# MoayedHajiAli/ElasticDiffusion-official

Measured on AMD Instinct MI355X. Metric: images/sec at 50 steps (SDXL 2048x1024), higher is better.
Workload: dtype fp16

## Files before the change

### elasticdiffusion_official_amd/csrc/gemm_kernels.hip

```cpp
#include <hip/hip_runtime.h>
#include <stdint.h>
#include <stdlib.h>

#include "elastic_hip.h"

namespace {

typedef float f32x4 __attribute__((ext_vector_type(4)));
typedef __bf16 bf16x8 __attribute__((ext_vector_type(8)));
typedef _Float16 f16x8 __attribute__((ext_vector_type(8)));
typedef uint32_t u32x4 __attribute__((ext_vector_type(4)));
typedef __attribute__((address_space(3))) void* lds_ptr_t;

struct BF {
  typedef bf16x8 v8;
  static __device__ __forceinline__ f32x4 mfma(v8 a, v8 b, f32x4 c) {
    return __builtin_amdgcn_mfma_f32_16x16x32_bf16(a, b, c, 0, 0, 0);
  }
  static __device__ __forceinline__ float to_f32(uint16_t h) { return __builtin_bit_cast(float, (uint32_t)h << 16); }
  static __device__ __forceinline__ uint16_t from_f32(float f) { return __builtin_bit_cast(uint16_t, (__bf16)f); }
  static __device__ __forceinline__ uint32_t pack2(float lo, float hi) {
    typedef float f2 __attribute__((ext_vector_type(2)));
    typedef __bf16 b2 __attribute__((ext_vector_type(2)));
    return __builtin_bit_cast(uint32_t, __builtin_convertvector(f2{lo, hi}, b2));
  }
};
struct HF {
  typedef f16x8 v8;
  static __device__ __forceinline__ f32x4 mfma(v8 a, v8 b, f32x4 c) {
    return __builtin_amdgcn_mfma_f32_16x16x32_f16(a, b, c, 0, 0, 0);
  }
  static __device__ __forceinline__ float to_f32(uint16_t h) { return (float)__builtin_bit_cast(_Float16, h); }
  static __device__ __forceinline__ uint16_t from_f32(float f) { return __builtin_bit_cast(uint16_t, (_Float16)f); }
  static __device__ __forceinline__ uint32_t pack2(float lo, float hi) {
    typedef float f2 __attribute__((ext_vector_type(2)));
    typedef _Float16 h2 __attribute__((ext_vector_type(2)));
    return __builtin_bit_cast(uint32_t, __builtin_convertvector(f2{lo, hi}, h2));
  }
};

constexpr int BM = 256;
constexpr int BN = 128;
constexpr int BK = 64;
constexpr int SUB = 1024;
constexpr int W_REGION = 32768;
constexpr int BUF = 65536;

__device__ __forceinline__ int swz(int p) { return p ^ (((p >> 9) & 1) << 5); }
__device__ __forceinline__ constexpr int x_sub(int rg, int kh) { return (rg * 2 + kh) * SUB; }
__device__ __forceinline__ constexpr int w_sub(int rg, int kh) { return W_REGION + (rg * 2 + kh) * SUB; }

__device__ __forceinline__ float gelu_as(float x) {
  const float z = __builtin_fabsf(x) * 0.70710678118654752f;
  const float t = __builtin_amdgcn_rcpf(__builtin_fmaf(0.3275911f, z, 1.0f));
  float p = __builtin_fmaf(1.061405429f, t, -1.453152027f);
  p = __builtin_fmaf(p, t, 1.421413741f);
  p = __builtin_fmaf(p, t, -0.284496736f);
  p = __builtin_fmaf(p, t, 0.254829592f);
  const float q = p * t * __builtin_amdgcn_exp2f(-1.4426950408889634f * z * z);
  const float h = 0.5f * x * q;
  return x > 0.f ? x - h : h;
}

__device__ __forceinline__ float abs_mul(float a, float b) {
  float r;
  asm("v_mul_f32_e64 %0, |%1|, %2" : "=v"(r) : "v"(a), "v"(b));
  return r;
}
__device__ __forceinline__ float relu1(float a) {
  float r;
  asm("v_max_f32_e32 %0, 0, %1" : "=v"(r) : "v"(a));
  return r;
}
__device__ __forceinline__ float geglu_one(float v, float g) {
  const float z = abs_mul(g, 0.70710678118654752f);
  const float t = __builtin_amdgcn_rcpf(__builtin_fmaf(0.3275911f, z, 1.0f));
  float p = __builtin_fmaf(0.5f * 1.061405429f, t, 0.5f * -1.453152027f);
  p = __builtin_fmaf(p, t, 0.5f * 1.421413741f);
  p = __builtin_fmaf(p, t, 0.5f * -0.284496736f);
  p = __builtin_fmaf(p, t, 0.5f * 0.254829592f);
  const float hq = (p * t) * __builtin_amdgcn_exp2f((-1.4426950408889634f * z) * z);
  return v * (relu1(g) - abs_mul(g, hq));
}

#define ED_WAIT_VM(n) asm volatile("s_waitcnt vmcnt(" #n ")" ::: "memory")
#define ED_WAIT_LGKM(n) asm volatile("s_waitcnt lgkmcnt(" #n ")" ::: "memory")
#define ED_BARRIER()                          \
  do {                                        \
    asm volatile("s_barrier" ::: "memory");   \
    __builtin_amdgcn_sched_barrier(0);        \
  } while (0)

struct Ctx {
  __amdgpu_buffer_rsrc_t xr, wr_;
  int x_voff[2], w_voff[2];
  int px_mask[2];
  int img_w, cin2, cpt;
  int wave;
  int xrd, wrd;
};

constexpr int CONV_UP2X = 2;
constexpr int CONV_S2 = 3;
constexpr int CONV_S2P0 = 4;
struct KPos {
  int tile, tap, ct, w;
};
template <int CONV>
__device__ __forceinline__ KPos k_next(KPos p, int cpt) {
  ++p.tile;
  if (CONV) {
    ++p.tap;
    p.w += cpt;
    if (p.tap == 9) {
      p.tap = 0;
      ++p.ct;
      p.w = p.ct;
    }
  } else {
    p.w = p.tile;
  }
  return p;
}

template <int BUFI, int CONV>
__device__ __forceinline__ void stage_x(uint8_t* lds, const Ctx& c, KPos p, int h) {
  const int rg = (c.wave & 3) + 8 * (c.wave >> 2) + 4 * h;
  uint8_t* dst = lds + BUFI * BUF + x_sub(0, 0) + rg * (2 * SUB);
  if (CONV) {
    const int dy = p.tap / 3 - 1, dx = p.tap - 3 * (p.tap / 3) - 1;
    int delta;
    if (CONV == CONV_UP2X) {
      const int yp = (c.px_mask[h] >> 16) & 1, xp = (c.px_mask[h] >> 17) & 1;
      delta = (((yp + dy) >> 1) * c.img_w + ((xp + dx) >> 1)) * c.cin2 + p.ct * (BK * 2);
    } else {
      delta = (dy * c.img_w + dx) * c.cin2 + p.ct * (BK * 2);
    }
    const int vo = ((c.px_mask[h] >> p.tap) & 1) ? c.x_voff[h] + delta : (int)0x80000000;
    __builtin_amdgcn_raw_ptr_buffer_load_lds(c.xr, (lds_ptr_t)dst, 16, vo, 0, 0, 0);
    __builtin_amdgcn_raw_ptr_buffer_load_lds(c.xr, (lds_ptr_t)(dst + SUB), 16, vo + 64, 0, 0, 0);
  } else {
    const int vo = c.x_voff[h] + p.tile * (BK * 2);
    __builtin_amdgcn_raw_ptr_buffer_load_lds(c.xr, (lds_ptr_t)dst, 16, vo, 0, 0, 0);
    __builtin_amdgcn_raw_ptr_buffer_load_lds(c.xr, (lds_ptr_t)(dst + SUB), 16, vo + 64, 0, 0, 0);
  }
}
template <int BUFI>
__device__ __forceinline__ void stage_w(uint8_t* lds, const Ctx& c, int widx, int g) {
  const int rg = 8 * g + c.wave;
  const int vo = c.w_voff[g] + widx * (BK * 2);
  uint8_t* dst = lds + BUFI * BUF + w_sub(0, 0) + rg * (2 * SUB);
  __builtin_amdgcn_raw_ptr_buffer_load_lds(c.wr_, (lds_ptr_t)dst, 16, vo, 0, 0, 0);
  __builtin_amdgcn_raw_ptr_buffer_load_lds(c.wr_, (lds_ptr_t)(dst + SUB), 16, vo + 64, 0, 0, 0);
}

template <class T>
struct Frags {
  typename T::v8 x[4][2];
  typename T::v8 wv[2][2];
  typename T::v8 wg[2][2];
};

template <class T, int BUFI>
__device__ __forceinline__ void read_x(const uint8_t* lds, const Ctx& c, Frags<T>& f, int mh) {
#pragma unroll
  for (int mf = 0; mf < 4; ++mf)
#pragma unroll
    for (int kh = 0; kh < 2; ++kh)
      f.x[mf][kh] = *reinterpret_cast<const typename T::v8*>(lds + c.xrd + BUFI * BUF + x_sub(mh * 4 + mf, kh));
}
template <class T, int BUFI, int G>
__device__ __forceinline__ void read_w(const uint8_t* lds, const Ctx& c, Frags<T>& f) {
#pragma unroll
  for (int nf = 0; nf < 2; ++nf)
#pragma unroll
    for (int kh = 0; kh < 2; ++kh) {
      typename T::v8 v = *reinterpret_cast<const typename T::v8*>(lds + c.wrd + BUFI * BUF + w_sub(8 * G + nf, kh) - W_REGION);
      if (G == 0) f.wv[nf][kh] = v; else f.wg[nf][kh] = v;
    }
}

template <class T, int MH, int G>
__device__ __forceinline__ void mma16(f32x4 (&acc)[8][4], const Frags<T>& f) {
  __builtin_amdgcn_s_setprio(1);
#pragma unroll
  for (int kh = 0; kh < 2; ++kh)
#pragma unroll
    for (int mf = 0; mf < 4; ++mf)
#pragma unroll
      for (int nf = 0; nf < 2; ++nf)
        acc[MH * 4 + mf][G * 2 + nf] = T::mfma(G == 0 ? f.wv[nf][kh] : f.wg[nf][kh], f.x[mf][kh], acc[MH * 4 + mf][G * 2 + nf]);
  __builtin_amdgcn_s_setprio(0);
}

template <class T, int BUFI, int CONV, bool FIRST = false>
__device__ __forceinline__ void tile_phases(uint8_t* lds, const Ctx& c, Frags<T>& f, f32x4 (&acc)[8][4], int tile, bool s1,
                                            bool s2, KPos p1, KPos p2) {
  read_w<T, BUFI, 0>(lds, c, f);
  __builtin_amdgcn_sched_barrier(0);
  read_x<T, BUFI>(lds, c, f, 0);
  if (s1) stage_x<BUFI ^ 1, CONV>(lds, c, p1, 1);
  ED_WAIT_LGKM(8);
  if (FIRST) ED_WAIT_VM(10);
  ED_BARRIER();
  ED_WAIT_LGKM(0);
  __builtin_amdgcn_sched_barrier(0);
  mma16<T, 0, 0>(acc, f);
  if (FIRST) ED_WAIT_VM(10);
  ED_BARRIER();
  read_w<T, BUFI, 1>(lds, c, f);
  if (s2) stage_w<BUFI>(lds, c, p2.w, 0);
  if (FIRST) ED_WAIT_VM(10);
  ED_BARRIER();
  ED_WAIT_LGKM(0);
  __builtin_amdgcn_sched_barrier(0);
  mma16<T, 0, 1>(acc, f);
  if (FIRST) ED_WAIT_VM(10);
  ED_BARRIER();
  read_x<T, BUFI>(lds, c, f, 1);
  if (s2) stage_x<BUFI, CONV>(lds, c, p2, 0);
  ED_BARRIER();
  ED_WAIT_LGKM(0);
  __builtin_amdgcn_sched_barrier(0);
  mma16<T, 1, 1>(acc, f);
  ED_BARRIER();
  if (s2) {
    stage_w<BUFI>(lds, c, p2.w, 1);
    ED_WAIT_VM(6);
  } else {
    ED_WAIT_VM(0);
  }
  ED_BARRIER();
  mma16<T, 1, 0>(acc, f);
  ED_BARRIER();
}

constexpr int TWO_MIN_TILES = 20;
template <class T, int BUFI, int CONV>
__device__ __forceinline__ void tile_phases_two(uint8_t* lds, const Ctx& c, Frags<T>& f, f32x4 (&acc)[8][4], int tile, bool s1, bool s2,
                                                KPos p1, KPos p2) {
  read_w<T, BUFI, 0>(lds, c, f);
  read_x<T, BUFI>(lds, c, f, 0);
  read_w<T, BUFI, 1>(lds, c, f);
  if (s1) stage_x<BUFI ^ 1, CONV>(lds, c, p1, 1);
  ED_WAIT_LGKM(0);
  ED_BARRIER();
  mma16<T, 0, 0>(acc, f);
  mma16<T, 0, 1>(acc, f);
  ED_BARRIER();
  read_x<T, BUFI>(lds, c, f, 1);
  if (s2) {
    stage_w<BUFI>(lds, c, p2.w, 0);
    stage_x<BUFI, CONV>(lds, c, p2, 0);
    stage_w<BUFI>(lds, c, p2.w, 1);
    ED_WAIT_VM(6);
  } else {
    ED_WAIT_VM(0);
  }
  ED_WAIT_LGKM(0);
  ED_BARRIER();
  mma16<T, 1, 1>(acc, f);
  mma16<T, 1, 0>(acc, f);
  ED_BARRIER();
}

template <class T, int BUFI, int CONV>
__device__ __forceinline__ void tile_phases_half(uint8_t* lds, const Ctx& c, Frags<T>& f, f32x4 (&acc)[8][4], int tile, bool s1, bool s2,
                                                 KPos p1, KPos p2) {
  read_w<T, BUFI, 0>(lds, c, f);
  read_x<T, BUFI>(lds, c, f, 0);
  if (s1) stage_x<BUFI ^ 1, CONV>(lds, c, p1, 1);
  ED_WAIT_LGKM(0);
  ED_BARRIER();
  mma16<T, 0, 0>(acc, f);
  ED_BARRIER();
  read_x<T, BUFI>(lds, c, f, 1);
  if (s2) {
    stage_w<BUFI>(lds, c, p2.w, 0);
    stage_x<BUFI, CONV>(lds, c, p2, 0);
    ED_WAIT_VM(4);
  } else {
    ED_WAIT_VM(0);
  }
  ED_WAIT_LGKM(0);
  ED_BARRIER();
  mma16<T, 1, 0>(acc, f);
  ED_BARRIER();
}

template <class T, int BUFI, int CONV>
__device__ __forceinline__ void tile_phases_rows(uint8_t* lds, const Ctx& c, Frags<T>& f, f32x4 (&acc)[8][4], bool s1, bool s2, KPos p1,
                                                 KPos p2) {
  read_w<T, BUFI, 0>(lds, c, f);
  read_x<T, BUFI>(lds, c, f, 0);
  if (s1) stage_w<BUFI ^ 1>(lds, c, p1.w, 1);
  ED_WAIT_LGKM(0);
  ED_BARRIER();
  mma16<T, 0, 0>(acc, f);
  ED_BARRIER();
  read_w<T, BUFI, 1>(lds, c, f);
  if (s2) {
    stage_w<BUFI>(lds, c, p2.w, 0);
    stage_x<BUFI, CONV>(lds, c, p2, 0);
    ED_WAIT_VM(4);
  } else {
    ED_WAIT_VM(0);
  }
  ED_WAIT_LGKM(0);
  ED_BARRIER();
  mma16<T, 0, 1>(acc, f);
  ED_BARRIER();
}

template <class T, int EPI, int CONV, bool ADD = true, bool OUT32 = false, bool TWO = false, bool ROWS = false>
__global__ void __launch_bounds__(512, 2)
k_gemm_8phase(const uint16_t* __restrict__ x, const uint16_t* __restrict__ w, const uint16_t* __restrict__ bias,
              const uint16_t* __restrict__ row_bias, const uint16_t* __restrict__ residual, uint16_t* __restrict__ out, int M,
              int K, int I, int n_blocks_n, int n_blocks, int img_h, int img_w, int rows_per_sample, float out_scale,
              const float* __restrict__ act_absmax) {
  __shared__ __attribute__((aligned(1024))) uint8_t lds[2 * BUF];

  const int bid = blockIdx.x;
  const int q = n_blocks >> 3, r = n_blocks & 7, xcd = bid & 7;
  const int tid = (xcd < r ? xcd * (q + 1) : r * (q + 1) + (xcd - r) * q) + (bid >> 3);
  const int n_blocks_m = n_blocks / n_blocks_n;
  const int per_group = 8 * n_blocks_n, grp = tid / per_group, first = grp * 8;
  const int rows_here = n_blocks_m - first < 8 ? n_blocks_m - first : 8;
  constexpr int TBM = ROWS ? BM / 2 : BM;
  constexpr int WROWS = TBM / 2;
  constexpr int NMB = WROWS / 16;
  const int m0 = (first + (tid % per_group) % rows_here) * TBM;
  const int n0 = ((tid % per_group) / rows_here) * (EPI == 0 ? BN : 2 * BN);
  const int gap = EPI == 0 ? I : BN;

  const int lane = threadIdx.x & 63;
  Ctx c;
  c.wave = __builtin_amdgcn_readfirstlane(threadIdx.x >> 6);
  const int wrow = c.wave >> 2, wcol = c.wave & 3;

  const int ps = swz(16 * lane), srow = ps >> 6, skb = ps & 63;
  const int row_bytes = K * 2;
  const int x_row_bytes = CONV ? row_bytes / 9 : row_bytes;
  c.xr = __builtin_amdgcn_make_buffer_rsrc((void*)x, 0, (int)((int64_t)(CONV == CONV_UP2X ? M / 4 : CONV >= CONV_S2 ? 4 * (int64_t)M : M) * x_row_bytes),
                                           0x00020000);
  c.wr_ = __builtin_amdgcn_make_buffer_rsrc((void*)w, 0, (int)((int64_t)(EPI == 0 ? 2 : 1) * I * row_bytes), 0x00020000);
  const int xrow0 = m0 + ((c.wave & 3) + (ROWS ? 4 : 8) * (c.wave >> 2)) * 16 + srow;
  c.x_voff[0] = xrow0 * x_row_bytes + skb;
  c.x_voff[1] = c.x_voff[0] + 64 * x_row_bytes;
  c.img_w = CONV == CONV_UP2X ? img_w / 2 : CONV >= CONV_S2 ? 2 * img_w : img_w;
  c.cin2 = x_row_bytes;
  c.cpt = CONV ? K / (9 * BK) : 1;
  c.px_mask[0] = c.px_mask[1] = 0;
  if (CONV) {
#pragma unroll
    for (int h = 0; h < 2; ++h) {
      const int m = xrow0 + 64 * h;
      if (m < M) {
        const int rem = m % (img_h * img_w), py = rem / img_w, px = rem - py * img_w;
        int mask = 0;
#pragma unroll
        for (int t = 0; t < 9; ++t) {
          if (CONV == CONV_S2) {
            if (2 * py + t / 3 - 1 >= 0 && 2 * px + t % 3 - 1 >= 0) mask |= 1 << t;
          } else if (CONV == CONV_S2P0) {
            if (2 * py + t / 3 < 2 * img_h && 2 * px + t % 3 < 2 * img_w) mask |= 1 << t;
          } else {
            const int yy = py + t / 3 - 1, xx = px + t % 3 - 1;
            if (yy >= 0 && yy < img_h && xx >= 0 && xx < img_w) mask |= 1 << t;
          }
        }
        c.px_mask[h] = mask;
        if (CONV == CONV_UP2X) {
          const int hs = img_h / 2, ws = img_w / 2;
          c.px_mask[h] = mask | ((py & 1) << 16) | ((px & 1) << 17);
          c.x_voff[h] = ((m / (img_h * img_w)) * (hs * ws) + (py >> 1) * ws + (px >> 1)) * x_row_bytes + skb;
        }
        if (CONV >= CONV_S2) {
          const int o1 = CONV == CONV_S2P0 ? 1 : 0;
          c.x_voff[h] = (((m / (img_h * img_w)) * (2 * img_h) + 2 * py + o1) * (2 * img_w) + 2 * px + o1) * x_row_bytes + skb;
        }
      }
    }
  }
  c.w_voff[0] = (n0 + 32 * (c.wave >> 1) + 8 * (srow >> 2) + (srow & 3) + 4 * (c.wave & 1)) * row_bytes + skb;
  c.w_voff[1] = c.w_voff[0] + gap * row_bytes;
  const int rd = swz((lane & 15) * 64 + (lane >> 4) * 16);
  c.xrd = rd + wrow * 8 * (2 * SUB);
  c.wrd = rd + W_REGION + wcol * 2 * (2 * SUB);

  const int ncol = n0 + 32 * wcol + 8 * (lane >> 4);
  u32x4 bias_v = {0, 0, 0, 0}, bias_g = {0, 0, 0, 0};
  if (bias && !OUT32) {
    if (EPI == 0 || ncol < I) bias_v = *reinterpret_cast<const u32x4*>(bias + ncol);
    if (EPI == 0 || ncol + gap < I) bias_g = *reinterpret_cast<const u32x4*>(bias + gap + ncol);
  }

  f32x4 acc[8][4];
#pragma unroll
  for (int a = 0; a < 8; ++a)
#pragma unroll
    for (int b = 0; b < 4; ++b) acc[a][b] = f32x4{0.f, 0.f, 0.f, 0.f};
  Frags<T> f;

  const int nt = K / BK;
  const KPos p0 = {0, 0, 0, 0};
  KPos pa = k_next<CONV>(p0, c.cpt);
  KPos pb = k_next<CONV>(pa, c.cpt);
  const bool half = !ROWS && EPI == 1 && n0 + BN >= I;
  if (ROWS) {
    stage_w<0>(lds, c, 0, 0);
    stage_x<0, CONV>(lds, c, p0, 0);
    stage_w<0>(lds, c, 0, 1);
    if (nt > 1) {
      stage_w<1>(lds, c, pa.w, 0);
      stage_x<1, CONV>(lds, c, pa, 0);
      ED_WAIT_VM(4);
    } else {
      ED_WAIT_VM(0);
    }
    ED_BARRIER();
    if (wrow == 1) ED_BARRIER();
    int tr = 0;
    for (; tr + 1 < nt; tr += 2) {
      tile_phases_rows<T, 0, CONV>(lds, c, f, acc, true, tr + 2 < nt, pa, pb);
      pa = pb;
      pb = k_next<CONV>(pb, c.cpt);
      tile_phases_rows<T, 1, CONV>(lds, c, f, acc, tr + 2 < nt, tr + 3 < nt, pa, pb);
      pa = pb;
      pb = k_next<CONV>(pb, c.cpt);
    }
    if (tr < nt) tile_phases_rows<T, 0, CONV>(lds, c, f, acc, false, false, pa, pb);
    if (wrow == 0) ED_BARRIER();
  } else if (half) {
    stage_w<0>(lds, c, 0, 0);
    stage_x<0, CONV>(lds, c, p0, 0);
    stage_x<0, CONV>(lds, c, p0, 1);
    if (nt > 1) {
      stage_w<1>(lds, c, pa.w, 0);
      stage_x<1, CONV>(lds, c, pa, 0);
      ED_WAIT_VM(4);
    } else {
      ED_WAIT_VM(0);
    }
    ED_BARRIER();
    if (wrow == 1) ED_BARRIER();
    int th = 0;
    for (; th + 1 < nt; th += 2) {
      tile_phases_half<T, 0, CONV>(lds, c, f, acc, th, true, th + 2 < nt, pa, pb);
      pa = pb;
      pb = k_next<CONV>(pb, c.cpt);
      tile_phases_half<T, 1, CONV>(lds, c, f, acc, th + 1, th + 2 < nt, th + 3 < nt, pa, pb);
      pa = pb;
      pb = k_next<CONV>(pb, c.cpt);
    }
    if (th < nt) tile_phases_half<T, 0, CONV>(lds, c, f, acc, th, false, false, pa, pb);
    if (wrow == 0) ED_BARRIER();
  } else {
  stage_w<0>(lds, c, 0, 0);
  stage_x<0, CONV>(lds, c, p0, 0);
  stage_w<0>(lds, c, 0, 1);
  stage_x<0, CONV>(lds, c, p0, 1);
  constexpr bool two = TWO;
  const bool early = nt >= 3 && !two;
  if (nt > 1) {
    stage_w<1>(lds, c, pa.w, 0);
    stage_x<1, CONV>(lds, c, pa, 0);
    stage_w<1>(lds, c, pa.w, 1);
    if (early) ED_WAIT_VM(10);
    else ED_WAIT_VM(6);
  } else {
    ED_WAIT_VM(0);
  }
  ED_BARRIER();
  if (wrow == 1) ED_BARRIER();

  int t = 0;
  if (two) {
    for (; t + 1 < nt; t += 2) {
      tile_phases_two<T, 0, CONV>(lds, c, f, acc, t, true, t + 2 < nt, pa, pb);
      pa = pb;
      pb = k_next<CONV>(pb, c.cpt);
      tile_phases_two<T, 1, CONV>(lds, c, f, acc, t + 1, t + 2 < nt, t + 3 < nt, pa, pb);
      pa = pb;
      pb = k_next<CONV>(pb, c.cpt);
    }
    if (t < nt) tile_phases_two<T, 0, CONV>(lds, c, f, acc, t, false, false, pa, pb);
    t = nt;
  }
  if (early) {
    tile_phases<T, 0, CONV, true>(lds, c, f, acc, 0, true, true, pa, pb);
    pa = pb;
    pb = k_next<CONV>(pb, c.cpt);
    tile_phases<T, 1, CONV>(lds, c, f, acc, 1, true, 3 < nt, pa, pb);
    pa = pb;
    pb = k_next<CONV>(pb, c.cpt);
    t = 2;
  }
  for (; t + 1 < nt; t += 2) {
    tile_phases<T, 0, CONV>(lds, c, f, acc, t, true, t + 2 < nt, pa, pb);
    pa = pb;
    pb = k_next<CONV>(pb, c.cpt);
    tile_phases<T, 1, CONV>(lds, c, f, acc, t + 1, t + 2 < nt, t + 3 < nt, pa, pb);
    pa = pb;
    pb = k_next<CONV>(pb, c.cpt);
  }
  if (t < nt) tile_phases<T, 0, CONV>(lds, c, f, acc, t, false, false, pa, pb);
  if (wrow == 0) ED_BARRIER();
  }

  if (OUT32) {
    const float* biasf = reinterpret_cast<const float*>(bias);
    const float* resf = reinterpret_cast<const float*>(residual);
    float* outf = reinterpret_cast<float*>(out);
    if (act_absmax) {
      const int E = (int)((__builtin_bit_cast(uint32_t, *act_absmax) >> 23) & 0xffu) - 127;
      const int e = E > 14 ? E - 14 : 0;
      out_scale *= __builtin_bit_cast(float, (uint32_t)(127 + e) << 23);
    }
    const bool col_v = ncol < I, col_g = ncol + gap < I;
    f32x4 b32[2][2] = {{f32x4{0.f, 0.f, 0.f, 0.f}, f32x4{0.f, 0.f, 0.f, 0.f}}, {f32x4{0.f, 0.f, 0.f, 0.f}, f32x4{0.f, 0.f, 0.f, 0.f}}};
    if (biasf) {
#pragma unroll
      for (int fr = 0; fr < 2; ++fr) {
        if (col_v) b32[0][fr] = *reinterpret_cast<const f32x4*>(biasf + ncol + 4 * fr);
        if (col_g) b32[1][fr] = *reinterpret_cast<const f32x4*>(biasf + ncol + gap + 4 * fr);
      }
    }
#pragma unroll
    for (int mb = 0; mb < NMB; ++mb) {
      const int m = m0 + WROWS * wrow + 16 * mb + (lane & 15);
      if (m >= M) continue;
#pragma unroll
      for (int hf = 0; hf < 2; ++hf) {
        if (!(hf == 0 ? col_v : col_g)) continue;
        const int64_t o = (int64_t)m * I + ncol + hf * gap;
#pragma unroll
        for (int fr = 0; fr < 2; ++fr) {
          f32x4 v = acc[mb][2 * hf + fr] * out_scale + b32[hf][fr];
          if (ADD && resf) v += *reinterpret_cast<const f32x4*>(resf + o + 4 * fr);
          *reinterpret_cast<f32x4*>(outf + o + 4 * fr) = v;
        }
      }
    }
    return;
  }
  float bv[2][4], bg[2][4];
#pragma unroll
  for (int e = 0; e < 8; ++e) {
    bv[e >> 2][e & 3] = T::to_f32((uint16_t)(bias_v[e >> 1] >> (16 * (e & 1))));
    bg[e >> 2][e & 3] = T::to_f32((uint16_t)(bias_g[e >> 1] >> (16 * (e & 1))));
  }
#pragma unroll
  for (int mb = 0; mb < NMB; ++mb) {
    const int m = m0 + WROWS * wrow + 16 * mb + (lane & 15);
    if (EPI == 0) {
      uint32_t pk[4];
#pragma unroll
      for (int nf = 0; nf < 2; ++nf)
#pragma unroll
        for (int jj = 0; jj < 2; ++jj) {
          const float o0 = geglu_one(acc[mb][nf][2 * jj] + bv[nf][2 * jj], acc[mb][2 + nf][2 * jj] + bg[nf][2 * jj]);
          const float o1 = geglu_one(acc[mb][nf][2 * jj + 1] + bv[nf][2 * jj + 1], acc[mb][2 + nf][2 * jj + 1] + bg[nf][2 * jj + 1]);
          pk[nf * 2 + jj] = T::pack2(o0, o1);
        }
      if (m < M) *reinterpret_cast<u32x4*>(out + (int64_t)m * I + ncol) = u32x4{pk[0], pk[1], pk[2], pk[3]};
    } else {
      const bool ok_v = m < M && ncol < I, ok_g = m < M && ncol + gap < I;
      u32x4 av[2] = {u32x4{0, 0, 0, 0}, u32x4{0, 0, 0, 0}}, ag[2] = {u32x4{0, 0, 0, 0}, u32x4{0, 0, 0, 0}};
      if (ADD && row_bias) {
        const int64_t rb = (int64_t)(m / rows_per_sample) * I;
        if (ok_v) av[0] = *reinterpret_cast<const u32x4*>(row_bias + rb + ncol);
        if (ok_g) ag[0] = *reinterpret_cast<const u32x4*>(row_bias + rb + ncol + gap);
      }
      if (ADD && residual) {
        if (ok_v) av[1] = *reinterpret_cast<const u32x4*>(residual + (int64_t)m * I + ncol);
        if (ok_g) ag[1] = *reinterpret_cast<const u32x4*>(residual + (int64_t)m * I + ncol + gap);
      }
      uint32_t pv[4], pg[4];
#pragma unroll
      for (int e = 0; e < 8; e += 2) {
        float v0 = acc[mb][e >> 2][e & 3] + bv[e >> 2][e & 3], v1 = acc[mb][e >> 2][(e & 3) + 1] + bv[e >> 2][(e & 3) + 1];
        float g0 = acc[mb][2 + (e >> 2)][e & 3] + bg[e >> 2][e & 3], g1 = acc[mb][2 + (e >> 2)][(e & 3) + 1] + bg[e >> 2][(e & 3) + 1];
        if (ADD) {
#pragma unroll
          for (int a = 0; a < 2; ++a) {
            v0 += T::to_f32((uint16_t)av[a][e >> 1]), v1 += T::to_f32((uint16_t)(av[a][e >> 1] >> 16));
            g0 += T::to_f32((uint16_t)ag[a][e >> 1]), g1 += T::to_f32((uint16_t)(ag[a][e >> 1] >> 16));
          }
        }
        pv[e >> 1] = (uint32_t)T::from_f32(v0) | ((uint32_t)T::from_f32(v1) << 16);
        pg[e >> 1] = (uint32_t)T::from_f32(g0) | ((uint32_t)T::from_f32(g1) << 16);
      }
      if (ok_v) *reinterpret_cast<u32x4*>(out + (int64_t)m * I + ncol) = u32x4{pv[0], pv[1], pv[2], pv[3]};
      if (ok_g) *reinterpret_cast<u32x4*>(out + (int64_t)m * I + ncol + gap) = u32x4{pg[0], pg[1], pg[2], pg[3]};
    }
  }
}

struct TilePos {
  int m0, n0;
};
__device__ __forceinline__ TilePos geglu_tile_of(int bid, int n_blocks, int n_blocks_n) {
  const int q = n_blocks >> 3, r = n_blocks & 7, xcd = bid & 7;
  const int tid = (xcd < r ? xcd * (q + 1) : r * (q + 1) + (xcd - r) * q) + (bid >> 3);
  const int n_blocks_m = n_blocks / n_blocks_n;
  const int per_group = 8 * n_blocks_n, grp = tid / per_group, first = grp * 8;
  const int rows_here = n_blocks_m - first < 8 ? n_blocks_m - first : 8;
  return TilePos{(first + (tid % per_group) % rows_here) * BM, ((tid % per_group) / rows_here) * BN};
}

template <class T>
__global__ void __launch_bounds__(512, 2)
k_geglu_persist(const uint16_t* __restrict__ x, const uint16_t* __restrict__ w, const uint16_t* __restrict__ bias,
                uint16_t* __restrict__ out, int M, int K, int I, int n_blocks_n, int n_blocks) {
  __shared__ __attribute__((aligned(1024))) uint8_t lds[2 * BUF];
  const int lane = threadIdx.x & 63;
  const int wave = __builtin_amdgcn_readfirstlane(threadIdx.x >> 6);
  const int wrow = wave >> 2, wcol = wave & 3;
  const int ps = swz(16 * lane), srow = ps >> 6, skb = ps & 63;
  const int row_bytes = K * 2;
  const int rd = swz((lane & 15) * 64 + (lane >> 4) * 16);
  const int nt = K / BK;
  const bool early = nt >= 3;

  auto setup = [&](TilePos tp) {
    Ctx c;
    c.wave = wave;
    c.xr = __builtin_amdgcn_make_buffer_rsrc((void*)x, 0, (int)((int64_t)M * row_bytes), 0x00020000);
    c.wr_ = __builtin_amdgcn_make_buffer_rsrc((void*)w, 0, (int)((int64_t)2 * I * row_bytes), 0x00020000);
    c.x_voff[0] = (tp.m0 + ((wave & 3) + 8 * (wave >> 2)) * 16 + srow) * row_bytes + skb;
    c.x_voff[1] = c.x_voff[0] + 64 * row_bytes;
    c.img_w = 0, c.cin2 = row_bytes, c.cpt = 1;
    c.px_mask[0] = c.px_mask[1] = 0;
    c.w_voff[0] = (tp.n0 + 32 * (wave >> 1) + 8 * (srow >> 2) + (srow & 3) + 4 * (wave & 1)) * row_bytes + skb;
    c.w_voff[1] = c.w_voff[0] + I * row_bytes;
    c.xrd = rd + wrow * 8 * (2 * SUB);
    c.wrd = rd + W_REGION + wcol * 2 * (2 * SUB);
    return c;
  };
  auto load_bias = [&](int ncol, u32x4& bv_raw, u32x4& bg_raw) {
    bv_raw = u32x4{0, 0, 0, 0}, bg_raw = u32x4{0, 0, 0, 0};
    if (bias) {
      bv_raw = *reinterpret_cast<const u32x4*>(bias + ncol);
      bg_raw = *reinterpret_cast<const u32x4*>(bias + I + ncol);
    }
  };
  auto issue_prologue = [&](const Ctx& c) {
    const KPos p0 = {0, 0, 0, 0}, p1 = {1, 0, 0, 1};
    stage_w<0>(lds, c, 0, 0);
    stage_x<0, false>(lds, c, p0, 0);
    stage_w<0>(lds, c, 0, 1);
    stage_x<0, false>(lds, c, p0, 1);
    if (nt > 1) {
      stage_w<1>(lds, c, 1, 0);
      stage_x<1, false>(lds, c, p1, 0);
      stage_w<1>(lds, c, 1, 1);
    }
  };

  int bid = blockIdx.x;
  TilePos tp = geglu_tile_of(bid, n_blocks, n_blocks_n);
  Ctx c = setup(tp);
  u32x4 bias_v, bias_g;
  load_bias(tp.n0 + 32 * wcol + 8 * (lane >> 4), bias_v, bias_g);
  issue_prologue(c);

  for (;;) {
    f32x4 acc[8][4];
#pragma unroll
    for (int a = 0; a < 8; ++a)
#pragma unroll
      for (int b = 0; b < 4; ++b) acc[a][b] = f32x4{0.f, 0.f, 0.f, 0.f};
    Frags<T> f;
    KPos pa = {1, 0, 0, 1}, pb = {2, 0, 0, 2};
    if (nt > 1) {
      if (early) ED_WAIT_VM(10);
      else ED_WAIT_VM(6);
    } else {
      ED_WAIT_VM(0);
    }
    ED_BARRIER();
    if (wrow == 1) ED_BARRIER();

    int t = 0;
    if (early) {
      tile_phases<T, 0, false, true>(lds, c, f, acc, 0, true, true, pa, pb);
      pa = pb, pb = KPos{pb.tile + 1, 0, 0, pb.tile + 1};
      tile_phases<T, 1, false>(lds, c, f, acc, 1, true, 3 < nt, pa, pb);
      pa = pb, pb = KPos{pb.tile + 1, 0, 0, pb.tile + 1};
      t = 2;
    }
    for (; t + 1 < nt; t += 2) {
      tile_phases<T, 0, false>(lds, c, f, acc, t, true, t + 2 < nt, pa, pb);
      pa = pb, pb = KPos{pb.tile + 1, 0, 0, pb.tile + 1};
      tile_phases<T, 1, false>(lds, c, f, acc, t + 1, t + 2 < nt, t + 3 < nt, pa, pb);
      pa = pb, pb = KPos{pb.tile + 1, 0, 0, pb.tile + 1};
    }
    if (t < nt) tile_phases<T, 0, false>(lds, c, f, acc, t, false, false, pa, pb);
    if (wrow == 0) ED_BARRIER();

    const int m0 = tp.m0, ncol = tp.n0 + 32 * wcol + 8 * (lane >> 4);
    float bv[2][4], bg[2][4];
#pragma unroll
    for (int e = 0; e < 8; ++e) {
      bv[e >> 2][e & 3] = T::to_f32((uint16_t)(bias_v[e >> 1] >> (16 * (e & 1))));
      bg[e >> 2][e & 3] = T::to_f32((uint16_t)(bias_g[e >> 1] >> (16 * (e & 1))));
    }
#pragma unroll
    for (int e = 0; e < 8; ++e) asm volatile("" : "+v"(bv[e >> 2][e & 3]), "+v"(bg[e >> 2][e & 3]));

    const int next = bid + (int)gridDim.x;
    const bool has_next = next < n_blocks;
    Ctx c2 = c;
    TilePos tp2 = tp;
    if (has_next) {
      tp2 = geglu_tile_of(next, n_blocks, n_blocks_n);
      c2 = setup(tp2);
      load_bias(tp2.n0 + 32 * wcol + 8 * (lane >> 4), bias_v, bias_g);
      __builtin_amdgcn_sched_barrier(0);
      issue_prologue(c2);
      __builtin_amdgcn_sched_barrier(0);
    }
#pragma unroll
    for (int mb = 0; mb < 8; ++mb) {
      const int m = m0 + 128 * wrow + 16 * mb + (lane & 15);
      uint32_t pk[4];
#pragma unroll
      for (int nf = 0; nf < 2; ++nf)
#pragma unroll
        for (int jj = 0; jj < 2; ++jj) {
          const float o0 = geglu_one(acc[mb][nf][2 * jj] + bv[nf][2 * jj], acc[mb][2 + nf][2 * jj] + bg[nf][2 * jj]);
          const float o1 = geglu_one(acc[mb][nf][2 * jj + 1] + bv[nf][2 * jj + 1], acc[mb][2 + nf][2 * jj + 1] + bg[nf][2 * jj + 1]);
          pk[nf * 2 + jj] = T::pack2(o0, o1);
        }
      if (m < M) *reinterpret_cast<u32x4*>(out + (int64_t)m * I + ncol) = u32x4{pk[0], pk[1], pk[2], pk[3]};
    }
    if (!has_next) break;
    bid = next, tp = tp2, c = c2;
  }
}

}

static int gemm_cus() {
  static int cus[16] = {0};
  int dev = 0;
  if (hipGetDevice(&dev) != hipSuccess || dev < 0 || dev >= 16) return 0;
  if (cus[dev] == 0) {
    int n = 0;
    if (hipDeviceGetAttribute(&n, hipDeviceAttributeMultiprocessorCount, dev) != hipSuccess || n < 8) return 0;
    cus[dev] = n / 8 * 8;
  }
  return cus[dev];
}
constexpr double ROWS_TILE_COST = 0.72;

template <int EPI, int CONV, bool OUT32 = false>
static int launch(const void* x, const void* w, const void* bias, const void* row_bias, const void* residual, void* out, int dtype,
                  int64_t M, int K, int I, int img_h, int img_w, int rows_per_sample, void* stream, float out_scale = 1.0f,
                  const float* act_absmax = nullptr) {
  if (M == 0) return 0;
  const int bad = (int)hipErrorInvalidValue;
  if (M < 0 || K % BK != 0 || K < BK || I <= 0 || (EPI == 0 ? I % BN != 0 : I % 8 != 0)) return bad;
  if (CONV && (K % (9 * BK) != 0 || img_h <= 0 || img_w <= 0 || M % ((int64_t)img_h * img_w) != 0)) return bad;
  if (CONV == CONV_UP2X && (img_h % 2 != 0 || img_w % 2 != 0 || row_bias || residual)) return bad;
  if (CONV >= CONV_S2 && (row_bias || residual || 4 * M * (int64_t)(K / 9) * 2 >= 0x7ffffff0ll)) return bad;
  if (row_bias && (rows_per_sample <= 0 || M % rows_per_sample != 0)) return bad;
  if (M * (int64_t)(CONV ? K / 9 : K) * 2 >= 0x7ffffff0ll || (int64_t)(EPI == 0 ? 2 : 1) * I * K * 2 >= 0x7ffffff0ll) return bad;
  if ((((uintptr_t)x | (uintptr_t)w | (uintptr_t)out | (uintptr_t)bias | (uintptr_t)row_bias | (uintptr_t)residual) & 15u)) return bad;
  const int nbn = EPI == 0 ? I / BN : (I + 2 * BN - 1) / (2 * BN);
  const int64_t nb256 = ((M + BM - 1) / BM) * nbn, nb128 = ((M + BM / 2 - 1) / (BM / 2)) * nbn;
  if (nb128 >= (1ll << 31) || M >= (1ll << 31)) return bad;
  hipStream_t s = (hipStream_t)stream;
  const bool add = EPI == 1 && (row_bias || residual);
  const bool two = CONV && K / BK >= TWO_MIN_TILES;
  bool rows = false;
  if (!OUT32 && EPI == 1 && CONV < CONV_UP2X) {
    const int cus = gemm_cus();
    const double r256 = (double)((nb256 + cus - 1) / cus), r128 = (double)((nb128 + cus - 1) / cus) * ROWS_TILE_COST;
    rows = cus > 0 && r128 < r256 - 1e-9;
    if (const char* e = getenv("ED_GEMM_ROWS")) rows = e[0] == '1' ? true : (e[0] == '0' ? false : rows);
  }
  const int64_t nb = rows ? nb128 : nb256;
#define ED_LAUNCH1(TT, ADD_, TWO_, ROWS_)                                                                                            \
  k_gemm_8phase<TT, EPI, CONV, ADD_, OUT32, TWO_, ROWS_><<<(int)nb, 512, 0, s>>>((const uint16_t*)x, (const uint16_t*)w, (const uint16_t*)bias, \
                                                             (const uint16_t*)row_bias, (const uint16_t*)residual, (uint16_t*)out,  \
                                                             (int)M, K, I, nbn, (int)nb, img_h, img_w, rows_per_sample > 0 ? rows_per_sample : 1, out_scale, \
                                                             act_absmax)
#define ED_LAUNCH(TT, ADD_)                                   \
  do {                                                        \
    if constexpr (OUT32 || EPI == 0) {                        \
      if constexpr (CONV) {                                   \
        if (two) ED_LAUNCH1(TT, ADD_, true, false);           \
        else ED_LAUNCH1(TT, ADD_, false, false);              \
      } else {                                                \
        ED_LAUNCH1(TT, ADD_, false, false);                   \
      }                                                       \
    } else if (CONV < CONV_UP2X && rows) {                    \
      if constexpr (CONV < CONV_UP2X) ED_LAUNCH1(TT, ADD_, false, true);   \
    } else if constexpr (CONV) {                              \
      if (two) ED_LAUNCH1(TT, ADD_, true, false);             \
      else ED_LAUNCH1(TT, ADD_, false, false);                \
    } else {                                                  \
      ED_LAUNCH1(TT, ADD_, false, false);                     \
    }                                                         \
  } while (0)
  if constexpr (OUT32) {
    if (dtype != ED_F16 || row_bias) return bad;
    if constexpr (CONV >= CONV_UP2X) {
      ED_LAUNCH(HF, false);
    } else {
      if (add) ED_LAUNCH(HF, true);
      else ED_LAUNCH(HF, false);
    }
  } else {
    if constexpr (CONV >= CONV_UP2X) {
      if (dtype == ED_BF16) ED_LAUNCH(BF, false);
      else if (dtype == ED_F16) ED_LAUNCH(HF, false);
      else return bad;
    } else if (dtype == ED_BF16) {
      if (EPI == 0 || add) ED_LAUNCH(BF, true);
      else ED_LAUNCH(BF, EPI == 0);
    } else if (dtype == ED_F16) {
      if (EPI == 0 || add) ED_LAUNCH(HF, true);
      else ED_LAUNCH(HF, EPI == 0);
    } else {
      return bad;
    }
  }
#undef ED_LAUNCH
#undef ED_LAUNCH1
  return (int)hipGetLastError();
}

extern "C" {

int ed_geglu_gemm(const void* x, const void* w, const void* bias, void* out, int dtype, int64_t M, int K, int I, void* stream) {
  if (M == 0) return 0;
  const int bad = (int)hipErrorInvalidValue;
  if (M < 0 || K % BK != 0 || K < BK || I <= 0 || I % BN != 0) return bad;
  if (M * (int64_t)K * 2 >= 0x7ffffff0ll || (int64_t)2 * I * K * 2 >= 0x7ffffff0ll) return bad;
  if ((((uintptr_t)x | (uintptr_t)w | (uintptr_t)out | (uintptr_t)bias) & 15u)) return bad;
  const int nbn = I / BN;
  const int64_t nb = ((M + BM - 1) / BM) * nbn;
  if (nb >= (1ll << 31) || M >= (1ll << 31)) return bad;
  const int ncu = gemm_cus();
  if (ncu <= 0) return (int)hipErrorInvalidDevice;
  const int grid = nb < ncu ? (int)nb : ncu;
  hipStream_t s = (hipStream_t)stream;
  if (dtype == ED_BF16)
    k_geglu_persist<BF><<<grid, 512, 0, s>>>((const uint16_t*)x, (const uint16_t*)w, (const uint16_t*)bias, (uint16_t*)out, (int)M, K, I, nbn, (int)nb);
  else if (dtype == ED_F16)
    k_geglu_persist<HF><<<grid, 512, 0, s>>>((const uint16_t*)x, (const uint16_t*)w, (const uint16_t*)bias, (uint16_t*)out, (int)M, K, I, nbn, (int)nb);
  else
    return bad;
  return (int)hipGetLastError();
}

int ed_linear(const void* x, const void* w, const void* bias, const void* residual, void* out, int dtype, int64_t M, int K, int N,
              void* stream) {
  return launch<1, 0>(x, w, bias, nullptr, residual, out, dtype, M, K, N, 0, 0, 0, stream);
}

int ed_conv3x3_nhwc(const void* x, const void* w, const void* bias, const void* sample_bias, const void* residual, void* out,
                    int dtype, int B, int H, int W, int Cin, int N, void* stream) {
  if (B < 0 || H <= 0 || W <= 0 || Cin <= 0) return (int)hipErrorInvalidValue;
  return launch<1, 1>(x, w, bias, sample_bias, residual, out, dtype, (int64_t)B * H * W, 9 * Cin, N, H, W, H * W, stream);
}

int ed_conv3x3_nhwc_up2x(const void* x, const void* w, const void* bias, void* out, int dtype, int B, int H, int W, int Cin, int N,
                         void* stream) {
  if (B < 0 || H <= 0 || W <= 0 || Cin <= 0) return (int)hipErrorInvalidValue;
  if ((int64_t)B * (H / 2) * (W / 2) * Cin * 2 >= 0x7ffffff0ll) return (int)hipErrorInvalidValue;
  return launch<1, CONV_UP2X>(x, w, bias, nullptr, nullptr, out, dtype, (int64_t)B * H * W, 9 * Cin, N, H, W, H * W, stream);
}

int ed_conv3x3_nhwc_s2(const void* x, const void* w, const void* bias, void* out, int dtype, int B, int H, int W, int Cin, int N,
                       void* stream) {
  if (B < 0 || H <= 0 || W <= 0 || Cin <= 0) return (int)hipErrorInvalidValue;
  return launch<1, CONV_S2>(x, w, bias, nullptr, nullptr, out, dtype, (int64_t)B * H * W, 9 * Cin, N, H, W, H * W, stream);
}

int ed_conv3x3_nhwc_f32out(const void* x, const void* w, const float* bias, const float* residual, float* out, int dtype, int B, int H, int W,
                           int Cin, int N, float out_scale, const float* act_absmax, void* stream) {
  if (B < 0 || H <= 0 || W <= 0 || Cin <= 0 || ((uintptr_t)act_absmax & 3u)) return (int)hipErrorInvalidValue;
  return launch<1, 1, true>(x, w, bias, nullptr, residual, out, dtype, (int64_t)B * H * W, 9 * Cin, N, H, W, H * W, stream, out_scale,
                               act_absmax);
}

int ed_conv3x3_nhwc_f32out_s2(const void* x, const void* w, const float* bias, float* out, int dtype, int B, int H, int W, int Cin, int N,
                              float out_scale, const float* act_absmax, void* stream) {
  if (B < 0 || H <= 0 || W <= 0 || Cin <= 0 || ((uintptr_t)act_absmax & 3u)) return (int)hipErrorInvalidValue;
  return launch<1, CONV_S2P0, true>(x, w, bias, nullptr, nullptr, out, dtype, (int64_t)B * H * W, 9 * Cin, N, H, W, H * W, stream, out_scale,
                                    act_absmax);
}

}
```

### elasticdiffusion_official_amd/csrc/vae_kernels.hip

```cpp
#include <hip/hip_runtime.h>
#include <stdint.h>

#include "elastic_hip.h"

namespace {

#define GV_THREADS 256
#define GV_UNROLL 4
#define GV_MAXG 256

__device__ __forceinline__ float silu32(float x) { return x / (1.0f + expf(-x)); }
__device__ __forceinline__ _Float16 sat16(float v) { return (_Float16)(v > 65504.f ? 65504.f : (v < -65504.f ? -65504.f : v)); }
__device__ __forceinline__ int split_exponent(float absmax) {
  const int E = (int)((__builtin_bit_cast(uint32_t, absmax) >> 23) & 0xffu) - 127;
  return E > 14 ? E - 14 : 0;
}

__global__ void __launch_bounds__(GV_THREADS)
k_gn32_nhwc_partial(const float* __restrict__ x, float* __restrict__ partial, int C, int HW, int G, int rows_per_block) {
  extern __shared__ float sh[];
  const int n = blockIdx.y, chunk = blockIdx.x;
  const int VC = C >> 2, cpg = C / G;
  const int ncol = (VC + GV_THREADS - 1) / GV_THREADS;
  const int R = ncol == 1 ? GV_THREADS / VC : 1;
  const int my_r = ncol == 1 ? threadIdx.x / VC : 0;
  const int my_c = ncol == 1 ? threadIdx.x % VC : threadIdx.x;
  const bool active = ncol == 1 ? (int)threadIdx.x < R * VC : true;
  const int r0 = chunk * rows_per_block, r1 = min(HW, r0 + rows_per_block);
  const float* base = x + (int64_t)n * HW * C;
  if (active) {
    for (int j = 0; j < ncol; ++j) {
      const int vc = my_c + j * GV_THREADS;
      if (vc >= VC) break;
      float s = 0.f, q = 0.f;
      const float K = base[((vc << 2) / cpg) * cpg];
      auto add = [&](float4 v) {
        v.x -= K, v.y -= K, v.z -= K, v.w -= K;
        s += (v.x + v.y) + (v.z + v.w);
        q += (v.x * v.x + v.y * v.y) + (v.z * v.z + v.w * v.w);
      };
      const float* col = base + (vc << 2);
      const int64_t step = (int64_t)R * C;
      int row = r0 + my_r;
      for (; row + (GV_UNROLL - 1) * R < r1; row += GV_UNROLL * R) {
        const float* p0 = col + (int64_t)row * C;
        float4 v[GV_UNROLL];
#pragma unroll
        for (int u = 0; u < GV_UNROLL; ++u) v[u] = *reinterpret_cast<const float4*>(p0 + u * step);
#pragma unroll
        for (int u = 0; u < GV_UNROLL; ++u) add(v[u]);
      }
      for (; row < r1; row += R) add(*reinterpret_cast<const float4*>(col + (int64_t)row * C));
      float* slot = sh + ((int64_t)my_r * VC + vc) * 2;
      slot[0] = s, slot[1] = q;
    }
  }
  __syncthreads();
  float* dst = partial + ((int64_t)n * gridDim.x + chunk) * 2 * G;
  const int cols_per_group = cpg >> 2;
  for (int g = threadIdx.x; g < G; g += GV_THREADS) {
    double s = 0.0, q = 0.0;
    for (int vc = g * cols_per_group; vc < (g + 1) * cols_per_group; ++vc)
      for (int r = 0; r < R; ++r) {
        const float* slot = sh + ((int64_t)r * VC + vc) * 2;
        s += (double)slot[0];
        q += (double)slot[1];
      }
    dst[2 * g] = (float)s;
    dst[2 * g + 1] = (float)q;
  }
}

template <bool ACT, bool SPLIT>
__global__ void __launch_bounds__(GV_THREADS)
k_gn32_nhwc_apply(const float* __restrict__ x, const float* __restrict__ gamma, const float* __restrict__ beta,
                  const float* __restrict__ partial, void* __restrict__ out, int C, int HW, int G, int rows_per_block, double count,
                  float eps) {
  __shared__ double red[2 * GV_THREADS];
  __shared__ float stats[2 * GV_MAXG];
  const int n = gridDim.y - 1 - blockIdx.y, chunk = gridDim.x - 1 - blockIdx.x, nchunks = gridDim.x;
  {
    const int parts = GV_THREADS / G > 0 ? GV_THREADS / G : 1;
    const int g = threadIdx.x % G, part = threadIdx.x / G;
    double s = 0.0, q = 0.0;
    if (part < parts) {
      const float* p = partial + (int64_t)n * nchunks * 2 * G + 2 * g;
      for (int c = part; c < nchunks; c += parts) {
        s += (double)p[(int64_t)c * 2 * G];
        q += (double)p[(int64_t)c * 2 * G + 1];
      }
    }
    red[2 * threadIdx.x] = s, red[2 * threadIdx.x + 1] = q;
    __syncthreads();
    if ((int)threadIdx.x < G) {
      double ss = 0.0, qq = 0.0;
      for (int k = 0; k < parts; ++k) {
        ss += red[2 * (k * G + threadIdx.x)];
        qq += red[2 * (k * G + threadIdx.x) + 1];
      }
      const double dmean = ss / count;
      double var = qq / count - dmean * dmean;
      if (var < 0.0) var = 0.0;
      const double mean = (double)x[(int64_t)n * HW * C + (int64_t)threadIdx.x * (C / G)] + dmean;
      stats[2 * threadIdx.x] = (float)mean;
      stats[2 * threadIdx.x + 1] = (float)(1.0 / sqrt(var + (double)eps));
    }
    __syncthreads();
  }
  const int VC = C >> 2, cpg = C / G;
  const int ncol = (VC + GV_THREADS - 1) / GV_THREADS;
  const int R = ncol == 1 ? GV_THREADS / VC : 1;
  const int my_r = ncol == 1 ? threadIdx.x / VC : 0;
  const int my_c = ncol == 1 ? threadIdx.x % VC : threadIdx.x;
  if (ncol == 1 && (int)threadIdx.x >= R * VC) return;
  const int r0 = chunk * rows_per_block, r1 = min(HW, r0 + rows_per_block);
  const float* xb = x + (int64_t)n * HW * C;
  for (int j = 0; j < ncol; ++j) {
    const int vc = my_c + j * GV_THREADS;
    if (vc >= VC) break;
    const int c0 = vc << 2, g = c0 / cpg;
    const float mean = stats[2 * g], rstd = stats[2 * g + 1];
    const float4 gm = *reinterpret_cast<const float4*>(gamma + c0), bt = *reinterpret_cast<const float4*>(beta + c0);
    const float a0 = rstd * gm.x, a1 = rstd * gm.y, a2 = rstd * gm.z, a3 = rstd * gm.w;
    const float b0 = fmaf(-a0, mean, bt.x), b1 = fmaf(-a1, mean, bt.y), b2 = fmaf(-a2, mean, bt.z), b3 = fmaf(-a3, mean, bt.w);
    auto norm = [&](const float4& v) {
      float4 o;
      o.x = fmaf(a0, v.x, b0), o.y = fmaf(a1, v.y, b1), o.z = fmaf(a2, v.z, b2), o.w = fmaf(a3, v.w, b3);
      if (ACT) o.x = silu32(o.x), o.y = silu32(o.y), o.z = silu32(o.z), o.w = silu32(o.w);
      return o;
    };
    auto store = [&](int64_t row, const float4& y) {
      if (SPLIT) {
        uint16_t* ob = reinterpret_cast<uint16_t*>(out) + ((int64_t)n * HW + row) * (3 * (int64_t)C) + c0;
        const _Float16 h0 = sat16(y.x), h1 = sat16(y.y), h2 = sat16(y.z), h3 = sat16(y.w);
        const _Float16 l0 = sat16(y.x - (float)h0), l1 = sat16(y.y - (float)h1), l2 = sat16(y.z - (float)h2), l3 = sat16(y.w - (float)h3);
        uint2 hi, lo;
        hi.x = (uint32_t)__builtin_bit_cast(uint16_t, h0) | ((uint32_t)__builtin_bit_cast(uint16_t, h1) << 16);
        hi.y = (uint32_t)__builtin_bit_cast(uint16_t, h2) | ((uint32_t)__builtin_bit_cast(uint16_t, h3) << 16);
        lo.x = (uint32_t)__builtin_bit_cast(uint16_t, l0) | ((uint32_t)__builtin_bit_cast(uint16_t, l1) << 16);
        lo.y = (uint32_t)__builtin_bit_cast(uint16_t, l2) | ((uint32_t)__builtin_bit_cast(uint16_t, l3) << 16);
        *reinterpret_cast<uint2*>(ob) = hi;
        *reinterpret_cast<uint2*>(ob + C) = lo;
        *reinterpret_cast<uint2*>(ob + 2 * C) = hi;
      } else {
        *reinterpret_cast<float4*>(reinterpret_cast<float*>(out) + ((int64_t)n * HW + row) * C + c0) = y;
      }
    };
    const int64_t step = (int64_t)R * C;
    int row = r0 + my_r;
    for (; row + (GV_UNROLL - 1) * R < r1; row += GV_UNROLL * R) {
      const float* p0 = xb + (int64_t)row * C + c0;
      float4 v[GV_UNROLL];
#pragma unroll
      for (int u = 0; u < GV_UNROLL; ++u) v[u] = *reinterpret_cast<const float4*>(p0 + u * step);
#pragma unroll
      for (int u = 0; u < GV_UNROLL; ++u) store(row + u * R, norm(v[u]));
    }
    for (; row < r1; row += R) store(row, norm(*reinterpret_cast<const float4*>(xb + (int64_t)row * C + c0)));
  }
}

template <int U>
__global__ void __launch_bounds__(256)
k_split32_nhwc(const float* __restrict__ x, uint16_t* __restrict__ out, int C, int H, int W, int64_t n_vec, const float* __restrict__ absmax) {
  const int VC = C >> 2;
  const float sc = absmax ? __builtin_bit_cast(float, (uint32_t)(127 - split_exponent(*absmax)) << 23) : 1.0f;
  for (int64_t i = (int64_t)blockIdx.x * blockDim.x + threadIdx.x; i < n_vec; i += (int64_t)gridDim.x * blockDim.x) {
    const int64_t pix = i / VC;
    const int c0 = (int)(i - pix * VC) << 2;
    const float4 v = *reinterpret_cast<const float4*>(x + pix * C + c0);
    const float f[4] = {v.x * sc, v.y * sc, v.z * sc, v.w * sc};
    uint32_t hw[2], lw[2];
#pragma unroll
    for (int e = 0; e < 4; e += 2) {
      uint16_t hb[2], lb[2];
#pragma unroll
      for (int j = 0; j < 2; ++j) {
        const _Float16 h = sat16(f[e + j]);
        const _Float16 l = sat16(f[e + j] - (float)h);
        hb[j] = __builtin_bit_cast(uint16_t, h), lb[j] = __builtin_bit_cast(uint16_t, l);
      }
      hw[e >> 1] = (uint32_t)hb[0] | ((uint32_t)hb[1] << 16);
      lw[e >> 1] = (uint32_t)lb[0] | ((uint32_t)lb[1] << 16);
    }
    const uint2 hi = {hw[0], hw[1]}, lo = {lw[0], lw[1]};
    const int64_t n = pix / ((int64_t)H * W), rem = pix - n * (int64_t)H * W;
    const int y = (int)(rem / W), xx = (int)(rem - (int64_t)y * W);
#pragma unroll
    for (int dy = 0; dy < U; ++dy)
#pragma unroll
      for (int dx = 0; dx < U; ++dx) {
        uint16_t* ob = out + ((n * (U * H) + (U * y + dy)) * (int64_t)(U * W) + (U * xx + dx)) * (3 * (int64_t)C) + c0;
        *reinterpret_cast<uint2*>(ob) = hi;
        *reinterpret_cast<uint2*>(ob + C) = lo;
        *reinterpret_cast<uint2*>(ob + 2 * C) = hi;
      }
  }
}

__global__ void __launch_bounds__(256)
k_absmax32(const float* __restrict__ x, uint32_t* __restrict__ out, int64_t n) {
  uint32_t m = 0;
  const int64_t n4 = n >> 2;
  for (int64_t i = (int64_t)blockIdx.x * blockDim.x + threadIdx.x; i < n4; i += (int64_t)gridDim.x * blockDim.x) {
    const uint4 v = *reinterpret_cast<const uint4*>(x + 4 * i);
    const uint32_t a = max(v.x & 0x7fffffffu, v.y & 0x7fffffffu), b = max(v.z & 0x7fffffffu, v.w & 0x7fffffffu);
    m = max(m, max(a, b));
  }
  if (blockIdx.x == 0 && (int64_t)threadIdx.x < n - 4 * n4) m = max(m, __builtin_bit_cast(uint32_t, x[4 * n4 + threadIdx.x]) & 0x7fffffffu);
#pragma unroll
  for (int off = 32; off > 0; off >>= 1) m = max(m, (uint32_t)__shfl_xor((int)m, off, 64));
  if ((threadIdx.x & 63) == 0 && m) atomicMax(out, m);
}

inline int done() { return (int)hipGetLastError(); }

inline int gv_chunks(int C, int HW, int* rows_per_block) {
  int rpb = (65536 + C - 1) / C;
  if ((HW + rpb - 1) / rpb > 256) rpb = (HW + 255) / 256;
  if (rpb < 1) rpb = 1;
  *rows_per_block = rpb;
  return (HW + rpb - 1) / rpb;
}

}

extern "C" {

int64_t ed_groupnorm_nhwc_f32_workspace(int N, int C, int HW, int G) {
  if (G <= 0 || C <= 0 || HW <= 0) return 0;
  int rpb;
  const int nchunks = gv_chunks(C, HW, &rpb);
  return (int64_t)N * nchunks * G * 2 * (int64_t)sizeof(float);
}

int ed_groupnorm_nhwc_f32(const void* x, const void* gamma, const void* beta, void* out, float* workspace, int N, int C, int HW, int G,
                          float eps, int act_silu, int split16, void* stream) {
  if (N == 0) return 0;
  if (N < 0 || G <= 0 || G > GV_MAXG || C % G != 0 || (C / G) % 4 != 0 || C > 4 * GV_THREADS * 4 || N > 65535 ||
      (((uintptr_t)x | (uintptr_t)out | (uintptr_t)gamma | (uintptr_t)beta | (uintptr_t)workspace) & 15u))
    return (int)hipErrorInvalidValue;
  hipStream_t s = (hipStream_t)stream;
  int rpb;
  const int nchunks = gv_chunks(C, HW, &rpb);
  dim3 grid(nchunks, N);
  const int VC = C / 4;
  const size_t lds = sizeof(float) * 2 * (size_t)VC * (VC <= GV_THREADS ? GV_THREADS / VC : 1);
  k_gn32_nhwc_partial<<<grid, GV_THREADS, lds, s>>>((const float*)x, workspace, C, HW, G, rpb);
  const double count = (double)HW * (C / G);
#define GV_APPLY(ACT, SPLIT)                                                                                                      \
  k_gn32_nhwc_apply<ACT, SPLIT><<<grid, GV_THREADS, 0, s>>>((const float*)x, (const float*)gamma, (const float*)beta, workspace, \
                                                            out, C, HW, G, rpb, count, eps)
  if (act_silu && split16) GV_APPLY(true, true);
  else if (act_silu) GV_APPLY(true, false);
  else if (split16) GV_APPLY(false, true);
  else GV_APPLY(false, false);
#undef GV_APPLY
  return done();
}

int ed_absmax_f32(const void* x, int64_t n, float* out, void* stream) {
  if (n < 0 || !out || ((uintptr_t)x & 15u) || ((uintptr_t)out & 3u)) return (int)hipErrorInvalidValue;
  hipStream_t s = (hipStream_t)stream;
  hipError_t e = hipMemsetAsync(out, 0, sizeof(float), s);
  if (e != hipSuccess) return (int)e;
  if (n == 0) return 0;
  int64_t blocks = ((n >> 2) + 256 * 8 - 1) / (256 * 8);
  if (blocks < 1) blocks = 1;
  if (blocks > 2048) blocks = 2048;
  k_absmax32<<<(unsigned)blocks, 256, 0, s>>>((const float*)x, reinterpret_cast<uint32_t*>(out), n);
  return done();
}

int ed_split_f32_nhwc(const void* x, void* out, int N, int C, int H, int W, int upsample2x, const float* absmax, void* stream) {
  if (N == 0) return 0;
  if (N < 0 || C <= 0 || C % 4 != 0 || H <= 0 || W <= 0 || (((uintptr_t)x | (uintptr_t)out) & 15u) || ((3 * C * 2) % 8) != 0 ||
      ((uintptr_t)absmax & 3u))
    return (int)hipErrorInvalidValue;
  const int64_t n_vec = (int64_t)N * H * W * (C / 4);
  int64_t blocks = (n_vec + 255) / 256;
  if (blocks > 65536 * 16) blocks = 65536 * 16;
  hipStream_t s = (hipStream_t)stream;
  if (upsample2x) k_split32_nhwc<2><<<(unsigned)blocks, 256, 0, s>>>((const float*)x, (uint16_t*)out, C, H, W, n_vec, absmax);
  else k_split32_nhwc<1><<<(unsigned)blocks, 256, 0, s>>>((const float*)x, (uint16_t*)out, C, H, W, n_vec, absmax);
  return done();
}

}
```

### elasticdiffusion_official_amd/models.py

```python
import math
import os
from types import SimpleNamespace

import torch
import torch.nn as nn
import torch.nn.functional as F

from . import ops


FUSED_KERNELS = True


CHANNELS_LAST = os.environ.get("ED_CHANNELS_LAST", "1") == "1"


_HALF = (torch.bfloat16, torch.float16)


def _fusable(x):
    return FUSED_KERNELS and x.is_cuda and x.dtype in _HALF and x.is_contiguous()


def _fusable_nhwc(x):
    return FUSED_KERNELS and x.is_cuda and x.dtype in _HALF and ops.is_nhwc(x)


def _stream32(x, module_dtype):
    return x.dtype == torch.float32 and module_dtype in _HALF


def _derived(module, slot, params, build):
    key = tuple((id(p), p.data_ptr(), p._version, p.dtype, str(p.device)) for p in params)
    cache = module.__dict__.setdefault("_derived", {})
    hit = cache.get(slot)
    if hit is None or hit[0] != key:
        hit = cache[slot] = (key, build())
    return hit[1]


def _f32_params(norm):
    w, b = norm.weight, norm.bias
    return _derived(norm, "f32", (w, b), lambda: (w.detach().float(), b.detach().float()))


def _f32_bias(mod):
    b = mod.bias
    return None if b is None else _derived(mod, "bias32", (b,), lambda: b.detach().float())


def group_norm_act(norm, x, silu=False, tokens=False, chan_bias=None, conv_bias=None):
    N, C, H, W = x.shape
    G = norm.num_groups
    cpg = C // G
    s32 = _stream32(x, norm.weight.dtype)
    nhwc = not s32 and _fusable_nhwc(x) and C % 8 == 0 and cpg >= 8
    if (chan_bias is not None or conv_bias is not None) and (
            s32 or not (FUSED_TEMB_ADD and (nhwc or (_fusable(x) and (H * W) % 8 == 0 and not tokens)))):
        if conv_bias is not None:
            x = x + conv_bias[None, :, None, None]
        if chan_bias is not None:
            x = x + chan_bias[:, :, None, None]
        chan_bias = conv_bias = None
        nhwc = not s32 and _fusable_nhwc(x) and C % 8 == 0 and cpg >= 8
    if s32 or nhwc:
        if nhwc:
            y = ops.groupnorm_nhwc(x, norm.weight, norm.bias, G, norm.eps, silu=silu,
                                   chan_bias=None if chan_bias is None else chan_bias.contiguous(), conv_bias=conv_bias)
        elif FUSED_KERNELS and x.is_cuda and C % 8 == 0 and cpg >= 8 and C <= 4096 and G <= 256 and ops.is_nhwc(x):
            y = ops.groupnorm_nhwc_s32(x, norm.weight, norm.bias, G, norm.eps, silu=silu)
        else:
            y = F.group_norm(x, G, *_f32_params(norm), norm.eps)
            if silu:
                y = F.silu(y)
            y = y.to(norm.weight.dtype)
            if CHANNELS_LAST and y.is_cuda:
                y = y.contiguous(memory_format=torch.channels_last)
        return y.permute(0, 2, 3, 1).reshape(N, H * W, C) if tokens else y
    if chan_bias is not None or conv_bias is not None:
        return ops.groupnorm(x, norm.weight, norm.bias, G, norm.eps, silu=silu,
                             chan_bias=None if chan_bias is None else chan_bias.contiguous(), conv_bias=conv_bias)
    if _fusable(x) and (H * W) % 8 == 0 and (not tokens or cpg % 4 == 0):
        return ops.groupnorm(x, norm.weight, norm.bias, G, norm.eps, silu=silu, tokens=tokens)
    if FUSED_KERNELS and x.is_cuda and x.dtype == torch.float32 and not tokens and norm.weight.dtype == torch.float32:
        if VAE_SPLIT_CONV and ops.is_nhwc(x) and ops.groupnorm_nhwc_f32_ok(C, G):
            return ops.groupnorm_nhwc_f32(x, norm.weight, norm.bias, G, norm.eps, silu=silu)
        if VAE_HIP_GROUPNORM and x.is_contiguous() and (H * W) % 4 == 0 and N * G <= 65535:
            return ops.groupnorm_f32(x, norm.weight, norm.bias, G, norm.eps, silu=silu)
    y = F.group_norm(x, G, norm.weight, norm.bias, norm.eps)
    if silu:
        y = F.silu(y)
    return y.permute(0, 2, 3, 1).reshape(N, H * W, C) if tokens else y


FUSED_LAYERNORM = True
FUSED_TEMB_ADD = True
FUSED_CONV_BIAS = True
FUSED_ADD_LAYERNORM = True
FUSED_TOKENS_ADD = True
FLASH_ATTENTION = True
FUSED_QKV = True
HIP_GEGLU_GEMM = True
HIP_LINEAR = True
FUSED_SKIP_CAT = True
FUSED_PROJ_OUT_ADD = True
HIP_DOWNSAMPLE_CONV = False
FUSED_RESIDUAL_LINEAR = False
FUSED_UPSAMPLE_CONV = True
HIP_CONV3X3 = True
VAE_HIP_GROUPNORM = True
VAE_HIP_ATTENTION = True
VAE_NCHW_RESIDUAL = True
VAE_SPLIT_CONV = True
VAE_SPLIT_DOWNSAMPLE = True
for _name in filter(None, os.environ.get("ED_DISABLE", "").split(",")):
    if _name not in globals() or not isinstance(globals()[_name], bool):
        raise RuntimeError(f"ED_DISABLE: unknown switch {_name!r}")
    globals()[_name] = False


def fused_unet_entry_points():
    hip_conv = FUSED_KERNELS and HIP_CONV3X3 and CHANNELS_LAST
    on = [("ed_groupnorm_nhwc" if CHANNELS_LAST else "ed_groupnorm", FUSED_KERNELS),
          ("ed_geglu_gemm" if HIP_GEGLU_GEMM else "ed_geglu", FUSED_KERNELS),
          ("ed_layernorm", FUSED_KERNELS and FUSED_LAYERNORM),
          ("ed_flash_attention", FUSED_KERNELS and FLASH_ATTENTION),
          ("ed_add_layernorm", FUSED_KERNELS and FUSED_ADD_LAYERNORM),
          ("ed_tokens_add_nchw", FUSED_KERNELS and FUSED_TOKENS_ADD and not CHANNELS_LAST),
          ("ed_bias_residual_add", FUSED_KERNELS and FUSED_CONV_BIAS and FUSED_TEMB_ADD and not hip_conv)]
    return {n for n, flag in on if flag}


def linear_(x, weight, bias=None):
    if (HIP_LINEAR and FUSED_KERNELS and _fusable(x) and weight.dtype == x.dtype and weight.is_contiguous()
            and ops.linear_wins(x.numel() // x.shape[-1], x.shape[-1], weight.shape[0])):
        return ops.linear(x, weight, bias)
    return F.linear(x, weight, bias)


def linear_res_(x, weight, bias, residual):
    if (FUSED_RESIDUAL_LINEAR and residual is not None and HIP_LINEAR and FUSED_KERNELS and _fusable(x) and _fusable(residual)
            and weight.dtype == x.dtype == residual.dtype and weight.is_contiguous()
            and residual.shape == x.shape[:-1] + (weight.shape[0],)
            and ops.linear_wins(x.numel() // x.shape[-1], x.shape[-1], weight.shape[0])):
        return ops.linear(x, weight, bias, residual=residual), True
    return linear_(x, weight, bias), False


def _hip_conv3x3(conv, like, cin):
    w = conv.weight
    if not (HIP_CONV3X3 and w.dtype == like.dtype and w.is_contiguous(memory_format=torch.channels_last)):
        return False
    B, _, H, W = like.shape
    return ops.conv3x3_wins(B, H, W, cin, w.shape[0])


def _hip_conv_pair(blk, like, cin):
    cout = blk.conv1.out_channels
    return (_fusable_nhwc(like) and cout % 8 == 0 and cout // blk.norm2.num_groups >= 8
            and _hip_conv3x3(blk.conv1, like, cin) and _hip_conv3x3(blk.conv2, like, cout))


def _shortcut_nhwc(sc, x):
    return linear_(x.permute(0, 2, 3, 1), sc.weight.reshape(sc.out_channels, -1), sc.bias).permute(0, 3, 1, 2)


def _sliced(x, nb, fn):
    outs = [fn(x[i:i + nb]) for i in range(0, x.shape[0], nb)]
    return outs[0] if len(outs) == 1 else torch.cat(outs).contiguous(memory_format=torch.channels_last)


def _to_nchw(x):
    return x if x.is_contiguous() else x.contiguous()


def _vae_split_ok(x, blk):
    if not (VAE_SPLIT_CONV and FUSED_KERNELS and x.is_cuda and x.dtype == torch.float32 and x.dim() == 4
            and blk.time_emb_proj is None and blk.conv1.weight.dtype == torch.float32):
        return False
    B, cin, H, W = x.shape
    cout = blk.conv1.out_channels
    return (ops.groupnorm_nhwc_f32_ok(cin, blk.norm1.num_groups) and ops.groupnorm_nhwc_f32_ok(cout, blk.norm2.num_groups)
            and cin % 64 == 0 and cout % 64 == 0 and H * W * 3 * max(cin, cout) * 2 < 2 ** 31 - 16)


def _split_weight(conv):
    return _derived(conv, "split", (conv.weight,), lambda: ops.split_conv_weight(conv.weight))


def _split_shortcut(sc, C1):
    def build():
        w2d = sc.weight.detach().reshape(sc.weight.shape[0], -1)
        return w2d[:, :C1].contiguous(), w2d[:, C1:].contiguous()
    return _derived(sc, ("ksplit", C1), (sc.weight,), build)


def prepare_vae_split(vae):
    if not (VAE_SPLIT_CONV and FUSED_KERNELS):
        return 0
    n = 0
    for m in vae.modules():
        convs = ()
        if isinstance(m, ResnetBlock2D) and m.time_emb_proj is None:
            convs = (m.conv1, m.conv2)
        elif isinstance(m, Upsample2D) and m.vae:
            convs = (m.conv,)
        elif isinstance(m, Downsample2D) and m.padding == 0:
            convs = (m.conv,)
        for c in convs:
            w = c.weight
            if w.is_cuda and w.dtype == torch.float32 and w.shape[1] % 64 == 0 and w.shape[0] % 8 == 0 and tuple(w.shape[2:]) == (3, 3):
                _split_weight(c)
                n += 1
    return n


def layer_norm(norm, x):
    D = x.shape[-1]
    if norm.elementwise_affine and _stream32(x, norm.weight.dtype):
        if FUSED_LAYERNORM and FUSED_KERNELS and x.is_cuda and x.is_contiguous() and D % 8 == 0 and D <= 2048:
            return ops.layernorm_s32(x, norm.weight, norm.bias, norm.eps)
        return F.layer_norm(x, (D,), *_f32_params(norm), norm.eps).to(norm.weight.dtype)
    if FUSED_LAYERNORM and _fusable(x) and D % 8 == 0 and D <= 2048 and norm.elementwise_affine:
        return ops.layernorm(x, norm.weight, norm.bias, norm.eps)
    return norm(x)


def add_layer_norm(norm, a, b):
    D = a.shape[-1]
    if (FUSED_ADD_LAYERNORM and _fusable(a) and _fusable(b) and a.shape == b.shape and D % 8 == 0 and D <= 2048
            and norm.elementwise_affine):
        return ops.add_layernorm(a, b, norm.weight, norm.bias, norm.eps)
    if (FUSED_ADD_LAYERNORM and FUSED_KERNELS and norm.elementwise_affine and _fusable(a) and _stream32(b, a.dtype) and b.is_cuda
            and b.is_contiguous() and a.shape == b.shape and D % 8 == 0 and D <= 2048 and norm.weight.dtype == a.dtype):
        return ops.add_layernorm_s32(a, b, norm.weight, norm.bias, norm.eps)
    s = a + b
    return s, layer_norm(norm, s)


class ModelOutput(dict):

    __getattr__ = dict.__getitem__


def timestep_embedding(t, dim, flip_sin_to_cos=True, freq_shift=0.0, max_period=10000.0):
    half = dim // 2
    exponent = -math.log(max_period) * torch.arange(half, dtype=torch.float32, device=t.device) / (half - freq_shift)
    emb = t[:, None].float() * torch.exp(exponent)[None, :]
    sin, cos = torch.sin(emb), torch.cos(emb)
    return torch.cat([cos, sin], dim=-1) if flip_sin_to_cos else torch.cat([sin, cos], dim=-1)


class TimestepEmbedding(nn.Module):
    def __init__(self, in_dim, dim):
        super().__init__()
        self.linear_1 = nn.Linear(in_dim, dim)
        self.linear_2 = nn.Linear(dim, dim)

    def forward(self, x):
        return self.linear_2(F.silu(self.linear_1(x)))


SHORTCUT_AS_GEMM = False


class ResnetBlock2D(nn.Module):
    def __init__(self, cin, cout, temb_dim=None, eps=1e-5, groups=32):
        super().__init__()
        self.norm1 = nn.GroupNorm(groups, cin, eps=eps)
        self.conv1 = nn.Conv2d(cin, cout, 3, padding=1)
        self.time_emb_proj = nn.Linear(temb_dim, cout) if temb_dim else None
        self.norm2 = nn.GroupNorm(groups, cout, eps=eps)
        self.conv2 = nn.Conv2d(cout, cout, 3, padding=1)
        self.conv_shortcut = nn.Conv2d(cin, cout, 1) if cin != cout else None

    def forward(self, x, temb=None):
        if _vae_split_ok(x, self):
            return self._forward_split(x)
        tb = self.time_emb_proj(F.silu(temb)) if self.time_emb_proj is not None else None
        sc, c1, c2 = self.conv_shortcut, self.conv1, self.conv2
        cout = c1.out_channels
        if _stream32(x, c1.weight.dtype):
            def add_to_stream(h):
                if sc is None:
                    return x + h
                xs = x.to(h.dtype)
                return (_shortcut_nhwc(sc, xs) if ops.is_nhwc(xs) else sc(xs)).float() + h

            def close(a2):
                B, _, H, W = a2.shape
                if a2.dtype == torch.float16 and ops.conv3x3_f32out_ok(B, H, W, cout, cout):
                    res = x if sc is None else _shortcut_nhwc(sc, x.to(a2.dtype)).float()
                    res = res.contiguous(memory_format=torch.channels_last)
                    return ops.conv3x3_f32out(a2, c2.weight, _f32_bias(c2), res, 1.0)
                return add_to_stream(ops.conv3x3_nhwc(a2, c2.weight, c2.bias))

            a = group_norm_act(self.norm1, x, silu=True)
            if _hip_conv_pair(self, a, a.shape[1]):
                return self._hip_convs(a, tb, close)
            return add_to_stream(c2(group_norm_act(self.norm2, c1(a), silu=True, chan_bias=tb)))
        cl = _fusable_nhwc(x) and cout % 8 == 0 and cout // self.norm2.num_groups >= 8
        if x.shape[1] // self.norm1.num_groups >= 8 and _hip_conv_pair(self, x, x.shape[1]):
            return self._hip_convs(group_norm_act(self.norm1, x, silu=True), tb, lambda a2: ops.conv3x3_nhwc(
                a2, c2.weight, c2.bias, residual=x if sc is None else _shortcut_nhwc(sc, x)))
        if FUSED_CONV_BIAS and FUSED_TEMB_ADD and (cl or (_fusable(x) and (x.shape[2] * x.shape[3]) % 8 == 0)):
            h = F.conv2d(group_norm_act(self.norm1, x, silu=True), c1.weight, None, padding=1)
            a = group_norm_act(self.norm2, h, silu=True, chan_bias=tb, conv_bias=c1.bias)
            h = F.conv2d(a, c2.weight, None, padding=1)
            if sc is None:
                return ops.bias_residual_add(h, c2.bias, x)
            if cl:
                res = F.linear(x.permute(0, 2, 3, 1), sc.weight.reshape(cout, -1)).permute(0, 3, 1, 2)
            else:
                res = F.conv2d(x, sc.weight, None)
            return ops.bias_residual_add(h, c2.bias, res, sc.bias)
        h = c1(group_norm_act(self.norm1, x, silu=True))
        a = group_norm_act(self.norm2, h, silu=True, chan_bias=tb)
        if sc is not None and SHORTCUT_AS_GEMM and _fusable(x):
            N, C, H, W = x.shape
            h = F.conv2d(a, c2.weight, c2.bias + sc.bias, padding=1)
            w = sc.weight.view(1, cout, C).expand(N, -1, -1)
            return torch.baddbmm(h.view(N, cout, H * W), w, x.view(N, C, H * W)).view(N, cout, H, W)
        return (x if sc is None else sc(x)) + c2(a)

    def _hip_convs(self, a, tb, close):
        h = ops.conv3x3_nhwc(a, self.conv1.weight, self.conv1.bias, sample_bias=None if tb is None else tb.contiguous())
        return close(group_norm_act(self.norm2, h, silu=True))

    def forward_cat(self, x, skip, temb=None):
        sc, c2 = self.conv_shortcut, self.conv2
        C1, C = x.shape[1], x.shape[1] + skip.shape[1]
        if (FUSED_SKIP_CAT and FUSED_KERNELS and sc is not None and _fusable_nhwc(skip) and x.dtype == skip.dtype
                and _hip_conv_pair(self, x, C) and ops.groupnorm_nhwc_cat_ok(x, skip, self.norm1.num_groups)
                and self.conv1.weight.shape[1] == C and sc.weight.dtype == x.dtype):
            def close(a2):
                w1, w2 = _split_shortcut(sc, C1)
                xt, st = x.permute(0, 2, 3, 1), skip.permute(0, 2, 3, 1)
                y = linear_(xt, w1, sc.bias)
                M, cout = st.numel() // st.shape[-1], w2.shape[0]
                if HIP_LINEAR and ops.linear_wins(M, st.shape[-1], cout):
                    y = ops.linear(st, w2, None, residual=y)
                else:
                    y = torch.addmm(y.reshape(M, cout), st.reshape(M, -1), w2.t()).view(y.shape)
                return ops.conv3x3_nhwc(a2, c2.weight, c2.bias, residual=y.permute(0, 3, 1, 2))

            tb = self.time_emb_proj(F.silu(temb)) if self.time_emb_proj is not None else None
            n1 = self.norm1
            return self._hip_convs(ops.groupnorm_nhwc_cat(x, skip, n1.weight, n1.bias, n1.num_groups, n1.eps, silu=True), tb, close)
        return self(torch.cat([x, skip], dim=1), temb)

    def _forward_split(self, x):
        n1, n2, sc = self.norm1, self.norm2, self.conv_shortcut
        _, cin, H, W = x.shape

        def block(xs):
            w1, s1 = _split_weight(self.conv1)
            w2, s2 = _split_weight(self.conv2)
            a = ops.groupnorm_nhwc_f32(xs, n1.weight, n1.bias, n1.num_groups, n1.eps, silu=True, split=True)
            h = ops.conv3x3_f32out(a, w1, self.conv1.bias, None, s1)
            a = ops.groupnorm_nhwc_f32(h, n2.weight, n2.bias, n2.num_groups, n2.eps, silu=True, split=True)
            res = xs if sc is None else _shortcut_nhwc(sc, xs)
            return ops.conv3x3_f32out(a, w2, self.conv2.bias, res, s2)

        per = H * W * 3 * max(cin, self.conv1.out_channels) * 2
        return _sliced(x.contiguous(memory_format=torch.channels_last), max(1, (2 ** 31 - 16) // per), block)


class Attention(nn.Module):
    def __init__(self, dim, heads, head_dim, cross_dim=None, bias=False):
        super().__init__()
        inner = heads * head_dim
        self.heads = heads
        self.to_q = nn.Linear(dim, inner, bias=bias)
        self.to_k = nn.Linear(cross_dim or dim, inner, bias=bias)
        self.to_v = nn.Linear(cross_dim or dim, inner, bias=bias)
        self.to_out = nn.ModuleList([nn.Linear(inner, dim), nn.Dropout(0.0)])
        self.to_k_ip = self.to_v_ip = None
        self.ip_tokens = 0
        self.ip_scale = 1.0

    def set_ip_adapter(self, to_k_ip=None, to_v_ip=None, tokens=0):
        for name, mod in (("to_k_ip", to_k_ip), ("to_v_ip", to_v_ip)):
            if isinstance(getattr(self, name), nn.Module):
                delattr(self, name)
            setattr(self, name, mod)
        self.ip_tokens = int(tokens) if to_k_ip is not None else 0
        self.__dict__.pop("_derived", None)

    def _fused_weight(self, names, q_scale=None):
        ws = [getattr(self, n).weight for n in names]

        def build():
            parts = [w.detach() for w in ws]
            if q_scale is not None:
                parts[0] = (parts[0].float() * q_scale).to(parts[0].dtype)
            return torch.cat(parts, dim=0).contiguous()
        return _derived(self, (names, q_scale), ws, build)

    def project_kv(self, context, out=None):
        w = self._fused_weight(("to_k", "to_v"))
        if out is None:
            out = torch.empty(context.shape[:-1] + (w.shape[0],), dtype=context.dtype, device=context.device)
        if self.ip_tokens:
            nt = context.shape[-2] - self.ip_tokens
            out[..., :nt, :] = torch.matmul(context[..., :nt, :], w.t())
            out[..., nt:, :] = torch.matmul(context[..., nt:, :], self._fused_weight(("to_k_ip", "to_v_ip")).t())
            return out
        torch.matmul(context, w.t(), out=out)
        return out

    def forward(self, x, context=None, kv=None, residual=None):
        out, fused = self._attend(x, context, kv, residual)
        return out if residual is None else (out, fused)

    def _attend(self, x, context, kv, residual):
        B, N, _ = x.shape
        inner = self.to_q.out_features
        if (FLASH_ATTENTION and _fusable(x) and inner % self.heads == 0 and inner // self.heads in (40, 64, 80, 160)
                and self.to_q.bias is None
                and (context is None or (_fusable(context) and context.dtype == x.dtype))):
            if context is None:
                c = ops.flash_prescale(N, N, 3 * inner if FUSED_QKV else inner) if inner == self.heads * 64 else None
                if FUSED_QKV:
                    qkv = linear_(x, self._fused_weight(("to_q", "to_k", "to_v"), c))
                    q, k, v = qkv[..., :inner], qkv[..., inner:2 * inner], qkv[..., 2 * inner:]
                else:
                    q = linear_(x, self.to_q.weight if c is None else self._fused_weight(("to_q",), c))
                    k, v = self.to_k(x), self.to_v(x)
                o = ops.flash_attention(q, k, v, self.heads, prescaled=c is not None)
            elif self.ip_tokens:
                q = linear_(x, self.to_q.weight)
                if kv is None:
                    kv = self.project_kv(context)
                k, v = kv[..., :inner], kv[..., inner:]
                nt = kv.shape[1] - self.ip_tokens
                if ops.flash_attention_ip_ok(inner // self.heads, nt, self.ip_tokens):
                    o = ops.flash_attention_ip(q, k, v, self.heads, nt, self.ip_scale)
                else:
                    o = ops.flash_attention(q, k[:, :nt], v[:, :nt], self.heads)
                    o = o.add_(ops.flash_attention(q, k[:, nt:], v[:, nt:], self.heads), alpha=self.ip_scale)
            else:
                q = linear_(x, self.to_q.weight)
                if kv is not None or FUSED_QKV:
                    if kv is None:
                        kv = self.project_kv(context)
                    k, v = kv[..., :inner], kv[..., inner:]
                else:
                    k, v = self.to_k(context), self.to_v(context)
                o = ops.flash_attention(q, k, v, self.heads)
            return linear_res_(o, self.to_out[0].weight, self.to_out[0].bias, residual)
        ctx = x if context is None else context
        q = self.to_q(x).view(B, N, self.heads, -1).transpose(1, 2)
        if context is not None and self.ip_tokens:
            if kv is None:
                kv = self.project_kv(ctx)
            nt = kv.shape[1] - self.ip_tokens
            k, v = (t.reshape(B, kv.shape[1], self.heads, -1).transpose(1, 2) for t in (kv[..., :inner], kv[..., inner:]))
            o = F.scaled_dot_product_attention(q, k[:, :, :nt], v[:, :, :nt])
            o = o + self.ip_scale * F.scaled_dot_product_attention(q, k[:, :, nt:], v[:, :, nt:])
            return self.to_out[0](o.transpose(1, 2).reshape(B, N, -1)), False
        if kv is not None:
            k, v = (t.reshape(B, ctx.shape[1], self.heads, -1).transpose(1, 2) for t in (kv[..., :inner], kv[..., inner:]))
        else:
            k = self.to_k(ctx).view(B, ctx.shape[1], self.heads, -1).transpose(1, 2)
            v = self.to_v(ctx).view(B, ctx.shape[1], self.heads, -1).transpose(1, 2)
        o = F.scaled_dot_product_attention(q, k, v)
        return self.to_out[0](o.transpose(1, 2).reshape(B, N, -1)), False


class GEGLU(nn.Module):
    def __init__(self, dim, inner):
        super().__init__()
        self.proj = nn.Linear(dim, inner * 2)

    def forward(self, x):
        if (HIP_GEGLU_GEMM and FUSED_KERNELS and _fusable(x) and self.proj.weight.dtype == x.dtype
                and ops.geglu_gemm_wins(x.numel() // x.shape[-1], x.shape[-1], self.proj.out_features // 2)):
            return ops.geglu_gemm(x, self.proj.weight, self.proj.bias)
        y = self.proj(x)
        if _fusable(y) and (y.shape[-1] // 2) % 8 == 0:
            return ops.geglu(y, y.shape[-1] // 2)
        h, gate = y.chunk(2, dim=-1)
        return h * F.gelu(gate)


class FeedForward(nn.Module):
    def __init__(self, dim):
        super().__init__()
        self.net = nn.ModuleList([GEGLU(dim, dim * 4), nn.Dropout(0.0), nn.Linear(dim * 4, dim)])

    def forward(self, x, residual=None):
        if residual is not None:
            return linear_res_(self.net[0](x), self.net[2].weight, self.net[2].bias, residual)
        return linear_(self.net[0](x), self.net[2].weight, self.net[2].bias)


class BasicTransformerBlock(nn.Module):
    def __init__(self, dim, heads, head_dim, cross_dim):
        super().__init__()
        self.norm1 = nn.LayerNorm(dim)
        self.attn1 = Attention(dim, heads, head_dim)
        self.norm2 = nn.LayerNorm(dim)
        self.attn2 = Attention(dim, heads, head_dim, cross_dim)
        self.norm3 = nn.LayerNorm(dim)
        self.ff = FeedForward(dim)

    def forward(self, x, context, pending=None, kv=None):
        if pending is not None:
            x, h = add_layer_norm(self.norm1, pending, x)
        else:
            h = layer_norm(self.norm1, x)
        a, fused = self.attn1(h, residual=x)
        x, h = (a, layer_norm(self.norm2, a)) if fused else add_layer_norm(self.norm2, a, x)
        a, fused = self.attn2(h, context, None if kv is None else kv.get(id(self.attn2)), residual=x)
        x, h = (a, layer_norm(self.norm3, a)) if fused else add_layer_norm(self.norm3, a, x)
        a, fused = self.ff(h, residual=x)
        return (None, a) if fused else (a, x)


class Transformer2DModel(nn.Module):
    def __init__(self, ch, heads, depth, cross_dim, linear_proj):
        super().__init__()
        self.linear_proj = linear_proj
        self.norm = nn.GroupNorm(32, ch, eps=1e-6)
        self.proj_in = nn.Linear(ch, ch) if linear_proj else nn.Conv2d(ch, ch, 1)
        self.transformer_blocks = nn.ModuleList([BasicTransformerBlock(ch, heads, ch // heads, cross_dim) for _ in range(depth)])
        self.proj_out = nn.Linear(ch, ch) if linear_proj else nn.Conv2d(ch, ch, 1)

    def forward(self, x, context, kv=None):
        B, C, H, W = x.shape
        if self.linear_proj:
            h = linear_(group_norm_act(self.norm, x, tokens=True), self.proj_in.weight, self.proj_in.bias)
        else:
            h = self.proj_in(group_norm_act(self.norm, x)).permute(0, 2, 3, 1).reshape(B, H * W, C).contiguous()
        s32 = _stream32(x, self.proj_out.weight.dtype)
        if s32:
            h = h.float()
        pend = None
        for blk in self.transformer_blocks:
            pend, h = blk(h, context, pend, kv)
        if pend is not None:
            h = pend + h
        if s32:
            h = h.to(self.proj_out.weight.dtype)
        if self.linear_proj:
            if (FUSED_PROJ_OUT_ADD and HIP_LINEAR and FUSED_KERNELS and _fusable_nhwc(x) and _fusable(h) and self.proj_out.weight.dtype == x.dtype == h.dtype
                    and self.proj_out.weight.is_contiguous() and ops.linear_wins(B * H * W, C, C)):
                y = ops.linear(h, self.proj_out.weight, self.proj_out.bias, residual=x.permute(0, 2, 3, 1).reshape(B, H * W, C))
                return y.view(B, H, W, C).permute(0, 3, 1, 2)
            h = linear_(h, self.proj_out.weight, self.proj_out.bias)
            if (FUSED_TOKENS_ADD and _fusable(x) and _fusable(h) and C % 64 == 0 and (H * W) % 64 == 0):
                return ops.tokens_add_nchw(x, h)
            h = h.view(B, H, W, C).permute(0, 3, 1, 2)
        else:
            h = self.proj_out(h.view(B, H, W, C).permute(0, 3, 1, 2))
        return x + h


class Downsample2D(nn.Module):
    def __init__(self, ch, padding=1):
        super().__init__()
        self.padding = padding
        self.conv = nn.Conv2d(ch, ch, 3, stride=2, padding=padding)

    def forward(self, x):
        if _stream32(x, self.conv.weight.dtype):
            return self.forward(x.to(self.conv.weight.dtype)).float()
        if self.padding == 0 and VAE_SPLIT_CONV and VAE_SPLIT_DOWNSAMPLE and FUSED_KERNELS and x.is_cuda and x.dtype == torch.float32 \
                and x.dim() == 4 and self.conv.weight.dtype == torch.float32:
            B, C, H, W = x.shape
            if C % 64 == 0 and ops.conv3x3_f32out_s2_ok(1, H, W, 3 * C, self.conv.weight.shape[0]):
                w, sc = _split_weight(self.conv)

                def conv(xs):
                    am = ops.absmax_f32(xs)
                    return ops.conv3x3_f32out_s2(ops.split_f32(xs, absmax=am), w, self.conv.bias, sc, act_absmax=am)
                return _sliced(x.contiguous(memory_format=torch.channels_last), max(1, (2 ** 31 - 16) // (H * W * 3 * C * 2)), conv)
        if self.padding == 0:
            x = F.pad(_to_nchw(x), (0, 1, 0, 1))
        if HIP_DOWNSAMPLE_CONV and HIP_CONV3X3 and self.padding == 1 and _fusable_nhwc(x) and x.shape[2] % 2 == 0 and x.shape[3] % 2 == 0:
            w = self.conv.weight
            B, C, H, W = x.shape
            if w.dtype == x.dtype and w.is_contiguous(memory_format=torch.channels_last) and ops.conv3x3_s2_wins(B, H // 2, W // 2, C, w.shape[0]):
                return ops.conv3x3_nhwc_s2(x, w, self.conv.bias)
        return self.conv(x)


class Upsample2D(nn.Module):
    def __init__(self, ch, vae=False):
        super().__init__()
        self.conv = nn.Conv2d(ch, ch, 3, padding=1)
        self.vae = vae

    def _split_ok(self, x):
        if not (self.vae and VAE_SPLIT_CONV and FUSED_KERNELS and x.is_cuda and x.dim() == 4 and self.conv.weight.dtype == torch.float32):
            return False
        B, C, H, W = x.shape
        return C % 64 == 0 and 4 * H * W * 3 * C * 2 < 2 ** 31 - 16

    def forward(self, x):
        if _stream32(x, self.conv.weight.dtype):
            return self.forward(x.to(self.conv.weight.dtype)).float()
        if x.dtype == torch.float32:
            if self._split_ok(x):
                w, sc = _split_weight(self.conv)
                B, C, H, W = x.shape

                def conv(xs):
                    am = ops.absmax_f32(xs)
                    return ops.conv3x3_f32out(ops.split_f32(xs, upsample2x=True, absmax=am), w, self.conv.bias, None, sc, act_absmax=am)
                return _sliced(x.contiguous(memory_format=torch.channels_last), max(1, (2 ** 31 - 16) // (4 * H * W * 3 * C * 2)), conv)
            x = _to_nchw(x)
        if FUSED_UPSAMPLE_CONV and HIP_CONV3X3 and _fusable_nhwc(x):
            w = self.conv.weight
            B, C, H, W = x.shape
            if w.dtype == x.dtype and w.is_contiguous(memory_format=torch.channels_last) and ops.conv3x3_up2x_wins(B, 2 * H, 2 * W, C, w.shape[0]):
                return ops.conv3x3_nhwc_up2x(x, w, self.conv.bias)
        up = F.interpolate(x, scale_factor=2.0, mode="nearest")
        if _fusable_nhwc(up) and _hip_conv3x3(self.conv, up, up.shape[1]):
            return ops.conv3x3_nhwc(up, self.conv.weight, self.conv.bias)
        return self.conv(up)


UNET_CONFIGS = {
    "sd15": dict(sample_size=64, in_channels=4, block_out_channels=(320, 640, 1280, 1280), layers_per_block=2,
                 attn=(True, True, True, False), transformer_depth=(1, 1, 1, 1), heads=(8, 8, 8, 8),
                 cross_attention_dim=768, use_linear_projection=False, addition_time_embed_dim=None,
                 pooled_projection_dim=None),
    "sd2": dict(sample_size=64, in_channels=4, block_out_channels=(320, 640, 1280, 1280), layers_per_block=2,
                attn=(True, True, True, False), transformer_depth=(1, 1, 1, 1), heads=(5, 10, 20, 20),
                cross_attention_dim=1024, use_linear_projection=True, addition_time_embed_dim=None,
                pooled_projection_dim=None),
    "sdxl": dict(sample_size=128, in_channels=4, block_out_channels=(320, 640, 1280), layers_per_block=2,
                 attn=(False, True, True), transformer_depth=(1, 2, 10), heads=(5, 10, 20),
                 cross_attention_dim=2048, use_linear_projection=True, addition_time_embed_dim=256,
                 pooled_projection_dim=1280),
}


SMALL_UNET_CONFIGS = {
    "sd15": dict(sample_size=64, in_channels=4, block_out_channels=(64, 128, 256, 256), layers_per_block=2,
                 attn=(True, True, True, False), transformer_depth=(1, 1, 1, 1), heads=(1, 2, 4, 4),
                 cross_attention_dim=64, use_linear_projection=False, addition_time_embed_dim=None,
                 pooled_projection_dim=None),
    "sdxl": dict(sample_size=128, in_channels=4, block_out_channels=(64, 128, 256), layers_per_block=2,
                 attn=(False, True, True), transformer_depth=(1, 1, 2), heads=(1, 2, 4),
                 cross_attention_dim=64, use_linear_projection=True, addition_time_embed_dim=16,
                 pooled_projection_dim=32),
}
SMALL_VAE_CHANNELS = (32, 64, 64, 64)

INPAINT_IN_CHANNELS = 9
INPAINT_SUFFIX = "-inpaint"


def unet_config(fam, small=False, in_channels=4):
    if in_channels not in (4, INPAINT_IN_CHANNELS):
        raise ValueError(f"in_channels must be 4 or {INPAINT_IN_CHANNELS} (an inpainting checkpoint), got {in_channels}")
    table = SMALL_UNET_CONFIGS if small else UNET_CONFIGS
    if fam not in table:
        raise ValueError(f"no {'reduced-width ' if small else ''}architecture for family {fam!r}")
    return dict(table[fam], in_channels=in_channels)


class _DownBlock(nn.Module):
    def __init__(self, cin, cout, temb, layers, attn, heads, depth, cross, linear, downsample):
        super().__init__()
        self.resnets = nn.ModuleList([ResnetBlock2D(cin if i == 0 else cout, cout, temb) for i in range(layers)])
        self.attentions = nn.ModuleList([Transformer2DModel(cout, heads, depth, cross, linear) for _ in range(layers)]) if attn else None
        self.downsamplers = nn.ModuleList([Downsample2D(cout)]) if downsample else None

    def forward(self, x, temb, ctx, kv=None):
        outs = []
        for i, r in enumerate(self.resnets):
            x = r(x, temb)
            if self.attentions is not None:
                x = self.attentions[i](x, ctx, kv)
            outs.append(x)
        if self.downsamplers is not None:
            x = self.downsamplers[0](x)
            outs.append(x)
        return x, outs


class _MidBlock(nn.Module):
    def __init__(self, ch, temb, heads, depth, cross, linear):
        super().__init__()
        self.resnets = nn.ModuleList([ResnetBlock2D(ch, ch, temb), ResnetBlock2D(ch, ch, temb)])
        self.attentions = nn.ModuleList([Transformer2DModel(ch, heads, depth, cross, linear)])

    def forward(self, x, temb, ctx, kv=None):
        return self.resnets[1](self.attentions[0](self.resnets[0](x, temb), ctx, kv), temb)


class _UpBlock(nn.Module):
    def __init__(self, cin, cout, cprev, temb, layers, attn, heads, depth, cross, linear, upsample):
        super().__init__()
        rs = []
        for i in range(layers):
            skip = cin if i == layers - 1 else cout
            rs.append(ResnetBlock2D((cprev if i == 0 else cout) + skip, cout, temb))
        self.resnets = nn.ModuleList(rs)
        self.attentions = nn.ModuleList([Transformer2DModel(cout, heads, depth, cross, linear) for _ in range(layers)]) if attn else None
        self.upsamplers = nn.ModuleList([Upsample2D(cout)]) if upsample else None

    def forward(self, x, skips, temb, ctx, kv=None):
        for i, r in enumerate(self.resnets):
            x = r.forward_cat(x, skips.pop(), temb)
            if self.attentions is not None:
                x = self.attentions[i](x, ctx, kv)
        if self.upsamplers is not None:
            x = self.upsamplers[0](x)
        return x


class ImageProjection(nn.Module):

    def __init__(self, clip_dim, cross_dim, tokens):
        super().__init__()
        self.tokens, self.cross_dim = tokens, cross_dim
        self.proj = nn.Linear(clip_dim, tokens * cross_dim)
        self.norm = nn.LayerNorm(cross_dim)

    def forward(self, embeds):
        return self.norm(self.proj(embeds).reshape(-1, self.tokens, self.cross_dim))


def flatten_ip_adapter_state(state):
    if not isinstance(state, dict):
        raise ValueError(f"IP-Adapter state must be a dict of tensors, got {type(state).__name__}")
    flat = {}
    for key, val in state.items():
        if isinstance(val, dict):
            for sub, t in val.items():
                flat[f"{key}.{sub}"] = t
        else:
            flat[key] = val
    bad = [k for k, t in flat.items() if not isinstance(t, torch.Tensor)]
    if bad:
        raise ValueError(f"IP-Adapter state holds non-tensor entries: {bad[:4]}")
    return flat


class UNet2DConditionModel(nn.Module):
    def __init__(self, sample_size, in_channels, block_out_channels, layers_per_block, attn, transformer_depth, heads,
                 cross_attention_dim, use_linear_projection, addition_time_embed_dim, pooled_projection_dim,
                 out_channels=4):
        super().__init__()
        boc = tuple(block_out_channels)
        temb = boc[0] * 4
        self.config = SimpleNamespace(sample_size=sample_size, in_channels=in_channels, out_channels=out_channels, block_out_channels=boc,
                                      cross_attention_dim=cross_attention_dim,
                                      addition_time_embed_dim=addition_time_embed_dim,
                                      pooled_projection_dim=pooled_projection_dim)
        self.conv_in = nn.Conv2d(in_channels, boc[0], 3, padding=1)
        self.time_embedding = TimestepEmbedding(boc[0], temb)
        if addition_time_embed_dim:
            self.add_embedding = TimestepEmbedding(addition_time_embed_dim * 6 + pooled_projection_dim, temb)
        n = len(boc)
        self.down_blocks = nn.ModuleList()
        ch = boc[0]
        for i in range(n):
            self.down_blocks.append(_DownBlock(ch, boc[i], temb, layers_per_block, attn[i], heads[i], transformer_depth[i],
                                               cross_attention_dim, use_linear_projection, downsample=(i < n - 1)))
            ch = boc[i]
        self.mid_block = _MidBlock(boc[-1], temb, heads[-1], transformer_depth[-1], cross_attention_dim, use_linear_projection)
        self.up_blocks = nn.ModuleList()
        rev, rattn, rheads, rdepth = boc[::-1], attn[::-1], heads[::-1], transformer_depth[::-1]
        prev = rev[0]
        for i in range(n):
            cout, cin = rev[i], rev[min(i + 1, n - 1)]
            self.up_blocks.append(_UpBlock(cin, cout, prev, temb, layers_per_block + 1, rattn[i], rheads[i], rdepth[i],
                                           cross_attention_dim, use_linear_projection, upsample=(i < n - 1)))
            prev = cout
        self.conv_norm_out = nn.GroupNorm(32, boc[0], eps=1e-5)
        self.conv_out = nn.Conv2d(boc[0], out_channels, 3, padding=1)
        self.ip_tokens = 0
        self.ip_image_proj = None

    @property
    def dtype(self):
        return self.conv_in.weight.dtype

    def embed(self, sample, timestep, added_cond_kwargs):
        B = sample.shape[0]
        t = torch.as_tensor(timestep, device=sample.device).reshape(-1).expand(B)
        emb = self.time_embedding(timestep_embedding(t, self.config.block_out_channels[0]).to(sample.dtype))
        if self.config.addition_time_embed_dim:
            ids = added_cond_kwargs["time_ids"]
            tid = timestep_embedding(ids.reshape(-1).float(), self.config.addition_time_embed_dim).reshape(B, -1)
            add = torch.cat([added_cond_kwargs["text_embeds"].to(sample.dtype), tid.to(sample.dtype)], dim=-1)
            emb = emb + self.add_embedding(add)
        return emb

    def cross_attention_kv(self, encoder_hidden_states, into=None):
        ctx = encoder_hidden_states.to(self.dtype)
        out = {} if into is None else into
        for m in self.modules():
            if isinstance(m, BasicTransformerBlock):
                out[id(m.attn2)] = m.attn2.project_kv(ctx, None if into is None else into[id(m.attn2)])
        return out

    def ip_attentions(self):
        out = []
        for blk in list(self.down_blocks) + list(self.up_blocks) + [self.mid_block]:
            for tr in (blk.attentions or ()):
                out.extend(tb.attn2 for tb in tr.transformer_blocks)
        return out

    @torch.no_grad()
    def install_ip_adapter(self, state):
        flat = flatten_ip_adapter_state(state)
        if any(k.startswith("image_proj.latents") or k.startswith("image_proj.layers.") or k.startswith("image_proj.proj_in")
               for k in flat):
            raise ValueError("this is an IP-Adapter 'Plus' / FaceID file (Resampler keys such as image_proj.latents): only the base "
                             "adapters' ImageProjection (image_proj.proj / image_proj.norm) is supported")
        attns = self.ip_attentions()
        cross = self.config.cross_attention_dim
        proj_w = flat.get("image_proj.proj.weight")
        if proj_w is None or proj_w.dim() != 2:
            raise ValueError("IP-Adapter: image_proj.proj.weight is missing or not a matrix")
        if proj_w.shape[0] % cross or not 1 <= proj_w.shape[0] // cross <= ops.IP_MAX_IMAGE_KEYS:
            raise ValueError(f"IP-Adapter: image_proj.proj has {proj_w.shape[0]} output features: not 1..{ops.IP_MAX_IMAGE_KEYS} "
                             f"image tokens of cross-attention width {cross}")
        ni, clip_dim = proj_w.shape[0] // cross, proj_w.shape[1]
        expected = {"image_proj.proj.weight": (ni * cross, clip_dim), "image_proj.proj.bias": (ni * cross,),
                    "image_proj.norm.weight": (cross,), "image_proj.norm.bias": (cross,)}
        for n, a in enumerate(attns):
            for name in ("to_k_ip", "to_v_ip"):
                expected[f"ip_adapter.{2 * n + 1}.{name}.weight"] = (a.to_k.out_features, cross)
        missing = sorted(set(expected) - set(flat))
        surplus = sorted(set(flat) - set(expected))
        wrong = sorted(k for k in expected if k in flat and tuple(flat[k].shape) != expected[k])
        if missing or surplus or wrong:
            raise ValueError(f"IP-Adapter does not fit this UNet ({len(attns)} cross attentions, width {cross}): "
                             f"missing {missing[:4]}, unexpected {surplus[:4]}, "
                             f"wrong shape {[(k, tuple(flat[k].shape), expected[k]) for k in wrong[:4]]}; nothing installed")
        like = self.conv_in.weight

        def linear(w, b=None):
            m = nn.Linear(w.shape[1], w.shape[0], bias=b is not None, device=like.device, dtype=like.dtype)
            m.weight.copy_(w)
            if b is not None:
                m.bias.copy_(b)
            return m.requires_grad_(False)
        self.remove_ip_adapter()
        proj = ImageProjection(clip_dim, cross, ni).to(device=like.device, dtype=like.dtype).requires_grad_(False)
        proj.proj.weight.copy_(flat["image_proj.proj.weight"]), proj.proj.bias.copy_(flat["image_proj.proj.bias"])
        proj.norm.weight.copy_(flat["image_proj.norm.weight"]), proj.norm.bias.copy_(flat["image_proj.norm.bias"])
        self.ip_image_proj = proj
        for n, a in enumerate(attns):
            a.set_ip_adapter(linear(flat[f"ip_adapter.{2 * n + 1}.to_k_ip.weight"]),
                             linear(flat[f"ip_adapter.{2 * n + 1}.to_v_ip.weight"]), ni)
        self.ip_tokens = ni
        return ni

    def remove_ip_adapter(self):
        for a in self.ip_attentions():
            a.set_ip_adapter()
        if isinstance(self.ip_image_proj, nn.Module):
            del self.ip_image_proj
        self.ip_image_proj = None
        self.ip_tokens = 0

    @property
    def ip_scale(self):
        a = self.ip_attentions()
        return a[0].ip_scale if a else 1.0

    @ip_scale.setter
    def ip_scale(self, scale):
        scale = float(scale)
        if not math.isfinite(scale):
            raise ValueError(f"IP-Adapter scale must be finite, got {scale}")
        for a in self.ip_attentions():
            a.ip_scale = scale

    @torch.no_grad()
    def ip_image_tokens(self, clip_embeds):
        if self.ip_image_proj is None:
            raise ValueError("no IP-Adapter is installed")
        p = self.ip_image_proj.proj.weight
        return self.ip_image_proj(clip_embeds.to(device=p.device, dtype=p.dtype))

    def forward(self, sample, timestep, encoder_hidden_states=None, added_cond_kwargs=None,
                down_block_additional_residuals=None, mid_block_additional_residual=None, cross_kv=None, **_):
        x = sample.to(self.dtype)
        if CHANNELS_LAST and x.is_cuda and x.dtype != torch.float32:
            x = x.contiguous(memory_format=torch.channels_last)
        ctx = encoder_hidden_states.to(self.dtype)
        if self.ip_tokens and ctx.shape[1] <= self.ip_tokens:
            raise ValueError(f"an IP-Adapter with {self.ip_tokens} image tokens is installed: the context must be [text tokens | image "
                             f"tokens], got {ctx.shape[1]} tokens in all")
        emb = self.embed(x, timestep, added_cond_kwargs)
        x = self.conv_in(x)
        if getattr(self, "residual_fp32", False) and x.dtype != torch.float32:
            x = x.float()
        skips = [x]
        for blk in self.down_blocks:
            x, outs = blk(x, emb, ctx, cross_kv)
            skips.extend(outs)
        if down_block_additional_residuals is not None:
            skips = [s + r for s, r in zip(skips, down_block_additional_residuals)]
        x = self.mid_block(x, emb, ctx, cross_kv)
        if mid_block_additional_residual is not None:
            x = x + mid_block_additional_residual
        for blk in self.up_blocks:
            x = blk(x, skips, emb, ctx, cross_kv)
        x = self.conv_out(group_norm_act(self.conv_norm_out, x, silu=True))
        return ModelOutput(sample=x)


class _CondEmbedding(nn.Module):
    def __init__(self, out_ch, chans=(16, 32, 96, 256)):
# ... 284 lines not shown
```

### elasticdiffusion_official_amd/ops.py

```python
import torch

from . import _hip

ED_F32, ED_F16, ED_BF16 = 0, 1, 2
_DTYPE = {torch.float32: ED_F32, torch.float16: ED_F16, torch.bfloat16: ED_BF16}


_LAUNCH = {"device": None}


def _stream_of(t):
    if _LAUNCH["device"] is None:
        _LAUNCH["device"] = t.device
    return _stream()


def _stream():
    dev = _LAUNCH["device"]
    if dev is None:
        raise RuntimeError("internal: _stream() before any device tensor argument")
    return torch.cuda.current_stream(dev).cuda_stream


class KernelTimer:
# ... 558 lines not shown
def linear_wins(M, K, N):
    ncb = -(-N // (2 * GEMM_BN))
    if linear_ok(M, K, N) and K <= 1280 and gemm_rows_mode(M, ncb):
        return -(-M // (GEMM_BM // 2)) * ncb >= GEMM_ROWS_MIN_BLOCKS_LINEAR
    blocks = -(-M // GEMM_BM) * ncb
    if K > 1280 and blocks < 200:
        return False
    return linear_ok(M, K, N) and (K <= 640 or N <= 640) and _gemm_grid_ok(blocks)


def linear(x, w, bias=None, residual=None):
    M, K = _gemm_x(x, "x")
    N = w.shape[0]
    if tuple(w.shape) != (N, K) or not linear_ok(M, K, N):
        _reject(f"linear: unsupported shape x {tuple(x.shape)} w {tuple(w.shape)}")
    out = torch.empty(x.shape[:-1] + (N,), dtype=x.dtype, device=x.device)
    if residual is not None and (residual.shape != out.shape or residual.dtype != x.dtype):
        _reject("linear: residual must match the output")
    TIMER.note_work("ed_linear", flops=2.0 * M * K * N, nbytes=2.0 * (M * K + N * K + M * N * (2 if residual is not None else 1)))
    _call("ed_linear", _dev(x, None, "x"), _dev(w, x.dtype, "w"), _opt(bias, x.dtype, "bias"), _opt(residual, x.dtype, "residual"),
          _dev(out, None, "out"), _code(x, "x"), M, K, N, _stream())
    return out


def conv3x3_ok(B, H, W, Cin, N):
    M = B * H * W
    return Cin % 64 == 0 and N % 8 == 0 and M * Cin * 2 < 2 ** 31 - 16 and N * 9 * Cin * 2 < 2 ** 31 - 16


def conv3x3_wins(B, H, W, Cin, N):
    ncb = -(-N // (2 * GEMM_BN))
    return conv3x3_ok(B, H, W, Cin, N) and _gemm_grid_ok(-(-(B * H * W) // GEMM_BM) * ncb, B * H * W, ncb, min_fill=0.5)


def conv3x3_nhwc(x, w, bias=None, sample_bias=None, residual=None):
    if not (isinstance(x, torch.Tensor) and x.is_cuda and x.dim() == 4 and x.dtype in (torch.float16, torch.bfloat16)):
        _reject("conv3x3_nhwc: x must be a 16-bit [B,C,H,W] tensor on the MI355X; no CPU fallback")
    B, Cin, H, W = x.shape
    N = w.shape[0]
    cl = torch.channels_last
    if tuple(w.shape) != (N, Cin, 3, 3) or w.dtype != x.dtype or not conv3x3_ok(B, H, W, Cin, N):
        _reject(f"conv3x3_nhwc: unsupported shape x {tuple(x.shape)} w {tuple(w.shape)}")
    if not x.is_contiguous(memory_format=cl) or not w.is_contiguous(memory_format=cl):
        _reject("conv3x3_nhwc: x and w must be channels_last")
    out = torch.empty((B, N, H, W), dtype=x.dtype, device=x.device, memory_format=cl)
    if residual is not None and (residual.shape != out.shape or residual.dtype != x.dtype or not residual.is_contiguous(memory_format=cl)):
        _reject("conv3x3_nhwc: residual must be a channels_last tensor of the output's shape")
    if sample_bias is not None and tuple(sample_bias.shape) != (B, N):
        _reject("conv3x3_nhwc: sample_bias must be [B, N]")
    TIMER.note_work("ed_conv3x3_nhwc", flops=2.0 * B * H * W * 9 * Cin * N,
                    nbytes=2.0 * (B * H * W * (Cin + N * (2 if residual is not None else 1)) + 9 * Cin * N))
    BA = conv3x3_batch_split(B, H, W, N) if CONV_BATCH_SPLIT else None
    for b0, nb in (((0, B),) if BA is None else ((0, BA), (BA, B - BA))):
        px, po = b0 * H * W * Cin * x.element_size(), b0 * H * W * N * x.element_size()
        _call("ed_conv3x3_nhwc", x.data_ptr() + px, w.data_ptr(), _opt(bias, x.dtype, "bias"),
              None if sample_bias is None else _dev(sample_bias, x.dtype, "sample_bias") + b0 * N * x.element_size(),
              None if residual is None else residual.data_ptr() + po, out.data_ptr() + po, _code(x, "x"), nb, H, W, Cin, N, _stream_of(x))
    return out


CONV_BATCH_SPLIT = True


def conv3x3_batch_split(B, H, W, N):
    HW = H * W
    if HW % GEMM_BM or B < 2:
        return None
    ncb = -(-N // (2 * GEMM_BN))
    tps = HW // GEMM_BM * ncb
    total = B * tps

    def rounds(tiles):
        return min(-(-tiles // GEMM_CUS), -(-2 * tiles // GEMM_CUS) * GEMM_ROWS_TILE_COST)

    full = total // GEMM_CUS
    if full < 3 or total % GEMM_CUS == 0:
        return None
    BA = full * GEMM_CUS // tps
    if BA <= 0 or BA >= B:
        return None
    return BA if -(-BA * tps // GEMM_CUS) + rounds((B - BA) * tps) < rounds(total) - 0.1 else None


def conv3x3_up2x_wins(B, H, W, Cin, N):
    ncb = -(-N // (2 * GEMM_BN))
    return (H % 2 == 0 and W % 2 == 0 and conv3x3_wins(B, H, W, Cin, N) and not gemm_rows_mode(B * H * W, ncb)
            and B * (H // 2) * (W // 2) * Cin * 2 < 2 ** 31 - 16)


def conv3x3_nhwc_up2x(x, w, bias=None):
    if not (isinstance(x, torch.Tensor) and x.is_cuda and x.dim() == 4 and x.dtype in (torch.float16, torch.bfloat16)):
        _reject("conv3x3_nhwc_up2x: x must be a 16-bit [B,C,H,W] tensor on the MI355X; no CPU fallback")
    B, Cin, Hs, Ws = x.shape
    H, W = 2 * Hs, 2 * Ws
    N = w.shape[0]
    cl = torch.channels_last
    if tuple(w.shape) != (N, Cin, 3, 3) or w.dtype != x.dtype or not conv3x3_ok(B, H, W, Cin, N):
        _reject(f"conv3x3_nhwc_up2x: unsupported shape x {tuple(x.shape)} w {tuple(w.shape)}")
    if not x.is_contiguous(memory_format=cl) or not w.is_contiguous(memory_format=cl):
        _reject("conv3x3_nhwc_up2x: x and w must be channels_last")
    out = torch.empty((B, N, H, W), dtype=x.dtype, device=x.device, memory_format=cl)
    TIMER.note_work("ed_conv3x3_nhwc_up2x", flops=2.0 * B * H * W * 9 * Cin * N, nbytes=2.0 * (B * Hs * Ws * Cin + B * H * W * N + 9 * Cin * N))
    _call("ed_conv3x3_nhwc_up2x", x.data_ptr(), w.data_ptr(), _opt(bias, x.dtype, "bias"), out.data_ptr(), _code(x, "x"), B, H, W, Cin, N,
          _stream_of(x))
    return out


def conv3x3_s2_wins(B, H, W, Cin, N):
    ncb = -(-N // (2 * GEMM_BN))
    return (conv3x3_wins(B, H, W, Cin, N) and not gemm_rows_mode(B * H * W, ncb) and 4 * B * H * W * Cin * 2 < 2 ** 31 - 16)


def conv3x3_nhwc_s2(x, w, bias=None):
    if not (isinstance(x, torch.Tensor) and x.is_cuda and x.dim() == 4 and x.dtype in (torch.float16, torch.bfloat16)):
        _reject("conv3x3_nhwc_s2: x must be a 16-bit [B,C,H,W] tensor on the MI355X; no CPU fallback")
    B, Cin, Hi, Wi = x.shape
    if Hi % 2 or Wi % 2:
        _reject("conv3x3_nhwc_s2: even input height and width")
    H, W = Hi // 2, Wi // 2
    N = w.shape[0]
    cl = torch.channels_last
    if tuple(w.shape) != (N, Cin, 3, 3) or w.dtype != x.dtype or not conv3x3_ok(B, Hi, Wi, Cin, N):
        _reject(f"conv3x3_nhwc_s2: unsupported shape x {tuple(x.shape)} w {tuple(w.shape)}")
    if not x.is_contiguous(memory_format=cl) or not w.is_contiguous(memory_format=cl):
        _reject("conv3x3_nhwc_s2: x and w must be channels_last")
    out = torch.empty((B, N, H, W), dtype=x.dtype, device=x.device, memory_format=cl)
    TIMER.note_work("ed_conv3x3_nhwc_s2", flops=2.0 * B * H * W * 9 * Cin * N, nbytes=2.0 * (B * Hi * Wi * Cin + B * H * W * N + 9 * Cin * N))
    _call("ed_conv3x3_nhwc_s2", x.data_ptr(), w.data_ptr(), _opt(bias, x.dtype, "bias"), out.data_ptr(), _code(x, "x"), B, H, W, Cin, N,
          _stream_of(x))
    return out


GROUPNORM_SPLIT = True


def groupnorm(x, gamma, beta, groups, eps, silu=False, tokens=False, chan_bias=None, conv_bias=None):
    N, C, H, W = x.shape
    if chan_bias is not None:
        assert tuple(chan_bias.shape) == (N, C)
    if conv_bias is not None:
        assert tuple(conv_bias.shape) == (C,)
    out = torch.empty((N, H * W, C) if tokens else (N, C, H, W), dtype=x.dtype, device=x.device)
    TIMER.note_work("ed_groupnorm", nbytes=3.0 * x.numel() * x.element_size())
    ws = None
    if GROUPNORM_SPLIT:
        nbytes = _hip.lib().ed_groupnorm_workspace(N, C, H * W, groups)
        ws = torch.empty(nbytes // 4, dtype=torch.float32, device=x.device) if nbytes else None
    _call("ed_groupnorm", _dev(x, None, "x"), _dev(gamma, x.dtype, "gamma"), _dev(beta, x.dtype, "beta"),
          _opt(conv_bias, x.dtype, "conv_bias"), _opt(chan_bias, x.dtype, "chan_bias"), _dev(out, None, "out"),
          _opt(ws, torch.float32, "workspace"), _code(x, "x"), N, C, H * W, groups, float(eps),
          int(silu), int(tokens), _stream())
    return out


def groupnorm_nhwc(x, gamma, beta, groups, eps, silu=False, chan_bias=None, conv_bias=None):
    N, C, H, W = x.shape
    if not x.is_cuda:
        _reject("x must be a tensor on the MI355X; no CPU fallback")
    if not x.is_contiguous(memory_format=torch.channels_last):
        _reject("x must be channels_last")
    out = torch.empty_like(x, memory_format=torch.channels_last)
    nbytes = _hip.lib().ed_groupnorm_nhwc_workspace(N, C, H * W, groups)
    ws = torch.empty(nbytes // 4, dtype=torch.float32, device=x.device)
    TIMER.note_work("ed_groupnorm_nhwc", nbytes=3.0 * x.numel() * x.element_size())
    _call("ed_groupnorm_nhwc", x.data_ptr(), _dev(gamma, x.dtype, "gamma"), _dev(beta, x.dtype, "beta"),
          _opt(conv_bias, x.dtype, "conv_bias"), _opt(chan_bias, x.dtype, "chan_bias"), out.data_ptr(),
          _dev(ws, torch.float32, "workspace"), _code(x, "x"), N, C, H * W, groups, float(eps), int(silu), _stream())
    return out


def groupnorm_nhwc_cat_ok(x1, x2, groups):
    def cl16(x):
        return isinstance(x, torch.Tensor) and x.is_cuda and x.dtype in (torch.float16, torch.bfloat16) and is_nhwc(x)
    if not (cl16(x1) and cl16(x2) and x1.dtype == x2.dtype and x1.device == x2.device and x1.shape[0] == x2.shape[0]
            and x1.shape[2:] == x2.shape[2:]):
        return False
    C1, C = x1.shape[1], x1.shape[1] + x2.shape[1]
    return C1 % 8 == 0 and C % 8 == 0 and C % groups == 0 and C // groups >= 8 and groups <= 256 and C <= 4096


def groupnorm_nhwc_cat(x1, x2, gamma, beta, groups, eps, silu=False):
    if not groupnorm_nhwc_cat_ok(x1, x2, groups):
        _reject("groupnorm_nhwc_cat: two channels_last 16-bit tensors of the same dtype / batch / size on the MI355X, C1 % 8 == 0, "
                "(C1 + C2) / groups >= 8; no CPU fallback")
    N, C1, H, W = x1.shape
    C2 = x2.shape[1]
    out = torch.empty((N, C1 + C2, H, W), dtype=x1.dtype, device=x1.device, memory_format=torch.channels_last)
    nbytes = _hip.lib().ed_groupnorm_nhwc_workspace(N, C1 + C2, H * W, groups)
    ws = torch.empty(nbytes // 4, dtype=torch.float32, device=x1.device)
    TIMER.note_work("ed_groupnorm_nhwc_cat", nbytes=3.0 * out.numel() * out.element_size())
    _LAUNCH["device"] = x1.device
    _call("ed_groupnorm_nhwc_cat", x1.data_ptr(), x2.data_ptr(), _dev(gamma, x1.dtype, "gamma"), _dev(beta, x1.dtype, "beta"),
          out.data_ptr(), ws.data_ptr(), _DTYPE[x1.dtype], N, C1, C2, H * W, groups, float(eps), int(silu), _stream())
    return out


def layernorm(x, gamma, beta, eps):
    D = x.shape[-1]
    out = torch.empty_like(x)
    TIMER.note_work("ed_layernorm", nbytes=2.0 * x.numel() * x.element_size())
    _call("ed_layernorm", _dev(x, None, "x"), _dev(gamma, x.dtype, "gamma"), _dev(beta, x.dtype, "beta"),
          _dev(out, None, "out"), _code(x, "x"), x.numel() // D, D, float(eps), _stream())
    return out


def add_layernorm(a, b, gamma, beta, eps):
    D = a.shape[-1]
    assert a.shape == b.shape and a.dtype == b.dtype
    s, out = torch.empty_like(a), torch.empty_like(a)
    TIMER.note_work("ed_add_layernorm", nbytes=4.0 * a.numel() * a.element_size())
    _call("ed_add_layernorm", _dev(a, None, "a"), _dev(b, a.dtype, "b"), _dev(gamma, a.dtype, "gamma"),
          _dev(beta, a.dtype, "beta"), _dev(s, None, "sum"), _dev(out, None, "out"), _code(a, "a"), a.numel() // D, D,
          float(eps), _stream())
    return s, out


def _stream_ok(x, w):
    return (isinstance(x, torch.Tensor) and x.is_cuda and x.dtype == torch.float32 and w.dtype in (torch.float16, torch.bfloat16)
            and w.device == x.device)


def layernorm_s32(x, gamma, beta, eps):
    if not _stream_ok(x, gamma) or not x.is_contiguous():
        _reject("layernorm_s32: x must be a contiguous fp32 tensor on the MI355X and gamma 16-bit; no CPU fallback")
    D = x.shape[-1]
    out = torch.empty(x.shape, dtype=gamma.dtype, device=x.device)
    TIMER.note_work("ed_layernorm_s32", nbytes=x.numel() * 6.0)
    _LAUNCH["device"] = x.device
    _call("ed_layernorm_s32", x.data_ptr(), _dev(gamma, None, "gamma"), _dev(beta, gamma.dtype, "beta"), out.data_ptr(),
          _DTYPE[gamma.dtype], x.numel() // D, D, float(eps), _stream())
    return out


def add_layernorm_s32(a, b, gamma, beta, eps):
    if not (_stream_ok(b, a) and a.shape == b.shape and a.is_contiguous() and b.is_contiguous() and gamma.dtype == a.dtype):
        _reject("add_layernorm_s32: a must be 16-bit and b fp32, same shape, contiguous, on the MI355X; no CPU fallback")
    D = a.shape[-1]
    s, out = torch.empty_like(b), torch.empty_like(a)
    TIMER.note_work("ed_add_layernorm_s32", nbytes=a.numel() * 12.0)
    _LAUNCH["device"] = a.device
    _call("ed_add_layernorm_s32", a.data_ptr(), b.data_ptr(), _dev(gamma, None, "gamma"), _dev(beta, a.dtype, "beta"), s.data_ptr(),
          out.data_ptr(), _DTYPE[a.dtype], a.numel() // D, D, float(eps), _stream())
    return s, out


def groupnorm_nhwc_s32(x, gamma, beta, groups, eps, silu=False):
    if not _stream_ok(x, gamma) or x.dim() != 4 or not x.is_contiguous(memory_format=torch.channels_last):
        _reject("groupnorm_nhwc_s32: x must be an fp32 channels_last [N,C,H,W] tensor on the MI355X and gamma 16-bit; no CPU fallback")
    N, C, H, W = x.shape
    out = torch.empty((N, C, H, W), dtype=gamma.dtype, device=x.device, memory_format=torch.channels_last)
    nbytes = _hip.lib().ed_groupnorm_nhwc_workspace(N, C, H * W, groups)
    ws = torch.empty(max(4, nbytes // 4), dtype=torch.float32, device=x.device)
    TIMER.note_work("ed_groupnorm_nhwc_s32", nbytes=x.numel() * 10.0)
    _LAUNCH["device"] = x.device
    _call("ed_groupnorm_nhwc_s32", x.data_ptr(), _dev(gamma, None, "gamma"), _dev(beta, gamma.dtype, "beta"), out.data_ptr(),
          ws.data_ptr(), _DTYPE[gamma.dtype], N, C, H * W, groups, float(eps), int(silu), _stream())
    return out


def bias_residual_add(h, h_bias, res, res_bias=None):
    N, C, H, W = h.shape
    assert res.shape == h.shape and res.dtype == h.dtype
    if not (h.is_cuda and res.is_cuda):
        _reject("bias_residual_add: h and res must be tensors on the MI355X; no CPU fallback")
    cl = is_nhwc(h) and C % 8 == 0
    fmt = torch.channels_last if cl else torch.contiguous_format
    h = h.contiguous(memory_format=fmt)
    res = res.contiguous(memory_format=fmt)
    out = torch.empty_like(h, memory_format=fmt)
    TIMER.note_work("ed_bias_residual_add", nbytes=3.0 * h.numel() * h.element_size())
    _call("ed_bias_residual_add", h.data_ptr(), _opt(h_bias, h.dtype, "h_bias"), res.data_ptr(),
          _opt(res_bias, h.dtype, "res_bias"), out.data_ptr(), _code(h, "h"), N, C, H * W, int(cl), _stream_of(h))
    return out


def tokens_add_nchw(x, tokens):
    N, C, H, W = x.shape
    assert tuple(tokens.shape) == (N, H * W, C) and tokens.dtype == x.dtype
    out = torch.empty_like(x)
    TIMER.note_work("ed_tokens_add_nchw", nbytes=3.0 * x.numel() * x.element_size())
    _call("ed_tokens_add_nchw", _dev(x, None, "x"), _dev(tokens, None, "tokens"), _dev(out, None, "out"), _code(x, "x"),
          N, C, H * W, _stream())
    return out


def groupnorm_f32(x, gamma, beta, groups, eps, silu=False):
    N, C, H, W = x.shape
    if (H * W) % 4:
        _reject("groupnorm_f32: H*W must be a multiple of 4")
    out = torch.empty_like(x)
    nbytes = _hip.lib().ed_groupnorm_f32_workspace(N, C, H * W, groups)
    ws = torch.empty(max(1, nbytes // 4), dtype=torch.float32, device=x.device)
    TIMER.note_work("ed_groupnorm_f32", nbytes=3.0 * x.numel() * 4)
    _call("ed_groupnorm_f32", _dev(x, torch.float32, "x"), _dev(gamma, torch.float32, "gamma"), _dev(beta, torch.float32, "beta"),
          _dev(out, torch.float32, "out"), _dev(ws, torch.float32, "workspace"), N, C, H * W, groups, float(eps), int(silu),
          _stream())
    return out


def groupnorm_nhwc_f32_ok(C, groups):
    return C % groups == 0 and (C // groups) % 4 == 0 and groups <= 256 and C <= 4096


def groupnorm_nhwc_f32(x, gamma, beta, groups, eps, silu=False, split=False):
    if not (isinstance(x, torch.Tensor) and x.is_cuda and x.dim() == 4 and x.dtype == torch.float32):
        _reject("groupnorm_nhwc_f32: x must be an fp32 [N,C,H,W] tensor on the MI355X; no CPU fallback")
    N, C, H, W = x.shape
    cl = torch.channels_last
    if not x.is_contiguous(memory_format=cl):
        _reject("groupnorm_nhwc_f32: x must be channels_last")
    if not groupnorm_nhwc_f32_ok(C, groups):
        _reject(f"groupnorm_nhwc_f32: unsupported C = {C}, groups = {groups}")
    out = (torch.empty((N, 3 * C, H, W), dtype=torch.float16, device=x.device, memory_format=cl) if split
           else torch.empty_like(x, memory_format=cl))
    nbytes = _hip.lib().ed_groupnorm_nhwc_f32_workspace(N, C, H * W, groups)
    ws = torch.empty(max(4, nbytes // 4), dtype=torch.float32, device=x.device)
    TIMER.note_work("ed_groupnorm_nhwc_f32", nbytes=x.numel() * (4.0 + 4.0 + (6.0 if split else 4.0)))
    _call("ed_groupnorm_nhwc_f32", x.data_ptr(), _dev(gamma, torch.float32, "gamma"), _dev(beta, torch.float32, "beta"), out.data_ptr(),
          _dev(ws, torch.float32, "workspace"), N, C, H * W, groups, float(eps), int(silu), int(split), _stream_of(x))
    return out


def absmax_f32(x):
    if not (isinstance(x, torch.Tensor) and x.is_cuda and x.dtype == torch.float32):
        _reject("absmax_f32: x must be an fp32 tensor on the MI355X; no CPU fallback")
    if not (x.is_contiguous() or (x.dim() == 4 and x.is_contiguous(memory_format=torch.channels_last))):
        _reject("absmax_f32: x must be dense (contiguous or channels_last)")
    out = torch.empty(1, dtype=torch.float32, device=x.device)
    TIMER.note_work("ed_absmax_f32", nbytes=x.numel() * 4.0)
    _LAUNCH["device"] = x.device
    _call("ed_absmax_f32", x.data_ptr(), x.numel(), out.data_ptr(), _stream())
    return out


def split_f32(x, upsample2x=False, absmax=None):
    if not (isinstance(x, torch.Tensor) and x.is_cuda and x.dim() == 4 and x.dtype == torch.float32):
        _reject("split_f32: x must be an fp32 [N,C,H,W] tensor on the MI355X; no CPU fallback")
    if absmax is not None and not (isinstance(absmax, torch.Tensor) and absmax.device == x.device and absmax.dtype == torch.float32
                                   and absmax.numel() == 1):
        _reject("split_f32: absmax must be a 1-element fp32 tensor on x's device")
    N, C, H, W = x.shape
    cl = torch.channels_last
    if not x.is_contiguous(memory_format=cl) or C % 4:
        _reject("split_f32: x must be channels_last with C % 4 == 0")
    u = 2 if upsample2x else 1
    out = torch.empty((N, 3 * C, u * H, u * W), dtype=torch.float16, device=x.device, memory_format=cl)
    TIMER.note_work("ed_split_f32_nhwc", nbytes=x.numel() * (4.0 + 6.0 * u * u))
    _LAUNCH["device"] = x.device
    _call("ed_split_f32_nhwc", x.data_ptr(), out.data_ptr(), N, C, H, W, int(bool(upsample2x)),
          None if absmax is None else absmax.data_ptr(), _stream())
    return out


def split_conv_weight(w):
    import math
    wmax = float(w.detach().abs().max())
    k = 0 if not (wmax > 0.0 and math.isfinite(wmax)) else max(-24, min(24, 13 - math.frexp(wmax)[1] + 1))
    ws = w.detach().float() * (2.0 ** k)
    hi = ws.half()
    lo = (ws - hi.float()).half()
    return torch.cat([hi, hi, lo], dim=1).contiguous(memory_format=torch.channels_last), 2.0 ** -k


def conv3x3_f32out_ok(B, H, W, Cin3, N):
    M = B * H * W
    return Cin3 % 64 == 0 and N % 8 == 0 and M * Cin3 * 2 < 2 ** 31 - 16 and N * 9 * Cin3 * 2 < 2 ** 31 - 16 and M < 2 ** 31


def conv3x3_f32out(a, w, bias=None, residual=None, out_scale=1.0, act_absmax=None):
    if not (isinstance(a, torch.Tensor) and a.is_cuda and a.dim() == 4 and a.dtype == torch.float16):
        _reject("conv3x3_f32out: a must be an fp16 [B,C,H,W] tensor on the MI355X; no CPU fallback")
    B, C3, H, W = a.shape
    N = w.shape[0]
    cl = torch.channels_last
    if tuple(w.shape) != (N, C3, 3, 3) or w.dtype != torch.float16 or not conv3x3_f32out_ok(B, H, W, C3, N):
        _reject(f"conv3x3_f32out: unsupported shape a {tuple(a.shape)} w {tuple(w.shape)}")
    if not a.is_contiguous(memory_format=cl) or not w.is_contiguous(memory_format=cl):
        _reject("conv3x3_f32out: a and w must be channels_last")
    out = torch.empty((B, N, H, W), dtype=torch.float32, device=a.device, memory_format=cl)
    if residual is not None and (residual.shape != out.shape or residual.dtype != torch.float32 or not residual.is_contiguous(memory_format=cl)):
        _reject("conv3x3_f32out: residual must be an fp32 channels_last tensor of the output's shape")
    TIMER.note_work("ed_conv3x3_nhwc_f32out", flops=2.0 * B * H * W * 9 * C3 * N,
                    nbytes=2.0 * (B * H * W * C3 + 9 * C3 * N) + 4.0 * B * H * W * N * (2 if residual is not None else 1))
    _call("ed_conv3x3_nhwc_f32out", a.data_ptr(), w.data_ptr(), _opt(bias, torch.float32, "bias"),
          None if residual is None else residual.data_ptr(), out.data_ptr(), _DTYPE[torch.float16], B, H, W, C3, N, float(out_scale),
          None if act_absmax is None else act_absmax.data_ptr(), _stream_of(a))
    return out


def conv3x3_f32out_s2_ok(B, Hi, Wi, Cin3, N):
    return (Hi % 2 == 0 and Wi % 2 == 0 and Cin3 % 64 == 0 and N % 8 == 0 and B * Hi * Wi * Cin3 * 2 < 2 ** 31 - 16
            and N * 9 * Cin3 * 2 < 2 ** 31 - 16)


def conv3x3_f32out_s2(a, w, bias=None, out_scale=1.0, act_absmax=None):
    if not (isinstance(a, torch.Tensor) and a.is_cuda and a.dim() == 4 and a.dtype == torch.float16):
        _reject("conv3x3_f32out_s2: a must be an fp16 [B,C,H,W] tensor on the MI355X; no CPU fallback")
    B, C3, Hi, Wi = a.shape
    N = w.shape[0]
    cl = torch.channels_last
    if tuple(w.shape) != (N, C3, 3, 3) or w.dtype != torch.float16 or not conv3x3_f32out_s2_ok(B, Hi, Wi, C3, N):
        _reject(f"conv3x3_f32out_s2: unsupported shape a {tuple(a.shape)} w {tuple(w.shape)}")
    if not a.is_contiguous(memory_format=cl) or not w.is_contiguous(memory_format=cl):
        _reject("conv3x3_f32out_s2: a and w must be channels_last")
    H, W = Hi // 2, Wi // 2
    out = torch.empty((B, N, H, W), dtype=torch.float32, device=a.device, memory_format=cl)
    TIMER.note_work("ed_conv3x3_nhwc_f32out_s2", flops=2.0 * B * H * W * 9 * C3 * N, nbytes=2.0 * (B * Hi * Wi * C3 + 9 * C3 * N) + 4.0 * B * H * W * N)
    _call("ed_conv3x3_nhwc_f32out_s2", a.data_ptr(), w.data_ptr(), _opt(bias, torch.float32, "bias"), out.data_ptr(), _DTYPE[torch.float16],
          B, H, W, C3, N, float(out_scale), None if act_absmax is None else act_absmax.data_ptr(), _stream_of(a))
    return out


def softmax_rows_(x, scale=1.0):
    cols = x.shape[-1]
    if cols % 4 and x.numel() != cols:
        _reject("softmax_rows_: cols must be a multiple of 4")
    TIMER.note_work("ed_softmax_rows", nbytes=3.0 * x.numel() * 4)
    _call("ed_softmax_rows", _dev(x, torch.float32, "x"), x.numel() // cols, cols, float(scale), _stream())
    return x


VAE_ATTENTION_CHUNK_BYTES = 1 << 30


def vae_attention(q, k, v):
    B, N, C = q.shape
    scale = C ** -0.5
    rows = max(64, min(N, VAE_ATTENTION_CHUNK_BYTES // (4 * N * B) // 64 * 64)) if N > 256 else N
    kt = k.transpose(1, 2)
    if rows >= N:
        return torch.bmm(softmax_rows_(torch.bmm(q, kt), scale), v)
    out = torch.empty_like(q)
    for a in range(0, N, rows):
        s = torch.bmm(q[:, a:a + rows], kt)
        out[:, a:a + rows] = torch.bmm(softmax_rows_(s, scale), v)
    return out


FLASH_V_PATH = None
FLASH_HEAD_DIMS = (40, 64, 80, 160)
FLASH_EXP2 = False
_ENV_VARIANT = __import__("os").environ.get("ED_FLASH_VARIANT")
LOG2E = 1.4426950408889634


def _pipe_fits(Nk, row_stride):
    return Nk >= 128 and (Nk + 128) * row_stride * 2 < 2 ** 31


def flash_prescale(Nq, Nk, row_stride, scale=0.125):
    if FLASH_V_PATH is not None:
        want = int(FLASH_V_PATH)
    elif _ENV_VARIANT is not None:
        want = -1 if _ENV_VARIANT == "legacy" else int(_ENV_VARIANT)
    else:
        want = 6 if FLASH_EXP2 else -1
    return scale * LOG2E if (want == 6 and _pipe_fits(Nk, row_stride)) else None


def _flash_variant(B, heads, Nq, Nk, k=None, v=None, prescaled=False):
    fits = k is None or _pipe_fits(Nk, max(k.stride(1), v.stride(1)))
    if prescaled:
        if not (Nk >= 128 and fits):
            _reject("flash_attention: exponent-domain q needs the pipelined kernel (Nk >= 128, 32-bit K / V offsets)")
        return 6
    if FLASH_V_PATH is not None and int(FLASH_V_PATH) != 6:
        return int(FLASH_V_PATH)
    legacy = 2 if (Nq >= 2048 and Nk >= 1024 and B * heads * (Nq // 256) >= 1024) else 0
    if _ENV_VARIANT == "legacy":
        return legacy
    if _ENV_VARIANT is not None and int(_ENV_VARIANT) != 6:
        want = int(_ENV_VARIANT)
        if want in (4, 5, 7, 9, 10):
            return want if (Nk >= 128 and fits) else (8 if Nk <= 96 else legacy)
        return want if (want != 8 or Nk <= SMALLKV_MAX_KEYS) else legacy
    if Nk <= 96 or _stream_two_chunks(Nq, Nk):
        return 8
    if Nk >= 128 and fits:
        return FLASH_DEFAULT_PIPE
    return legacy


SMALLKV_MAX_KEYS = 160


def _stream_two_chunks(Nq, Nk):
    return 128 <= Nk <= SMALLKV_MAX_KEYS and Nq >= 4096


FLASH_DEFAULT_PIPE = 5


def flash_attention(q, k, v, heads, v_path=None, prescaled=False):
    B, Nq, HD = q.shape
    Nk = k.shape[1]
    hd = HD // heads
    if HD != heads * hd or hd not in FLASH_HEAD_DIMS or k.shape != (B, Nk, HD) or v.shape != (B, Nk, HD):
        _reject(f"flash_attention: head_dim must be one of {FLASH_HEAD_DIMS} and shapes consistent (q {tuple(q.shape)}, "
                f"k {tuple(k.shape)}, v {tuple(v.shape)}, heads {heads})")
    if hd != 64 and (prescaled or v_path is not None):
        _reject("flash_attention: kernel variants exist for head_dim 64 only")
    for t, name in ((q, "q"), (k, "k"), (v, "v")):
        if not t.is_cuda or t.dtype != q.dtype or t.stride(2) != 1:
            _reject(f"flash_attention: {name} must be a 16-bit tensor on the MI355X with unit last stride; no CPU fallback")
        if _LAUNCH["device"] is None:
            _LAUNCH["device"] = t.device
        elif _LAUNCH["device"] != t.device:
            _reject(f"flash_attention: {name} lives on {t.device}, q on {_LAUNCH['device']}")
    if v_path is not None and (int(v_path) == 6) != bool(prescaled):
        _reject("flash_attention: v_path 6 takes exponent-domain q (prescaled=True) and nothing else does")
    out = torch.empty(B, Nq, HD, dtype=q.dtype, device=q.device)
    TIMER.note_work("ed_flash_attention", flops=4.0 * B * heads * Nq * Nk * hd,
                    nbytes=2.0 * q.element_size() * HD * B * (Nq + Nk))
    variant = 0 if hd != 64 else (_flash_variant(B, heads, Nq, Nk, k, v, prescaled) if v_path is None else int(v_path))
    _call("ed_flash_attention", q.data_ptr(), k.data_ptr(), v.data_ptr(), out.data_ptr(), _code(q, "q"), B, heads, Nq, Nk,
          hd, q.stride(0), q.stride(1), k.stride(0), k.stride(1), v.stride(0), v.stride(1), out.stride(0), out.stride(1),
          hd ** -0.5, variant, _stream())
    return out


IP_MAX_TEXT_KEYS = SMALLKV_MAX_KEYS
IP_MAX_IMAGE_KEYS = 32


def flash_attention_ip_ok(head_dim, n_text, n_image):
    return head_dim == 64 and 1 <= n_text <= IP_MAX_TEXT_KEYS and 1 <= n_image <= IP_MAX_IMAGE_KEYS


def flash_attention_ip(q, k, v, heads, n_text, ip_scale):
    B, Nq, HD = q.shape
    N = k.shape[1]
    hd = HD // heads
    n_text, ip_scale = int(n_text), float(ip_scale)
    if HD != heads * hd or hd != 64 or k.shape != (B, N, HD) or v.shape != (B, N, HD):
        _reject(f"flash_attention_ip: head_dim must be 64 and shapes consistent (q {tuple(q.shape)}, k {tuple(k.shape)}, "
                f"v {tuple(v.shape)}, heads {heads})")
    if not flash_attention_ip_ok(hd, n_text, N - n_text):
        _reject(f"flash_attention_ip: needs 1 <= text keys <= {IP_MAX_TEXT_KEYS} and 1 <= image keys <= {IP_MAX_IMAGE_KEYS}, "
                f"got {n_text} and {N - n_text}")
    if ip_scale != ip_scale or ip_scale in (float("inf"), float("-inf")):
        _reject(f"flash_attention_ip: ip_scale must be finite, got {ip_scale}")
    for t, name in ((q, "q"), (k, "k"), (v, "v")):
        if not t.is_cuda or t.dtype != q.dtype or t.dtype not in (torch.float16, torch.bfloat16) or t.stride(2) != 1:
            _reject(f"flash_attention_ip: {name} must be a 16-bit tensor on the MI355X with unit last stride; no CPU fallback")
        if _LAUNCH["device"] is None:
            _LAUNCH["device"] = t.device
        elif _LAUNCH["device"] != t.device:
            _reject(f"flash_attention_ip: {name} lives on {t.device}, q on {_LAUNCH['device']}")
    out = torch.empty(B, Nq, HD, dtype=q.dtype, device=q.device)
    TIMER.note_work("ed_flash_attention_ip", flops=4.0 * B * heads * Nq * N * hd,
                    nbytes=2.0 * q.element_size() * HD * B * (Nq + N))
    _call("ed_flash_attention_ip", q.data_ptr(), k.data_ptr(), v.data_ptr(), out.data_ptr(), _code(q, "q"), B, heads, Nq, n_text,
          N - n_text, hd, q.stride(0), q.stride(1), k.stride(0), k.stride(1), v.stride(0), v.stride(1), out.stride(0), out.stride(1),
          hd ** -0.5, ip_scale, _stream())
    return out


CANNY_MAX_DIM = 8192


def _canny_dims(t, name, channels):
    if t.dim() == 2 and 1 in channels:
        H, W, C = t.shape[0], t.shape[1], 1
    elif t.dim() == 3 and t.shape[2] in channels:
        H, W, C = t.shape
    else:
        _reject(f"{name} must be uint8 [H,W,C] with C in {sorted(channels)}{' or [H,W]' if 1 in channels else ''}, got {tuple(t.shape)}")
    if not (1 <= H <= CANNY_MAX_DIM and 1 <= W <= CANNY_MAX_DIM):
        _reject(f"{name}: H and W must be in 1..{CANNY_MAX_DIM}, got {H} x {W}")
    return H, W, C


def _canny_threshold(v, name):
    import math
    if not math.isfinite(v):
        _reject(f"canny: {name} threshold must be finite, got {v}")
    return max(-2 ** 31, min(2 ** 31 - 1, int(math.floor(v))))


def canny_map(img, low=100, high=200):
    p_img = _dev(img, torch.uint8, "img")
    H, W, C = _canny_dims(img, "img", (1, 3))
    lo, hi = _canny_threshold(low, "low"), _canny_threshold(high, "high")
    cmap = torch.empty((H, W), dtype=torch.uint8, device=img.device)
    TIMER.note_work("ed_canny_map", nbytes=float(H * W * (C + 1)))
    _call("ed_canny_map", p_img, H, W, C, lo, hi, _dev(cmap, torch.uint8, "map"), _stream())
    return cmap


def canny_hysteresis(cmap):
    import ctypes
    p_map = _dev(cmap, torch.uint8, "map")
    H, W, _ = _canny_dims(cmap, "map", (1,))
    if cmap.dim() != 2:
        _reject(f"map must be [H,W], got {tuple(cmap.shape)}")
    if torch.cuda.is_current_stream_capturing():
        _reject("canny_hysteresis reads a device flag between passes and cannot be captured into a graph")
    ws = torch.empty(_hip.lib().ed_canny_workspace(H, W, 1) // 4, dtype=torch.int32, device=cmap.device)
    passes = ctypes.c_int32(0)
    TIMER.note_work("ed_canny_hysteresis", nbytes=float(H * W))
    _call("ed_canny_hysteresis", p_map, H, W, _dev(ws, torch.int32, "workspace"), ctypes.addressof(passes), _stream())
    return cmap, int(passes.value)


def canny_edges(cmap, out="u8"):
    if out not in ("u8", "cond"):
        raise ValueError(f"out must be 'u8' or 'cond', got {out!r}")
    p_map = _dev(cmap, torch.uint8, "map")
    H, W, _ = _canny_dims(cmap, "map", (1,))
    if cmap.dim() != 2:
        _reject(f"map must be [H,W], got {tuple(cmap.shape)}")
    if out == "u8":
        res = torch.empty((H, W, 3), dtype=torch.uint8, device=cmap.device)
        TIMER.note_work("ed_canny_edges", nbytes=float(4 * H * W))
        _call("ed_canny_edges", p_map, H, W, _dev(res, torch.uint8, "edges"), None, _stream())
    else:
        res = torch.empty((1, 3, H, W), dtype=torch.float32, device=cmap.device)
        TIMER.note_work("ed_canny_edges", nbytes=float(13 * H * W))
        _call("ed_canny_edges", p_map, H, W, None, _dev(res, torch.float32, "cond"), _stream())
    return res


def canny(img, low=100, high=200, out="u8"):
    if out not in ("u8", "cond"):
        raise ValueError(f"out must be 'u8' or 'cond', got {out!r}")
    cmap, _ = canny_hysteresis(canny_map(img, low, high))
    return canny_edges(cmap, out)


RESIZE_MAX_DIM = 8192
_RESIZE_TABLES = {}


def _resize_tables(device, key, make):
    hit = _RESIZE_TABLES.get((device, key))
    if hit is None:
        if len(_RESIZE_TABLES) >= 64:
            _RESIZE_TABLES.clear()
        coeff, bounds = make()
        hit = (torch.from_numpy(coeff.copy()).to(device), torch.from_numpy(bounds.copy()).to(device))
        _RESIZE_TABLES[(device, key)] = hit
    return hit


def _identity_tables(n):
    import numpy as np
    from . import resample
    coeff = np.full((n, 1), 1 << resample.PRECISION_BITS, np.int32)
    bounds = np.stack([np.arange(n, dtype=np.int32), np.ones(n, np.int32)], axis=1)
    return coeff, bounds


def resize_u8(img, size, filter="bicubic", out="u8"):
    from . import resample
    if out not in ("u8", "cond"):
        raise ValueError(f"out must be 'u8' or 'cond', got {out!r}")
    if filter not in resample.FILTERS:
        raise ValueError(f"filter must be one of {sorted(resample.FILTERS)}, got {filter!r}")
    p_img = _dev(img, torch.uint8, "img")
    H, W, C = _canny_dims(img, "img", (1, 3))
    try:
        Ho, Wo = (int(v) for v in size)
    except (TypeError, ValueError):
        _reject(f"size must be (H_out, W_out), got {size!r}")
    if not (1 <= Ho <= RESIZE_MAX_DIM and 1 <= Wo <= RESIZE_MAX_DIM):
        _reject(f"size: H_out and W_out must be in 1..{RESIZE_MAX_DIM}, got {Ho} x {Wo}")
    dev = img.device
    if (Ho, Wo) == (H, W) and out == "u8":
        _LAUNCH["device"] = None
        return img.clone()
    passes = resample.plan((H, W), (Ho, Wo), filter)
    src, rows, pitch = p_img, H, W * C
    mid = None
    if passes and passes[0][0] == "rows":
        _, kh, _, y0, y1 = passes[0]
        coeff, bounds = _resize_tables(dev, (W, Wo, filter), lambda: resample.coefficients(W, Wo, filter))
        rows, mid_pitch = y1 - y0, (Wo * C + 3) // 4 * 4
        mid = torch.empty((rows, mid_pitch), dtype=torch.uint8, device=dev)
        TIMER.note_work("ed_resize_rows_u8", flops=2.0 * rows * Wo * C * kh.shape[1], nbytes=float(rows * (W * C + mid_pitch)))
        _call("ed_resize_rows_u8", p_img + y0 * pitch, rows, W, C, pitch, _dev(coeff, torch.int32, "coeff"),
              _dev(bounds, torch.int32, "bounds"), kh.shape[1], Wo, _dev(mid, torch.uint8, "intermediate"), mid_pitch, _stream())
        src, pitch = _dev(mid, torch.uint8, "intermediate"), mid_pitch
    if passes and passes[-1][0] == "cols":
        _, kv, bv = passes[-1]
        shift = int(bv[0, 0]) if len(passes) == 2 else None
        coeff, bounds = _resize_tables(dev, (H, Ho, filter, shift), lambda: (kv, bv))
        ksz = kv.shape[1]
    else:
        coeff, bounds = _resize_tables(dev, (Ho, "identity"), lambda: _identity_tables(Ho))
        ksz = 1
    if out == "u8":
        res = torch.empty((Ho, Wo) if img.dim() == 2 else (Ho, Wo, C), dtype=torch.uint8, device=dev)
        p_u8, p_cond = _dev(res, torch.uint8, "out"), None
    else:
        res = torch.empty((1, 3, Ho, Wo), dtype=torch.float32, device=dev)
        p_u8, p_cond = None, _dev(res, torch.float32, "out")
    TIMER.note_work("ed_resize_cols_u8", flops=2.0 * Ho * Wo * C * ksz,
                    nbytes=float(rows * Wo * C + Ho * Wo * (C if out == "u8" else 12)))
    _call("ed_resize_cols_u8", src, rows, Wo * C, pitch, _dev(coeff, torch.int32, "coeff"), _dev(bounds, torch.int32, "bounds"),
          ksz, Ho, C, p_u8, p_cond, _stream())
    return res


VAE_INPUT_MAX_DIM = 8192


def u8_to_vae_input(img, dtype=torch.float32):
    p_img = _dev(img, torch.uint8, "img")
    if img.dim() != 3 or img.shape[2] != 3:
        _reject(f"img must be uint8 [H,W,3], got {tuple(img.shape)}")
    H, W = int(img.shape[0]), int(img.shape[1])
# ... 279 lines not shown
```

### include/elastic_hip.h

```cpp
#ifndef ELASTIC_HIP_H
#define ELASTIC_HIP_H

#include <stdint.h>

#ifdef __cplusplus
extern "C" {
#endif

enum { ED_F32 = 0, ED_F16 = 1, ED_BF16 = 2 };

enum { ED_PRED_EPSILON = 0, ED_PRED_V = 1 };

int ed_version(void);

const char* ed_error_string(int err);

int ed_gather_views(const float* latent, void* out, int dtype, int B, int C, int H, int W,
                    const int32_t* win_y0, const int32_t* win_x0, int V, int Sh, int Sw,
                    int PH, int PW, int off_y, int off_x, const float* frame, float divisor, void* stream);

int ed_scatter_centres(const void* pred, int dtype, float* local, int B, int C, int H, int W,
                       int PH, int PW, int n_col_blocks,
                       const int32_t* row_blk, const int32_t* row_src,
                       const int32_t* col_blk, const int32_t* col_src, void* stream);

int ed_pick_assemble(const float* latent, const uint8_t* idx, const int32_t* src_row, const int32_t* src_col,
                     const float* frame, void* out, int dtype, float* low,
                     int K, int B, int C, int H, int W, int h, int w, int PH, int PW, int off_y, int off_x,
                     void* stream);

int ed_unpad_direction(const void* unet_out, int dtype, float* dirs, float* uncond_last,
                       int K, int B, int C, int h, int w, int PH, int PW, int off_y, int off_x, void* stream);

int ed_fill_directions(const float* dirs, const int8_t* stamp,
                       const int32_t* inv_row, const int32_t* inv_col,
                       const int32_t* up_row, const int32_t* up_col,
                       const int32_t* down_row, const int32_t* down_col,
                       float* target, float* low_dir,
                       int K, int B, int C, int H, int W, int h, int w, void* stream);

int ed_cfg_ddim_step(const float* local, const float* direction, const float* x, float* prev, float* x0,
                     float g, float sqrt_beta_t, float sqrt_alpha_t, float sqrt_alpha_prev,
                     float sqrt_one_minus_alpha_prev, int64_t n, void* stream);

int ed_cfg_ddim_step_pt(const float* local, const float* direction, const float* x, float* prev, float* x0,
                        float g, float sqrt_beta_t, float sqrt_alpha_t, float sqrt_alpha_prev,
                        float sqrt_one_minus_alpha_prev, int64_t n, int prediction_type, void* stream);

int ed_undo_step(const float* x_in, const float* noise, const float* coef, float* x_out,
                 int n_sub, int64_t n, void* stream);

int ed_rrg_update(const float* prev, const float* x0, const float* low_latent, const float* low_uncond,
                  const float* low_dir, const int32_t* up_row, const int32_t* up_col, float* out,
                  float g, float sqrt_beta_t, float sqrt_alpha_t, float norm, float weight,
                  int B, int C, int H, int W, int h, int w, void* stream);

int ed_rrg_update_pt(const float* prev, const float* x0, const float* low_latent, const float* low_uncond,
                     const float* low_dir, const int32_t* up_row, const int32_t* up_col, float* out,
                     float g, float sqrt_beta_t, float sqrt_alpha_t, float norm, float weight,
                     int B, int C, int H, int W, int h, int w, int prediction_type, void* stream);

int ed_gather2d(const void* in, int in_dtype, void* out, int out_dtype, int C, int H, int W,
                const int32_t* src_n, const int32_t* rows, const int32_t* cols, int N, int oh, int ow, void* stream);

int ed_tile_gather_pad(const float* latent, void* tiles, int dtype, int B, int C, int H, int W,
                       const int32_t* tile_y0, const int32_t* tile_x0, int T, int Ts, float scaling_factor,
                       void* stream);

#define ED_TILE_MAXC 4
int ed_tile_accumulate_normalise(const void* decoded, int dtype, float* image, int B, int Cimg, int HP, int WP,
                                 int TP, int n_col_tiles,
                                 const int32_t* row_tile, const int32_t* row_src,
                                 const int32_t* col_tile, const int32_t* col_src, void* stream);


int ed_geglu(const void* in, void* out, int dtype, int64_t M, int I, void* stream);

int ed_groupnorm(const void* x, const void* gamma, const void* beta, const void* conv_bias, const void* chan_bias,
                 void* out, float* workspace, int dtype, int N, int C, int HW, int G, float eps, int act_silu,
                 int tokens_out, void* stream);
int64_t ed_groupnorm_workspace(int N, int C, int HW, int G);

int ed_bias_residual_add(const void* h, const void* h_bias, const void* res, const void* res_bias, void* out, int dtype,
                         int N, int C, int HW, int channels_last, void* stream);

int ed_layernorm(const void* x, const void* gamma, const void* beta, void* out, int dtype, int64_t M, int D, float eps,
                 void* stream);
int ed_layernorm_s32(const void* x, const void* gamma, const void* beta, void* out, int dtype, int64_t M, int D, float eps,
                     void* stream);
int ed_add_layernorm_s32(const void* a, const void* b, const void* gamma, const void* beta, void* sum_out, void* out,
                         int dtype, int64_t M, int D, float eps, void* stream);
int ed_groupnorm_nhwc_s32(const void* x, const void* gamma, const void* beta, void* out, float* workspace, int dtype, int N, int C,
                          int HW, int G, float eps, int act_silu, void* stream);

int ed_add_layernorm(const void* a, const void* b, const void* gamma, const void* beta, void* sum_out, void* out,
                     int dtype, int64_t M, int D, float eps, void* stream);

int ed_tokens_add_nchw(const void* x, const void* tokens, void* out, int dtype, int N, int C, int HW, void* stream);

int ed_groupnorm_nhwc(const void* x, const void* gamma, const void* beta, const void* conv_bias, const void* chan_bias,
                      void* out, float* workspace, int dtype, int N, int C, int HW, int G, float eps, int act_silu,
                      void* stream);
int64_t ed_groupnorm_nhwc_workspace(int N, int C, int HW, int G);

int ed_groupnorm_nhwc_cat(const void* x1, const void* x2, const void* gamma, const void* beta, void* out, float* workspace, int dtype,
                          int N, int C1, int C2, int HW, int G, float eps, int act_silu, void* stream);

int ed_assemble_rows(const float* latent, int B, int C, int H, int W, const uint8_t* idx, const int32_t* src_row,
                     const int32_t* src_col, const float* gframe, void* g_rows, float* low, int K, int h, int w, int gPH,
                     int gPW, int g_off_y, int g_off_x, const int32_t* win_y0, const int32_t* win_x0,
                     const float* vframe, void* v_rows, int V, int Sh, int Sw, int vPH, int vPW, int v_off_y, int v_off_x,
                     int dtype, void* stream);

int ed_assemble_rows_x(const float* latent, int B, int C, int H, int W, const uint8_t* idx, const int32_t* src_row,
                       const int32_t* src_col, const float* gframe, void* g_rows, float* low, int K, int h, int w, int gPH,
                       int gPW, int g_off_y, int g_off_x, const int32_t* win_y0, const int32_t* win_x0,
                       const float* vframe, void* v_rows, int V, int Sh, int Sw, int vPH, int vPW, int v_off_y, int v_off_x,
                       int dtype, const float* extra, int E, const float* pad_value, void* stream);

int ed_phase_epilogue(const void* g_out, const void* v_out, int dtype, const float* x, const int8_t* stamp,
                      const int32_t* inv_row, const int32_t* inv_col, const int32_t* up_row, const int32_t* up_col,
                      const int32_t* down_row, const int32_t* down_col, const int32_t* row_blk, const int32_t* row_src,
                      const int32_t* col_blk, const int32_t* col_src, const float* low_latent, float* prev, float* x0,
                      float* x_next, float* low_dir, float* uncond_last, float* direction, float* local, int K, int B,
                      int C, int H, int W, int h, int w, int gPH, int gPW, int g_off_y, int g_off_x, int vPH, int vPW,
                      int n_col_blocks, float g, float sqrt_beta_t, float sqrt_alpha_t, float sqrt_alpha_prev,
                      float sqrt_1m_alpha_prev, float rrg_norm, float rrg_weight, void* stream);

int ed_phase_epilogue_pt(const void* g_out, const void* v_out, int dtype, const float* x, const int8_t* stamp,
                         const int32_t* inv_row, const int32_t* inv_col, const int32_t* up_row, const int32_t* up_col,
                         const int32_t* down_row, const int32_t* down_col, const int32_t* row_blk, const int32_t* row_src,
                         const int32_t* col_blk, const int32_t* col_src, const float* low_latent, float* prev, float* x0,
                         float* x_next, float* low_dir, float* uncond_last, float* direction, float* local, int K, int B,
                         int C, int H, int W, int h, int w, int gPH, int gPW, int g_off_y, int g_off_x, int vPH, int vPW,
                         int n_col_blocks, float g, float sqrt_beta_t, float sqrt_alpha_t, float sqrt_alpha_prev,
                         float sqrt_1m_alpha_prev, float rrg_norm, float rrg_weight, int prediction_type, void* stream);

int64_t ed_guidance_moments_workspace(int B, int64_t n_full, int64_t n_low);

int ed_guidance_moments(const float* local, const float* direction, const float* text, float g, int B, int64_t n,
                        float* ratio, void* workspace, void* stream);

int ed_phase_moments(const void* g_out, const void* v_out, int dtype, const int8_t* stamp, const int32_t* inv_row,
                     const int32_t* inv_col, const int32_t* up_row, const int32_t* up_col, const int32_t* down_row,
                     const int32_t* down_col, const int32_t* row_blk, const int32_t* row_src, const int32_t* col_blk,
                     const int32_t* col_src, float* ratio, float* ratio_low, void* workspace, int K, int B, int C, int H,
                     int W, int h, int w, int gPH, int gPW, int g_off_y, int g_off_x, int vPH, int vPW, int n_col_blocks,
                     float g, void* stream);

int ed_cfg_ddim_step_gr(const float* local, const float* direction, const float* x, float* prev, float* x0,
                        float g, float sqrt_beta_t, float sqrt_alpha_t, float sqrt_alpha_prev,
                        float sqrt_one_minus_alpha_prev, int64_t n, int prediction_type, const float* ratio, float gr,
                        float omgr, int B, void* stream);
int ed_cfg_ddim_step_width(const float* local, const float* direction, const float* x, const float* prev, const float* x0,
                           int64_t n, const float* ratio, int B);
int ed_rrg_update_gr(const float* prev, const float* x0, const float* low_latent, const float* low_uncond,
                     const float* low_dir, const int32_t* up_row, const int32_t* up_col, float* out,
                     float g, float sqrt_beta_t, float sqrt_alpha_t, float norm, float weight,
                     int B, int C, int H, int W, int h, int w, int prediction_type, const float* ratio_low, float gr,
                     float omgr, void* stream);
int ed_phase_epilogue_gr(const void* g_out, const void* v_out, int dtype, const float* x, const int8_t* stamp,
                         const int32_t* inv_row, const int32_t* inv_col, const int32_t* up_row, const int32_t* up_col,
                         const int32_t* down_row, const int32_t* down_col, const int32_t* row_blk, const int32_t* row_src,
                         const int32_t* col_blk, const int32_t* col_src, const float* low_latent, float* prev, float* x0,
                         float* x_next, float* low_dir, float* uncond_last, float* direction, float* local, int K, int B,
                         int C, int H, int W, int h, int w, int gPH, int gPW, int g_off_y, int g_off_x, int vPH, int vPW,
                         int n_col_blocks, float g, float sqrt_beta_t, float sqrt_alpha_t, float sqrt_alpha_prev,
                         float sqrt_1m_alpha_prev, float rrg_norm, float rrg_weight, int prediction_type,
                         const float* ratio, const float* ratio_low, float gr, float omgr, void* stream);

int ed_cfg_ddim_step_ms(const float* local, const float* direction, const float* x, float* prev, float* x0,
                        float g, float sqrt_beta_t, float sqrt_alpha_t, float c_x, float b, float half_b, float r_inv,
                        int64_t n, int prediction_type, const float* ratio, float gr, float omgr, int B,
                        const float* x0_hist, void* stream);
int ed_phase_epilogue_ms(const void* g_out, const void* v_out, int dtype, const float* x, const int8_t* stamp,
                         const int32_t* inv_row, const int32_t* inv_col, const int32_t* up_row, const int32_t* up_col,
                         const int32_t* down_row, const int32_t* down_col, const int32_t* row_blk, const int32_t* row_src,
                         const int32_t* col_blk, const int32_t* col_src, const float* low_latent, float* prev, float* x0,
                         float* x_next, float* low_dir, float* uncond_last, float* direction, float* local, int K, int B,
                         int C, int H, int W, int h, int w, int gPH, int gPW, int g_off_y, int g_off_x, int vPH, int vPW,
                         int n_col_blocks, float g, float sqrt_beta_t, float sqrt_alpha_t, float c_x, float b, float half_b,
                         float r_inv, float rrg_norm, float rrg_weight, int prediction_type, const float* ratio,
                         const float* ratio_low, float gr, float omgr, const float* x0_hist, void* stream);

int ed_flash_attention(const void* q, const void* k, const void* v, void* out, int dtype, int B, int H, int Nq, int Nk,
                       int head_dim, int64_t q_sb, int64_t q_sn, int64_t k_sb, int64_t k_sn, int64_t v_sb, int64_t v_sn,
                       int64_t o_sb, int64_t o_sn, float scale, int v_path, void* stream);

int ed_flash_attention_ip(const void* q, const void* k, const void* v, void* out, int dtype, int B, int H, int Nq, int Nt, int Ni,
                          int head_dim, int64_t q_sb, int64_t q_sn, int64_t k_sb, int64_t k_sn, int64_t v_sb, int64_t v_sn,
                          int64_t o_sb, int64_t o_sn, float scale, float ip_scale, void* stream);

int64_t ed_groupnorm_f32_workspace(int N, int C, int HW, int G);
int ed_groupnorm_f32(const void* x, const void* gamma, const void* beta, void* out, float* workspace, int N, int C, int HW,
                     int G, float eps, int act_silu, void* stream);

int ed_softmax_rows(void* x, int64_t rows, int64_t cols, float scale, void* stream);

int ed_geglu_gemm(const void* x, const void* w, const void* bias, void* out, int dtype, int64_t M, int K, int I, void* stream);

int ed_linear(const void* x, const void* w, const void* bias, const void* residual, void* out, int dtype, int64_t M, int K, int N,
              void* stream);

int ed_conv3x3_nhwc(const void* x, const void* w, const void* bias, const void* sample_bias, const void* residual, void* out,
                    int dtype, int B, int H, int W, int Cin, int N, void* stream);

int ed_conv3x3_nhwc_up2x(const void* x, const void* w, const void* bias, void* out, int dtype, int B, int H, int W, int Cin, int N,
                         void* stream);

int ed_conv3x3_nhwc_s2(const void* x, const void* w, const void* bias, void* out, int dtype, int B, int H, int W, int Cin, int N,
                       void* stream);

int ed_absmax_f32(const void* x, int64_t n, float* out, void* stream);
int ed_split_f32_nhwc(const void* x, void* out, int N, int C, int H, int W, int upsample2x, const float* absmax, void* stream);
int64_t ed_groupnorm_nhwc_f32_workspace(int N, int C, int HW, int G);
int ed_groupnorm_nhwc_f32(const void* x, const void* gamma, const void* beta, void* out, float* workspace, int N, int C, int HW, int G,
                          float eps, int act_silu, int split16, void* stream);
int ed_conv3x3_nhwc_f32out(const void* x, const void* w, const float* bias, const float* residual, float* out, int dtype, int B, int H, int W,
                           int Cin, int N, float out_scale, const float* act_absmax, void* stream);

int ed_conv3x3_nhwc_f32out_s2(const void* x, const void* w, const float* bias, float* out, int dtype, int B, int H, int W, int Cin, int N,
                              float out_scale, const float* act_absmax, void* stream);

int64_t ed_canny_workspace(int H, int W, int C);
int ed_canny_map(const uint8_t* img, int H, int W, int C, int low, int high, uint8_t* map, void* stream);
int ed_canny_hysteresis(uint8_t* map, int H, int W, void* workspace, int32_t* passes_out, void* stream);
int ed_canny_edges(const uint8_t* map, int H, int W, uint8_t* edges, float* cond, void* stream);

int ed_resize_rows_u8(const uint8_t* src, int H, int W, int C, int src_pitch, const int32_t* coeff, const int32_t* bounds, int ksize,
                      int W_out, uint8_t* dst, int dst_pitch, void* stream);
int ed_resize_cols_u8(const uint8_t* src, int H, int WC_bytes, int src_pitch, const int32_t* coeff, const int32_t* bounds, int ksize,
                      int H_out, int C, uint8_t* dst_u8, float* dst_cond, void* stream);

int ed_u8_to_vae_input(const uint8_t* img, int H, int W, void* out, int dtype, void* stream);
int ed_u8_to_clip_input(const uint8_t* img, int H, int W, int y0, int x0, int S, float* out, float mean0, float mean1, float mean2,
                        float std0, float std1, float std2, void* stream);
int ed_img2img_init(const void* mean, const void* std, int dtype, const float* eps, const float* noise, float sf, float a,
                    float b, float* z0, float* x, int64_t n, void* stream);
int ed_mask_to_latent(const uint8_t* src, int H, int W, int scale, int threshold, uint8_t* mask, int Hl, int Wl, void* stream);
int ed_inpaint_blend(const float* x, const uint8_t* mask, const float* z0, const float* noise, float a, float b, int clean,
                     float* out, int planes, int64_t HW, void* stream);

int ed_u8_to_vae_input_masked(const uint8_t* img, const uint8_t* mask, int threshold, int H, int W, void* out, int dtype,
                              void* stream);

int ed_box_blur3_rows_u8(const uint8_t* src, int H, int W, int r, int ww, int fw, uint8_t* dst, void* stream);
int ed_box_blur3_cols_u8(const uint8_t* src, int H, int W, int r, int ww, int fw, uint8_t* dst, void* stream);
int ed_box_blur3_cols_strip(int H, int W);
int ed_mask_levels_to_latent(const uint8_t* src, int H, int W, int scale, uint8_t* level, int Hl, int Wl, void* stream);
int ed_inpaint_blend_level(const float* x, const uint8_t* level, int thr, const float* z0, const float* noise, float a, float b,
                           int clean, float* out, int planes, int64_t HW, void* stream);
int ed_composite_u8(const float* decoded, const uint8_t* init, const uint8_t* mask, uint8_t* out, int H, int W, void* stream);
int ed_canvas_pad_u8(const uint8_t* img, int H, int W, int left, int top, int right, int bottom, uint8_t* canvas, uint8_t* mask,
                     void* stream);

enum { ED_LORA_TENSOR_WORDS = 8, ED_LORA_ADAPTER_WORDS = 4, ED_LORA_TILE_N = 64, ED_LORA_TILE_K = 128 };
int ed_lora_merge(const int64_t* table_host, const int64_t* table_dev, int n_tensors, int n_adapters, int64_t n_tiles,
                  void* stream);

#ifdef __cplusplus
}
#endif
#endif
```

Baseline: 0.1021.

## Store VAE split activations as two segments and wrap conv K index

```diff
diff --git a/elasticdiffusion_official_amd/csrc/gemm_kernels.hip b/elasticdiffusion_official_amd/csrc/gemm_kernels.hip
--- a/elasticdiffusion_official_amd/csrc/gemm_kernels.hip
+++ b/elasticdiffusion_official_amd/csrc/gemm_kernels.hip
@@ -96,6 +96,7 @@
   int x_voff[2], w_voff[2];
   int px_mask[2];
   int img_w, cin2, cpt;
+  int a_wrap;
   int wave;
   int xrd, wrd;
 };
@@ -104,10 +105,10 @@
 constexpr int CONV_S2 = 3;
 constexpr int CONV_S2P0 = 4;
 struct KPos {
-  int tile, tap, ct, w;
+  int tile, tap, ct, w, xc;
 };
-template <int CONV>
-__device__ __forceinline__ KPos k_next(KPos p, int cpt) {
+template <int CONV, bool WRAP = false>
+__device__ __forceinline__ KPos k_next(KPos p, int cpt, int wrap) {
   ++p.tile;
   if (CONV) {
     ++p.tap;
@@ -117,6 +118,7 @@
       ++p.ct;
       p.w = p.ct;
     }
+    p.xc = WRAP && p.ct >= wrap ? p.ct - wrap : p.ct;
   } else {
     p.w = p.tile;
   }
@@ -132,9 +134,9 @@
     int delta;
     if (CONV == CONV_UP2X) {
       const int yp = (c.px_mask[h] >> 16) & 1, xp = (c.px_mask[h] >> 17) & 1;
-      delta = (((yp + dy) >> 1) * c.img_w + ((xp + dx) >> 1)) * c.cin2 + p.ct * (BK * 2);
+      delta = (((yp + dy) >> 1) * c.img_w + ((xp + dx) >> 1)) * c.cin2 + p.xc * (BK * 2);
     } else {
-      delta = (dy * c.img_w + dx) * c.cin2 + p.ct * (BK * 2);
+      delta = (dy * c.img_w + dx) * c.cin2 + p.xc * (BK * 2);
     }
     const int vo = ((c.px_mask[h] >> p.tap) & 1) ? c.x_voff[h] + delta : (int)0x80000000;
     __builtin_amdgcn_raw_ptr_buffer_load_lds(c.xr, (lds_ptr_t)dst, 16, vo, 0, 0, 0);
@@ -317,7 +319,7 @@
 k_gemm_8phase(const uint16_t* __restrict__ x, const uint16_t* __restrict__ w, const uint16_t* __restrict__ bias,
               const uint16_t* __restrict__ row_bias, const uint16_t* __restrict__ residual, uint16_t* __restrict__ out, int M,
               int K, int I, int n_blocks_n, int n_blocks, int img_h, int img_w, int rows_per_sample, float out_scale,
-              const float* __restrict__ act_absmax) {
+              const float* __restrict__ act_absmax, int a2seg) {
   __shared__ __attribute__((aligned(1024))) uint8_t lds[2 * BUF];
 
   const int bid = blockIdx.x;
@@ -340,7 +342,8 @@
 
   const int ps = swz(16 * lane), srow = ps >> 6, skb = ps & 63;
   const int row_bytes = K * 2;
-  const int x_row_bytes = CONV ? row_bytes / 9 : row_bytes;
+  const bool wrap = CONV && OUT32 && a2seg;
+  const int x_row_bytes = CONV ? (wrap ? row_bytes / 27 * 2 : row_bytes / 9) : row_bytes;
   c.xr = __builtin_amdgcn_make_buffer_rsrc((void*)x, 0, (int)((int64_t)(CONV == CONV_UP2X ? M / 4 : CONV >= CONV_S2 ? 4 * (int64_t)M : M) * x_row_bytes),
                                            0x00020000);
   c.wr_ = __builtin_amdgcn_make_buffer_rsrc((void*)w, 0, (int)((int64_t)(EPI == 0 ? 2 : 1) * I * row_bytes), 0x00020000);
@@ -350,6 +353,7 @@
   c.img_w = CONV == CONV_UP2X ? img_w / 2 : CONV >= CONV_S2 ? 2 * img_w : img_w;
   c.cin2 = x_row_bytes;
   c.cpt = CONV ? K / (9 * BK) : 1;
+  c.a_wrap = wrap ? c.cpt / 3 * 2 : c.cpt;
   c.px_mask[0] = c.px_mask[1] = 0;
   if (CONV) {
 #pragma unroll
@@ -404,8 +408,8 @@
 
   const int nt = K / BK;
   const KPos p0 = {0, 0, 0, 0};
-  KPos pa = k_next<CONV>(p0, c.cpt);
-  KPos pb = k_next<CONV>(pa, c.cpt);
+  KPos pa = k_next<CONV, OUT32>(p0, c.cpt, c.a_wrap);
+  KPos pb = k_next<CONV, OUT32>(pa, c.cpt, c.a_wrap);
   const bool half = !ROWS && EPI == 1 && n0 + BN >= I;
   if (ROWS) {
     stage_w<0>(lds, c, 0, 0);
@@ -424,10 +428,10 @@
     for (; tr + 1 < nt; tr += 2) {
       tile_phases_rows<T, 0, CONV>(lds, c, f, acc, true, tr + 2 < nt, pa, pb);
       pa = pb;
-      pb = k_next<CONV>(pb, c.cpt);
+      pb = k_next<CONV, OUT32>(pb, c.cpt, c.a_wrap);
       tile_phases_rows<T, 1, CONV>(lds, c, f, acc, tr + 2 < nt, tr + 3 < nt, pa, pb);
       pa = pb;
-      pb = k_next<CONV>(pb, c.cpt);
+      pb = k_next<CONV, OUT32>(pb, c.cpt, c.a_wrap);
     }
     if (tr < nt) tile_phases_rows<T, 0, CONV>(lds, c, f, acc, false, false, pa, pb);
     if (wrow == 0) ED_BARRIER();
@@ -448,10 +452,10 @@
     for (; th + 1 < nt; th += 2) {
       tile_phases_half<T, 0, CONV>(lds, c, f, acc, th, true, th + 2 < nt, pa, pb);
       pa = pb;
-      pb = k_next<CONV>(pb, c.cpt);
+      pb = k_next<CONV, OUT32>(pb, c.cpt, c.a_wrap);
       tile_phases_half<T, 1, CONV>(lds, c, f, acc, th + 1, th + 2 < nt, th + 3 < nt, pa, pb);
       pa = pb;
-      pb = k_next<CONV>(pb, c.cpt);
+      pb = k_next<CONV, OUT32>(pb, c.cpt, c.a_wrap);
     }
     if (th < nt) tile_phases_half<T, 0, CONV>(lds, c, f, acc, th, false, false, pa, pb);
     if (wrow == 0) ED_BARRIER();
@@ -479,10 +483,10 @@
     for (; t + 1 < nt; t += 2) {
       tile_phases_two<T, 0, CONV>(lds, c, f, acc, t, true, t + 2 < nt, pa, pb);
       pa = pb;
-      pb = k_next<CONV>(pb, c.cpt);
+      pb = k_next<CONV, OUT32>(pb, c.cpt, c.a_wrap);
       tile_phases_two<T, 1, CONV>(lds, c, f, acc, t + 1, t + 2 < nt, t + 3 < nt, pa, pb);
       pa = pb;
-      pb = k_next<CONV>(pb, c.cpt);
+      pb = k_next<CONV, OUT32>(pb, c.cpt, c.a_wrap);
     }
     if (t < nt) tile_phases_two<T, 0, CONV>(lds, c, f, acc, t, false, false, pa, pb);
     t = nt;
@@ -490,19 +494,19 @@
   if (early) {
     tile_phases<T, 0, CONV, true>(lds, c, f, acc, 0, true, true, pa, pb);
     pa = pb;
-    pb = k_next<CONV>(pb, c.cpt);
+    pb = k_next<CONV, OUT32>(pb, c.cpt, c.a_wrap);
     tile_phases<T, 1, CONV>(lds, c, f, acc, 1, true, 3 < nt, pa, pb);
     pa = pb;
-    pb = k_next<CONV>(pb, c.cpt);
+    pb = k_next<CONV, OUT32>(pb, c.cpt, c.a_wrap);
     t = 2;
   }
   for (; t + 1 < nt; t += 2) {
     tile_phases<T, 0, CONV>(lds, c, f, acc, t, true, t + 2 < nt, pa, pb);
     pa = pb;
-    pb = k_next<CONV>(pb, c.cpt);
+    pb = k_next<CONV, OUT32>(pb, c.cpt, c.a_wrap);
     tile_phases<T, 1, CONV>(lds, c, f, acc, t + 1, t + 2 < nt, t + 3 < nt, pa, pb);
     pa = pb;
-    pb = k_next<CONV>(pb, c.cpt);
+    pb = k_next<CONV, OUT32>(pb, c.cpt, c.a_wrap);
   }
   if (t < nt) tile_phases<T, 0, CONV>(lds, c, f, acc, t, false, false, pa, pb);
   if (wrow == 0) ED_BARRIER();
@@ -630,7 +634,7 @@
     c.wr_ = __builtin_amdgcn_make_buffer_rsrc((void*)w, 0, (int)((int64_t)2 * I * row_bytes), 0x00020000);
     c.x_voff[0] = (tp.m0 + ((wave & 3) + 8 * (wave >> 2)) * 16 + srow) * row_bytes + skb;
     c.x_voff[1] = c.x_voff[0] + 64 * row_bytes;
-    c.img_w = 0, c.cin2 = row_bytes, c.cpt = 1;
+    c.img_w = 0, c.cin2 = row_bytes, c.cpt = 1, c.a_wrap = 1;
     c.px_mask[0] = c.px_mask[1] = 0;
     c.w_voff[0] = (tp.n0 + 32 * (wave >> 1) + 8 * (srow >> 2) + (srow & 3) + 4 * (wave & 1)) * row_bytes + skb;
     c.w_voff[1] = c.w_voff[0] + I * row_bytes;
@@ -758,15 +762,17 @@
 template <int EPI, int CONV, bool OUT32 = false>
 static int launch(const void* x, const void* w, const void* bias, const void* row_bias, const void* residual, void* out, int dtype,
                   int64_t M, int K, int I, int img_h, int img_w, int rows_per_sample, void* stream, float out_scale = 1.0f,
-                  const float* act_absmax = nullptr) {
+                  const float* act_absmax = nullptr, bool a2seg = false) {
   if (M == 0) return 0;
   const int bad = (int)hipErrorInvalidValue;
   if (M < 0 || K % BK != 0 || K < BK || I <= 0 || (EPI == 0 ? I % BN != 0 : I % 8 != 0)) return bad;
   if (CONV && (K % (9 * BK) != 0 || img_h <= 0 || img_w <= 0 || M % ((int64_t)img_h * img_w) != 0)) return bad;
+  if (a2seg && (!OUT32 || !CONV || K % (27 * BK) != 0)) return bad;
+  const int64_t xc = CONV ? (a2seg ? K / 27 * 2 : K / 9) : K;
   if (CONV == CONV_UP2X && (img_h % 2 != 0 || img_w % 2 != 0 || row_bias || residual)) return bad;
-  if (CONV >= CONV_S2 && (row_bias || residual || 4 * M * (int64_t)(K / 9) * 2 >= 0x7ffffff0ll)) return bad;
+  if (CONV >= CONV_S2 && (row_bias || residual || 4 * M * xc * 2 >= 0x7ffffff0ll)) return bad;
   if (row_bias && (rows_per_sample <= 0 || M % rows_per_sample != 0)) return bad;
-  if (M * (int64_t)(CONV ? K / 9 : K) * 2 >= 0x7ffffff0ll || (int64_t)(EPI == 0 ? 2 : 1) * I * K * 2 >= 0x7ffffff0ll) return bad;
+  if (M * xc * 2 >= 0x7ffffff0ll || (int64_t)(EPI == 0 ? 2 : 1) * I * K * 2 >= 0x7ffffff0ll) return bad;
   if ((((uintptr_t)x | (uintptr_t)w | (uintptr_t)out | (uintptr_t)bias | (uintptr_t)row_bias | (uintptr_t)residual) & 15u)) return bad;
   const int nbn = EPI == 0 ? I / BN : (I + 2 * BN - 1) / (2 * BN);
   const int64_t nb256 = ((M + BM - 1) / BM) * nbn, nb128 = ((M + BM / 2 - 1) / (BM / 2)) * nbn;
@@ -786,7 +792,7 @@
   k_gemm_8phase<TT, EPI, CONV, ADD_, OUT32, TWO_, ROWS_><<<(int)nb, 512, 0, s>>>((const uint16_t*)x, (const uint16_t*)w, (const uint16_t*)bias, \
                                                              (const uint16_t*)row_bias, (const uint16_t*)residual, (uint16_t*)out,  \
                                                              (int)M, K, I, nbn, (int)nb, img_h, img_w, rows_per_sample > 0 ? rows_per_sample : 1, out_scale, \
-                                                             act_absmax)
+                                                             act_absmax, (int)a2seg)
 #define ED_LAUNCH(TT, ADD_)                                   \
   do {                                                        \
     if constexpr (OUT32 || EPI == 0) {                        \
@@ -884,15 +890,15 @@
 int ed_conv3x3_nhwc_f32out(const void* x, const void* w, const float* bias, const float* residual, float* out, int dtype, int B, int H, int W,
                            int Cin, int N, float out_scale, const float* act_absmax, void* stream) {
   if (B < 0 || H <= 0 || W <= 0 || Cin <= 0 || ((uintptr_t)act_absmax & 3u)) return (int)hipErrorInvalidValue;
-  return launch<1, 1, true>(x, w, bias, nullptr, residual, out, dtype, (int64_t)B * H * W, 9 * Cin, N, H, W, H * W, stream, out_scale,
-                               act_absmax);
+  return launch<1, 1, true>(x, w, bias, nullptr, residual, out, dtype & ~ED_A2SEG, (int64_t)B * H * W, 9 * Cin, N, H, W, H * W, stream, out_scale,
+                               act_absmax, (dtype & ED_A2SEG) != 0);
 }
 
 int ed_conv3x3_nhwc_f32out_s2(const void* x, const void* w, const float* bias, float* out, int dtype, int B, int H, int W, int Cin, int N,
                               float out_scale, const float* act_absmax, void* stream) {
   if (B < 0 || H <= 0 || W <= 0 || Cin <= 0 || ((uintptr_t)act_absmax & 3u)) return (int)hipErrorInvalidValue;
-  return launch<1, CONV_S2P0, true>(x, w, bias, nullptr, nullptr, out, dtype, (int64_t)B * H * W, 9 * Cin, N, H, W, H * W, stream, out_scale,
-                                    act_absmax);
-}
-
-}
+  return launch<1, CONV_S2P0, true>(x, w, bias, nullptr, nullptr, out, dtype & ~ED_A2SEG, (int64_t)B * H * W, 9 * Cin, N, H, W, H * W, stream, out_scale,
+                                    act_absmax, (dtype & ED_A2SEG) != 0);
+}
+
+}
diff --git a/elasticdiffusion_official_amd/csrc/vae_kernels.hip b/elasticdiffusion_official_amd/csrc/vae_kernels.hip
--- a/elasticdiffusion_official_amd/csrc/vae_kernels.hip
+++ b/elasticdiffusion_official_amd/csrc/vae_kernels.hip
@@ -71,7 +71,7 @@
   }
 }
 
-template <bool ACT, bool SPLIT>
+template <bool ACT, int SPLIT>
 __global__ void __launch_bounds__(GV_THREADS)
 k_gn32_nhwc_apply(const float* __restrict__ x, const float* __restrict__ gamma, const float* __restrict__ beta,
                   const float* __restrict__ partial, void* __restrict__ out, int C, int HW, int G, int rows_per_block, double count,
@@ -131,7 +131,7 @@
     };
     auto store = [&](int64_t row, const float4& y) {
       if (SPLIT) {
-        uint16_t* ob = reinterpret_cast<uint16_t*>(out) + ((int64_t)n * HW + row) * (3 * (int64_t)C) + c0;
+        uint16_t* ob = reinterpret_cast<uint16_t*>(out) + ((int64_t)n * HW + row) * (SPLIT * (int64_t)C) + c0;
         const _Float16 h0 = sat16(y.x), h1 = sat16(y.y), h2 = sat16(y.z), h3 = sat16(y.w);
         const _Float16 l0 = sat16(y.x - (float)h0), l1 = sat16(y.y - (float)h1), l2 = sat16(y.z - (float)h2), l3 = sat16(y.w - (float)h3);
         uint2 hi, lo;
@@ -141,7 +141,7 @@
         lo.y = (uint32_t)__builtin_bit_cast(uint16_t, l2) | ((uint32_t)__builtin_bit_cast(uint16_t, l3) << 16);
         *reinterpret_cast<uint2*>(ob) = hi;
         *reinterpret_cast<uint2*>(ob + C) = lo;
-        *reinterpret_cast<uint2*>(ob + 2 * C) = hi;
+        if (SPLIT == 3) *reinterpret_cast<uint2*>(ob + 2 * C) = hi;
       } else {
         *reinterpret_cast<float4*>(reinterpret_cast<float*>(out) + ((int64_t)n * HW + row) * C + c0) = y;
       }
@@ -160,7 +160,7 @@
   }
 }
 
-template <int U>
+template <int U, int S>
 __global__ void __launch_bounds__(256)
 k_split32_nhwc(const float* __restrict__ x, uint16_t* __restrict__ out, int C, int H, int W, int64_t n_vec, const float* __restrict__ absmax) {
   const int VC = C >> 2;
@@ -190,10 +190,10 @@
     for (int dy = 0; dy < U; ++dy)
 #pragma unroll
       for (int dx = 0; dx < U; ++dx) {
-        uint16_t* ob = out + ((n * (U * H) + (U * y + dy)) * (int64_t)(U * W) + (U * xx + dx)) * (3 * (int64_t)C) + c0;
+        uint16_t* ob = out + ((n * (U * H) + (U * y + dy)) * (int64_t)(U * W) + (U * xx + dx)) * (S * (int64_t)C) + c0;
         *reinterpret_cast<uint2*>(ob) = hi;
         *reinterpret_cast<uint2*>(ob + C) = lo;
-        *reinterpret_cast<uint2*>(ob + 2 * C) = hi;
+        if (S == 3) *reinterpret_cast<uint2*>(ob + 2 * C) = hi;
       }
   }
 }
@@ -251,10 +251,16 @@
 #define GV_APPLY(ACT, SPLIT)                                                                                                      \
   k_gn32_nhwc_apply<ACT, SPLIT><<<grid, GV_THREADS, 0, s>>>((const float*)x, (const float*)gamma, (const float*)beta, workspace, \
                                                             out, C, HW, G, rpb, count, eps)
-  if (act_silu && split16) GV_APPLY(true, true);
-  else if (act_silu) GV_APPLY(true, false);
-  else if (split16) GV_APPLY(false, true);
-  else GV_APPLY(false, false);
+  if (split16 < 0 || split16 > 2) return (int)hipErrorInvalidValue;
+  if (act_silu) {
+    if (split16 == 2) GV_APPLY(true, 2);
+    else if (split16) GV_APPLY(true, 3);
+    else GV_APPLY(true, 0);
+  } else {
+    if (split16 == 2) GV_APPLY(false, 2);
+    else if (split16) GV_APPLY(false, 3);
+    else GV_APPLY(false, 0);
+  }
 #undef GV_APPLY
   return done();
 }
@@ -274,6 +280,7 @@
 
 int ed_split_f32_nhwc(const void* x, void* out, int N, int C, int H, int W, int upsample2x, const float* absmax, void* stream) {
   if (N == 0) return 0;
+  const bool up = (upsample2x & ~ED_SPLIT_2SEG) != 0, two = (upsample2x & ED_SPLIT_2SEG) != 0;
   if (N < 0 || C <= 0 || C % 4 != 0 || H <= 0 || W <= 0 || (((uintptr_t)x | (uintptr_t)out) & 15u) || ((3 * C * 2) % 8) != 0 ||
       ((uintptr_t)absmax & 3u))
     return (int)hipErrorInvalidValue;
@@ -281,8 +288,15 @@
   int64_t blocks = (n_vec + 255) / 256;
   if (blocks > 65536 * 16) blocks = 65536 * 16;
   hipStream_t s = (hipStream_t)stream;
-  if (upsample2x) k_split32_nhwc<2><<<(unsigned)blocks, 256, 0, s>>>((const float*)x, (uint16_t*)out, C, H, W, n_vec, absmax);
-  else k_split32_nhwc<1><<<(unsigned)blocks, 256, 0, s>>>((const float*)x, (uint16_t*)out, C, H, W, n_vec, absmax);
+#define GV_SPLIT(U, S) k_split32_nhwc<U, S><<<(unsigned)blocks, 256, 0, s>>>((const float*)x, (uint16_t*)out, C, H, W, n_vec, absmax)
+  if (up) {
+    if (two) GV_SPLIT(2, 2);
+    else GV_SPLIT(2, 3);
+  } else {
+    if (two) GV_SPLIT(1, 2);
+    else GV_SPLIT(1, 3);
+  }
+#undef GV_SPLIT
   return done();
 }
 
diff --git a/elasticdiffusion_official_amd/models.py b/elasticdiffusion_official_amd/models.py
--- a/elasticdiffusion_official_amd/models.py
+++ b/elasticdiffusion_official_amd/models.py
@@ -113,6 +113,11 @@
 VAE_NCHW_RESIDUAL = True
 VAE_SPLIT_CONV = True
 VAE_SPLIT_DOWNSAMPLE = True
+VAE_TWO_SEGMENT = True
+
+
+def _vae_segments():
+    return 2 if VAE_TWO_SEGMENT else 3
 for _name in filter(None, os.environ.get("ED_DISABLE", "").split(",")):
     if _name not in globals() or not isinstance(globals()[_name], bool):
         raise RuntimeError(f"ED_DISABLE: unknown switch {_name!r}")
@@ -181,7 +186,7 @@
     B, cin, H, W = x.shape
     cout = blk.conv1.out_channels
     return (ops.groupnorm_nhwc_f32_ok(cin, blk.norm1.num_groups) and ops.groupnorm_nhwc_f32_ok(cout, blk.norm2.num_groups)
-            and cin % 64 == 0 and cout % 64 == 0 and H * W * 3 * max(cin, cout) * 2 < 2 ** 31 - 16)
+            and cin % 64 == 0 and cout % 64 == 0 and H * W * _vae_segments() * max(cin, cout) * 2 < 2 ** 31 - 16)
 
 
 def _split_weight(conv):
@@ -356,13 +361,14 @@
         def block(xs):
             w1, s1 = _split_weight(self.conv1)
             w2, s2 = _split_weight(self.conv2)
-            a = ops.groupnorm_nhwc_f32(xs, n1.weight, n1.bias, n1.num_groups, n1.eps, silu=True, split=True)
+            a = ops.groupnorm_nhwc_f32(xs, n1.weight, n1.bias, n1.num_groups, n1.eps, silu=True, split=True, segments=seg)
             h = ops.conv3x3_f32out(a, w1, self.conv1.bias, None, s1)
-            a = ops.groupnorm_nhwc_f32(h, n2.weight, n2.bias, n2.num_groups, n2.eps, silu=True, split=True)
+            a = ops.groupnorm_nhwc_f32(h, n2.weight, n2.bias, n2.num_groups, n2.eps, silu=True, split=True, segments=seg)
             res = xs if sc is None else _shortcut_nhwc(sc, xs)
             return ops.conv3x3_f32out(a, w2, self.conv2.bias, res, s2)
 
-        per = H * W * 3 * max(cin, self.conv1.out_channels) * 2
+        seg = _vae_segments()
+        per = H * W * seg * max(cin, self.conv1.out_channels) * 2
         return _sliced(x.contiguous(memory_format=torch.channels_last), max(1, (2 ** 31 - 16) // per), block)
 
 
@@ -569,13 +575,14 @@
         if self.padding == 0 and VAE_SPLIT_CONV and VAE_SPLIT_DOWNSAMPLE and FUSED_KERNELS and x.is_cuda and x.dtype == torch.float32 \
                 and x.dim() == 4 and self.conv.weight.dtype == torch.float32:
             B, C, H, W = x.shape
-            if C % 64 == 0 and ops.conv3x3_f32out_s2_ok(1, H, W, 3 * C, self.conv.weight.shape[0]):
+            seg = _vae_segments()
+            if C % 64 == 0 and ops.conv3x3_f32out_s2_ok(1, H, W, 3 * C, self.conv.weight.shape[0], seg):
                 w, sc = _split_weight(self.conv)
 
                 def conv(xs):
                     am = ops.absmax_f32(xs)
-                    return ops.conv3x3_f32out_s2(ops.split_f32(xs, absmax=am), w, self.conv.bias, sc, act_absmax=am)
-                return _sliced(x.contiguous(memory_format=torch.channels_last), max(1, (2 ** 31 - 16) // (H * W * 3 * C * 2)), conv)
+                    return ops.conv3x3_f32out_s2(ops.split_f32(xs, absmax=am, segments=seg), w, self.conv.bias, sc, act_absmax=am)
+                return _sliced(x.contiguous(memory_format=torch.channels_last), max(1, (2 ** 31 - 16) // (H * W * seg * C * 2)), conv)
         if self.padding == 0:
             x = F.pad(_to_nchw(x), (0, 1, 0, 1))
         if HIP_DOWNSAMPLE_CONV and HIP_CONV3X3 and self.padding == 1 and _fusable_nhwc(x) and x.shape[2] % 2 == 0 and x.shape[3] % 2 == 0:
@@ -596,7 +603,7 @@
         if not (self.vae and VAE_SPLIT_CONV and FUSED_KERNELS and x.is_cuda and x.dim() == 4 and self.conv.weight.dtype == torch.float32):
             return False
         B, C, H, W = x.shape
-        return C % 64 == 0 and 4 * H * W * 3 * C * 2 < 2 ** 31 - 16
+        return C % 64 == 0 and 4 * H * W * _vae_segments() * C * 2 < 2 ** 31 - 16
 
     def forward(self, x):
         if _stream32(x, self.conv.weight.dtype):
@@ -608,8 +615,10 @@
 
                 def conv(xs):
                     am = ops.absmax_f32(xs)
-                    return ops.conv3x3_f32out(ops.split_f32(xs, upsample2x=True, absmax=am), w, self.conv.bias, None, sc, act_absmax=am)
-                return _sliced(x.contiguous(memory_format=torch.channels_last), max(1, (2 ** 31 - 16) // (4 * H * W * 3 * C * 2)), conv)
+                    return ops.conv3x3_f32out(ops.split_f32(xs, upsample2x=True, absmax=am, segments=seg), w, self.conv.bias, None, sc,
+                                              act_absmax=am)
+                seg = _vae_segments()
+                return _sliced(x.contiguous(memory_format=torch.channels_last), max(1, (2 ** 31 - 16) // (4 * H * W * seg * C * 2)), conv)
             x = _to_nchw(x)
         if FUSED_UPSAMPLE_CONV and HIP_CONV3X3 and _fusable_nhwc(x):
             w = self.conv.weight
diff --git a/elasticdiffusion_official_amd/ops.py b/elasticdiffusion_official_amd/ops.py
--- a/elasticdiffusion_official_amd/ops.py
+++ b/elasticdiffusion_official_amd/ops.py
@@ -884,7 +884,12 @@
     return C % groups == 0 and (C // groups) % 4 == 0 and groups <= 256 and C <= 4096
 
 
-def groupnorm_nhwc_f32(x, gamma, beta, groups, eps, silu=False, split=False):
+_A2SEG, _SPLIT_2SEG = 0x100, 2
+
+
+def groupnorm_nhwc_f32(x, gamma, beta, groups, eps, silu=False, split=False, segments=3):
+    if segments not in (2, 3):
+        _reject("groupnorm_nhwc_f32: segments must be 2 or 3")
     if not (isinstance(x, torch.Tensor) and x.is_cuda and x.dim() == 4 and x.dtype == torch.float32):
         _reject("groupnorm_nhwc_f32: x must be an fp32 [N,C,H,W] tensor on the MI355X; no CPU fallback")
     N, C, H, W = x.shape
@@ -893,13 +898,13 @@
         _reject("groupnorm_nhwc_f32: x must be channels_last")
     if not groupnorm_nhwc_f32_ok(C, groups):
         _reject(f"groupnorm_nhwc_f32: unsupported C = {C}, groups = {groups}")
-    out = (torch.empty((N, 3 * C, H, W), dtype=torch.float16, device=x.device, memory_format=cl) if split
+    out = (torch.empty((N, segments * C, H, W), dtype=torch.float16, device=x.device, memory_format=cl) if split
            else torch.empty_like(x, memory_format=cl))
     nbytes = _hip.lib().ed_groupnorm_nhwc_f32_workspace(N, C, H * W, groups)
     ws = torch.empty(max(4, nbytes // 4), dtype=torch.float32, device=x.device)
-    TIMER.note_work("ed_groupnorm_nhwc_f32", nbytes=x.numel() * (4.0 + 4.0 + (6.0 if split else 4.0)))
+    TIMER.note_work("ed_groupnorm_nhwc_f32", nbytes=x.numel() * (4.0 + 4.0 + (2.0 * segments if split else 4.0)))
     _call("ed_groupnorm_nhwc_f32", x.data_ptr(), _dev(gamma, torch.float32, "gamma"), _dev(beta, torch.float32, "beta"), out.data_ptr(),
-          _dev(ws, torch.float32, "workspace"), N, C, H * W, groups, float(eps), int(silu), int(split), _stream_of(x))
+          _dev(ws, torch.float32, "workspace"), N, C, H * W, groups, float(eps), int(silu), (2 if segments == 2 else 1) if split else 0, _stream_of(x))
     return out
 
 
@@ -915,7 +920,9 @@
     return out
 
 
-def split_f32(x, upsample2x=False, absmax=None):
+def split_f32(x, upsample2x=False, absmax=None, segments=3):
+    if segments not in (2, 3):
+        _reject("split_f32: segments must be 2 or 3")
     if not (isinstance(x, torch.Tensor) and x.is_cuda and x.dim() == 4 and x.dtype == torch.float32):
         _reject("split_f32: x must be an fp32 [N,C,H,W] tensor on the MI355X; no CPU fallback")
     if absmax is not None and not (isinstance(absmax, torch.Tensor) and absmax.device == x.device and absmax.dtype == torch.float32
@@ -926,10 +933,10 @@
     if not x.is_contiguous(memory_format=cl) or C % 4:
         _reject("split_f32: x must be channels_last with C % 4 == 0")
     u = 2 if upsample2x else 1
-    out = torch.empty((N, 3 * C, u * H, u * W), dtype=torch.float16, device=x.device, memory_format=cl)
-    TIMER.note_work("ed_split_f32_nhwc", nbytes=x.numel() * (4.0 + 6.0 * u * u))
+    out = torch.empty((N, segments * C, u * H, u * W), dtype=torch.float16, device=x.device, memory_format=cl)
+    TIMER.note_work("ed_split_f32_nhwc", nbytes=x.numel() * (4.0 + 2.0 * segments * u * u))
     _LAUNCH["device"] = x.device
-    _call("ed_split_f32_nhwc", x.data_ptr(), out.data_ptr(), N, C, H, W, int(bool(upsample2x)),
+    _call("ed_split_f32_nhwc", x.data_ptr(), out.data_ptr(), N, C, H, W, int(bool(upsample2x)) | (_SPLIT_2SEG if segments == 2 else 0),
           None if absmax is None else absmax.data_ptr(), _stream())
     return out
 
@@ -944,18 +951,26 @@
     return torch.cat([hi, hi, lo], dim=1).contiguous(memory_format=torch.channels_last), 2.0 ** -k
 
 
-def conv3x3_f32out_ok(B, H, W, Cin3, N):
+def conv3x3_f32out_ok(B, H, W, Cin3, N, segments=3):
     M = B * H * W
-    return Cin3 % 64 == 0 and N % 8 == 0 and M * Cin3 * 2 < 2 ** 31 - 16 and N * 9 * Cin3 * 2 < 2 ** 31 - 16 and M < 2 ** 31
+    Ca = Cin3 if segments == 3 else Cin3 // 3 * 2
+    return (Cin3 % (64 if segments == 3 else 192) == 0 and N % 8 == 0 and M * Ca * 2 < 2 ** 31 - 16 and N * 9 * Cin3 * 2 < 2 ** 31 - 16
+            and M < 2 ** 31)
+
+
+def _a_segments(a, w):
+    Ca, C3 = a.shape[1], w.shape[1]
+    return 3 if Ca == C3 else (2 if 3 * Ca == 2 * C3 else None)
 
 
 def conv3x3_f32out(a, w, bias=None, residual=None, out_scale=1.0, act_absmax=None):
     if not (isinstance(a, torch.Tensor) and a.is_cuda and a.dim() == 4 and a.dtype == torch.float16):
         _reject("conv3x3_f32out: a must be an fp16 [B,C,H,W] tensor on the MI355X; no CPU fallback")
-    B, C3, H, W = a.shape
-    N = w.shape[0]
+    B, _, H, W = a.shape
+    N, C3 = w.shape[:2]
     cl = torch.channels_last
-    if tuple(w.shape) != (N, C3, 3, 3) or w.dtype != torch.float16 or not conv3x3_f32out_ok(B, H, W, C3, N):
+    seg = _a_segments(a, w)
+    if tuple(w.shape) != (N, C3, 3, 3) or w.dtype != torch.float16 or seg is None or not conv3x3_f32out_ok(B, H, W, C3, N, seg):
         _reject(f"conv3x3_f32out: unsupported shape a {tuple(a.shape)} w {tuple(w.shape)}")
     if not a.is_contiguous(memory_format=cl) or not w.is_contiguous(memory_format=cl):
         _reject("conv3x3_f32out: a and w must be channels_last")
@@ -963,32 +978,36 @@
     if residual is not None and (residual.shape != out.shape or residual.dtype != torch.float32 or not residual.is_contiguous(memory_format=cl)):
         _reject("conv3x3_f32out: residual must be an fp32 channels_last tensor of the output's shape")
     TIMER.note_work("ed_conv3x3_nhwc_f32out", flops=2.0 * B * H * W * 9 * C3 * N,
-                    nbytes=2.0 * (B * H * W * C3 + 9 * C3 * N) + 4.0 * B * H * W * N * (2 if residual is not None else 1))
+                    nbytes=2.0 * (a.numel() + 9 * C3 * N) + 4.0 * B * H * W * N * (2 if residual is not None else 1))
     _call("ed_conv3x3_nhwc_f32out", a.data_ptr(), w.data_ptr(), _opt(bias, torch.float32, "bias"),
-          None if residual is None else residual.data_ptr(), out.data_ptr(), _DTYPE[torch.float16], B, H, W, C3, N, float(out_scale),
+          None if residual is None else residual.data_ptr(), out.data_ptr(), _DTYPE[torch.float16] | (_A2SEG if seg == 2 else 0), B, H, W, C3, N,
+          float(out_scale),
           None if act_absmax is None else act_absmax.data_ptr(), _stream_of(a))
     return out
 
 
-def conv3x3_f32out_s2_ok(B, Hi, Wi, Cin3, N):
-    return (Hi % 2 == 0 and Wi % 2 == 0 and Cin3 % 64 == 0 and N % 8 == 0 and B * Hi * Wi * Cin3 * 2 < 2 ** 31 - 16
+def conv3x3_f32out_s2_ok(B, Hi, Wi, Cin3, N, segments=3):
+    Ca = Cin3 if segments == 3 else Cin3 // 3 * 2
+    return (Hi % 2 == 0 and Wi % 2 == 0 and Cin3 % (64 if segments == 3 else 192) == 0 and N % 8 == 0 and B * Hi * Wi * Ca * 2 < 2 ** 31 - 16
             and N * 9 * Cin3 * 2 < 2 ** 31 - 16)
 
 
 def conv3x3_f32out_s2(a, w, bias=None, out_scale=1.0, act_absmax=None):
     if not (isinstance(a, torch.Tensor) and a.is_cuda and a.dim() == 4 and a.dtype == torch.float16):
         _reject("conv3x3_f32out_s2: a must be an fp16 [B,C,H,W] tensor on the MI355X; no CPU fallback")
-    B, C3, Hi, Wi = a.shape
-    N = w.shape[0]
+    B, _, Hi, Wi = a.shape
+    N, C3 = w.shape[:2]
     cl = torch.channels_last
-    if tuple(w.shape) != (N, C3, 3, 3) or w.dtype != torch.float16 or not conv3x3_f32out_s2_ok(B, Hi, Wi, C3, N):
+    seg = _a_segments(a, w)
+    if tuple(w.shape) != (N, C3, 3, 3) or w.dtype != torch.float16 or seg is None or not conv3x3_f32out_s2_ok(B, Hi, Wi, C3, N, seg):
         _reject(f"conv3x3_f32out_s2: unsupported shape a {tuple(a.shape)} w {tuple(w.shape)}")
     if not a.is_contiguous(memory_format=cl) or not w.is_contiguous(memory_format=cl):
         _reject("conv3x3_f32out_s2: a and w must be channels_last")
     H, W = Hi // 2, Wi // 2
     out = torch.empty((B, N, H, W), dtype=torch.float32, device=a.device, memory_format=cl)
-    TIMER.note_work("ed_conv3x3_nhwc_f32out_s2", flops=2.0 * B * H * W * 9 * C3 * N, nbytes=2.0 * (B * Hi * Wi * C3 + 9 * C3 * N) + 4.0 * B * H * W * N)
-    _call("ed_conv3x3_nhwc_f32out_s2", a.data_ptr(), w.data_ptr(), _opt(bias, torch.float32, "bias"), out.data_ptr(), _DTYPE[torch.float16],
+    TIMER.note_work("ed_conv3x3_nhwc_f32out_s2", flops=2.0 * B * H * W * 9 * C3 * N, nbytes=2.0 * (a.numel() + 9 * C3 * N) + 4.0 * B * H * W * N)
+    _call("ed_conv3x3_nhwc_f32out_s2", a.data_ptr(), w.data_ptr(), _opt(bias, torch.float32, "bias"), out.data_ptr(),
+          _DTYPE[torch.float16] | (_A2SEG if seg == 2 else 0),
           B, H, W, C3, N, float(out_scale), None if act_absmax is None else act_absmax.data_ptr(), _stream_of(a))
     return out
 
diff --git a/include/elastic_hip.h b/include/elastic_hip.h
--- a/include/elastic_hip.h
+++ b/include/elastic_hip.h
@@ -8,6 +8,8 @@
 #endif
 
 enum { ED_F32 = 0, ED_F16 = 1, ED_BF16 = 2 };
+
+enum { ED_A2SEG = 0x100, ED_SPLIT_2SEG = 2 };
 
 enum { ED_PRED_EPSILON = 0, ED_PRED_V = 1 };
 
```

After: 0.1023, median of 6. About the same (+0.2%).
